# blairstar/NaturalDiffusion

Hardware: AMD Instinct MI355X
Metric: images/sec at 15-step Natural Inference (CIFAR10 32x32, NCSN++), 3-stream throughput (higher is better)
Workload: dtype bf16; 1 GPU; CIFAR10 NI 15-step step_15_weight_173.npz B=512/GPU NCSN++ 61.8M bf16, ni_step fp64 history; nfe=15, batch_per_gpu=512, streams=3

## Files before the change

include/natinf_ncsnpp.h:

```cpp
#ifndef NATINF_NCSNPP_H
#define NATINF_NCSNPP_H

#include <stdint.h>
#include "natinf.h"

#ifdef __cplusplus
extern "C" {
#endif

typedef struct natinf_ncsnpp* natinf_ncsnpp_t;

#define NATINF_NCSNPP_KEEP_ACTIVATIONS 1
#define NATINF_NCSNPP_DDPM 2

int64_t natinf_ncsnpp_param_count(void);
int64_t natinf_ncsnpp_packed_bytes(void);
int64_t natinf_ncsnpp_handle_param_count(natinf_ncsnpp_t h);
int64_t natinf_ncsnpp_handle_packed_bytes(natinf_ncsnpp_t h);
int64_t natinf_ncsnpp_workspace_bytes(natinf_ncsnpp_t h, int max_batch);

int natinf_ncsnpp_create(natinf_ncsnpp_t* out, int flags);
int natinf_ncsnpp_destroy(natinf_ncsnpp_t h);

int natinf_ncsnpp_describe(natinf_ncsnpp_t h, char* buf, int cap);

int natinf_ncsnpp_load(natinf_ncsnpp_t h, const float* params_f32, int64_t n_params,
                       void* packed, int64_t packed_bytes, natinf_stream_t stream);

int natinf_ncsnpp_share(natinf_ncsnpp_t h, natinf_ncsnpp_t loaded);

int natinf_ncsnpp_forward(natinf_ncsnpp_t h, const float* x, const float* labels, float* out, int B,
                          void* workspace, int64_t workspace_bytes, natinf_stream_t stream);

int natinf_ncsnpp_describe_gemms(natinf_ncsnpp_t h, int B, char* buf, int cap);

int natinf_debug_gemm(int variant, int M, int N, int K0, int K1, int taps, int logW, int batch,
                      const void* a0, const void* a1, const void* b, const float* bias_n, void* c, int c_f32, float scale,
                      int iters, natinf_stream_t stream);
int natinf_debug_quant_fp8_rows(const float* w, void* q, float* row_scale, int rows, int cols, natinf_stream_t stream);
int natinf_debug_gemm_fused(int variant, int M, int N, int K, const void* a, const void* b, const float* bias_n, const float* bias_m,
                            const float* rowvec, const float* gate, int log_rows_per_sample, const void* resid_bf16, const float* resid_f32,
                            float scale, int act, void* c, int c_f32, float* gn_part, int* bm_out, int fp32_slab, natinf_stream_t stream);
int natinf_debug_set_conv_operand(int logW, const void* a1, int c1);
int natinf_debug_gemm_fp8(int M, int N, int K, const void* a8, const float* a_scale, const void* a_mx, const void* b8, const float* b_scale,
                          const float* bias_n, void* c, void* c_mx, int c_mode, int iters, natinf_stream_t stream);
int natinf_debug_conv_gn_up(int flags);
int natinf_debug_conv_gn_fin(float* fin_scale, float* fin_shift, const float* gamma, const float* beta, int channels_per_group, float mul);
int natinf_debug_conv_gn(int res, int B, int N, int cin, int c1, const void* x, const float* scale, const float* shift, const void* w_packed, void* w_frag,
                         const void* a1, const float* bias_n, const void* resid, float out_scale, void* out, float* gn_part, int iters,
                         natinf_stream_t stream);
#define NATINF_ATTN_BLOCK_OFF_WQKV 0
#define NATINF_ATTN_BLOCK_OFF_W3 393216
#define NATINF_ATTN_BLOCK_OFF_FOLD_WQK 524288
#define NATINF_ATTN_BLOCK_OFF_FOLD_WVO 786432
#define NATINF_ATTN_BLOCK_OFF_FOLD_CQ 1048576
#define NATINF_ATTN_BLOCK_OFF_FOLD_BO 1049600
#define NATINF_ATTN_BLOCK_OFF_WQK_PACKED 1050624
#define NATINF_ATTN_BLOCK_OFF_WVO_PACKED 1181696
#define NATINF_ATTN_BLOCK_PACKED_BYTES 1312768
#define NATINF_ATTN_BLOCK_SCRATCH_BYTES_PER_SAMPLE 393216
int natinf_debug_attn_block(int plan, int B, const void* x, int x_ld, const float* scale, const float* shift, const float* w, const float* bias,
                            void* packed, void* scratch, void* out, int o_ld, float out_scale, float* gn_part, natinf_stream_t stream);
int natinf_set_gemm_variant(int variant);
int natinf_set_gemm_epilogue(int fp32_slab);
int natinf_set_gemm_pref512(int on);
int natinf_set_gemm_half_issue(int on);
int natinf_set_gemm_round_model(int on);
int natinf_set_gemm_w128(int on);
int natinf_set_gemm_raster(int rows);
int natinf_set_fuse_gn(int on);
int natinf_set_conv_gn_wide(int mask);
int natinf_set_conv_gn_w128(int mask);
int natinf_set_conv_gn_w128_min_k(int shape, int k);
int natinf_set_conv_gn_regw(int on);
int natinf_set_fuse_up(int on);
int natinf_set_fuse_up_fold(int on);
int natinf_debug_fold_up_weights(const float* w, int N, int cin, float w_mul, float* out_f32, void* out_packed, natinf_stream_t stream);
int natinf_debug_conv_up_fold(int B, int N, int cin, const void* x, const float* scale, const float* shift, const float* w, void* w_packed, void* h_scratch,
                              const float* bias_n, const float* rowvec, float out_scale, void* out, float* gn_part, int iters, natinf_stream_t stream);
int natinf_set_fuse_head(int on);
int natinf_set_fuse_gn8(int on);
int natinf_set_fuse_gn4(int on);
int natinf_set_fuse_fin(int on);
int natinf_set_conv_gn_warm(int mask);
int natinf_set_attn256(int on);
int natinf_set_attn_proj(int on);
int natinf_set_attn_waves8(int on);
int natinf_set_attn_block(int on);
int natinf_set_attn_qkv(int on);
int natinf_set_conv_gn8_tile(int one_image);
int natinf_set_gemm_splitk(int on);
int natinf_debug_set_splitk_workspace(float* ws, int max_slices);
int natinf_debug_timestamps(void* dev_buf16);

int natinf_ncsnpp_profile(natinf_ncsnpp_t h, int enable);
int natinf_ncsnpp_profile_read(natinf_ncsnpp_t h, double* ms_by_class , int64_t* launches_by_class );

int natinf_gemm_profile(int enable);
int natinf_gemm_profile_read(char* buf, int cap);

int natinf_ncsnpp_debug_tap(natinf_ncsnpp_t h, int module_idx, float* out, int64_t capacity_elems,
                            natinf_stream_t stream);

int natinf_debug_gn_stats(const void* x, int ld, int C, int HW, int B, const float* gamma, const float* beta, float* scale, float* shift, float eps, float out_mul,
                          natinf_stream_t stream);
int natinf_debug_gn_finalize(const float* P0, int tps0, int quads0, const float* P1, int tps1, int quads1, int C, int HW, int B, const float* gamma, const float* beta,
                             float* scale, float* shift, float eps, float out_mul, natinf_stream_t stream);
int natinf_debug_gn_fold(const float* P, int tps, int quads, int fold, int B, float* out, natinf_stream_t stream);
int natinf_debug_gn_apply(const void* x, int ld, int C, int logW, int logHW, int B, const float* scale, const float* shift, void* y, void* xr, int act, int mode, int pad,
                          natinf_stream_t stream);
int natinf_debug_head_conv(const void* x, int ld, int B, const float* scale, const float* shift, const void* w16, const float* bias, float* out, natinf_stream_t stream);
int natinf_debug_time_embed(const float* labels, void* emb, int B, natinf_stream_t stream);
int natinf_debug_stem_im2col(const float* x, void* A, int B, natinf_stream_t stream);
int natinf_debug_pack_conv(const float* src, void* dst, int N, int Cin, int taps, int dst_ld, int koff, int tap_stride_c, int chunked, float wmul, natinf_stream_t stream);
int natinf_debug_pack_transpose(const float* src, void* dst, int K, int N, int dst_ld, natinf_stream_t stream);
int natinf_debug_nhwc_to_nchw(const void* x, int ld, int C, int HW, int B, float* out, natinf_stream_t stream);

#ifdef __cplusplus
}
#endif
#endif
```

naturaldiffusion_amd/_lib.py:

```python
from __future__ import annotations

import ctypes as C
import os
from pathlib import Path

os.environ.setdefault("GPU_MAX_HW_QUEUES", "8")

_HERE = Path(__file__).resolve().parent
LIB_PATH = Path(os.environ.get("NATINF_LIB", _HERE / "libnatinf.so"))

if not LIB_PATH.exists():
    raise ImportError(
        f"{LIB_PATH} not found: build it with `make -C {_HERE / 'csrc'}` "
        "(or `python -c 'import __graft_entry__ as g; g.build()'`). "
        "naturaldiffusion_amd has no CPU or eager-PyTorch fallback.")

lib = C.CDLL(str(LIB_PATH))

_p, _i32, _i64, _f32, _f64 = C.c_void_p, C.c_int, C.c_int64, C.c_float, C.c_double

SIGNATURES = {
    "natinf_abi_version": (C.c_int, []),
    "natinf_strerror": (C.c_char_p, [_i32]),
    "natinf_probe": (C.c_int, []),
    "natinf_step_f64hist": (C.c_int, [_p, _p, _p, _p, _p, _p, _p, _i32, _f64, _i32, _f64, _f64, _f32, _f32, _i64, _p]),
    "natinf_step_f32hist": (C.c_int, [_p, _p, _p, _p, _p, _p, _p, _i32, _f32, _i32, _f32, _f32, _f32, _f32, _i64, _p]),
    "natinf_weighted_sum_f64": (C.c_int, [_p, _p, _p, _p, _i32, _i64, _p]),
    "natinf_randn_philox_f32": (C.c_int, [_p, _i64, _i64, _p, _i64, _i64, C.c_uint64, _p]),
    "natinf_randn_philox_col_f32": (C.c_int, [_p, _i64, _i64, _p, _i64, _i64, C.c_uint64, C.c_uint32, _p]),
    "natinf_step_f64hist_noise": (C.c_int, [_p, _p, _p, _p, _p, _p, _p, _i32, _f64, _p, _p, _i32, _i32, _f64, _f64, _f32,
                                            C.c_uint64, _p, _i64, _i64, _i64, _i64, _p]),
    "natinf_known_blend_f32": (C.c_int, [_p, _p, _p, _p, _i64, _i64, _f32, _f32, C.c_uint32, C.c_uint64, _p, _i64, _i64, _i64, _i64, _p]),
    "natinf_step_f64hist_inpaint": (C.c_int, [_p, _p, _p, _p, _p, _p, _p, _i32, _f64, _p, _p, _i32, _i32, _f64, _f64, _f32,
                                              C.c_uint64, _p, _i64, _i64, _i64, _i64, _p, _p, _i64, _i64, _f32, _f32, C.c_uint32, _p]),
    "natinf_x0_threshold_f64": (C.c_int, [_p, _p, _i64, _i64, _i32, _f64, _f64, _p]),
    "natinf_step_f64hist_x0fix": (C.c_int, [_p, _p, _p, _p, _p, _p, _p, _i32, _f64, _p, _p, _i32, _i32, _f64, _f64, _f32,
                                            C.c_uint64, _p, _i64, _i64, _i64, _i64, _p, _p, _i64, _i64, _f32, _f32, C.c_uint32,
                                            _i32, _f64, _f64, _p, _p]),
    "natinf_x0_project_f64": (C.c_int, [_p, _p, _p, _i64, _i32, _i32, _i32, _i32, _i64, _p]),
    "natinf_step_f64hist_project": (C.c_int, [_p, _p, _p, _p, _p, _p, _p, _i32, _f64, _p, _p, _i32, _i32, _f64, _f64, _f32,
                                              C.c_uint64, _p, _i64, _i64, _i64, _i64, _p, _i64, _i32, _i32, _i32, _i32, _p, _p]),
    "natinf_color_blend_f32": (C.c_int, [_p, _p, _p, _i64, _p, _p, _f32, _f32, C.c_uint32, C.c_uint64, _p, _i64, _i64, _i64, _i64, _p]),
    "natinf_step_f64hist_colorize": (C.c_int, [_p, _p, _p, _p, _p, _p, _p, _i32, _f64, _p, _p, _i32, _i32, _f64, _f64, _f32,
                                               C.c_uint64, _p, _i64, _i64, _i64, _i64, _p, _i64, _p, _p, _f32, _f32, C.c_uint32, _p]),
    "natinf_to_pixel_u8": (C.c_int, [_p, _p, _i32, _i32, _i32, _i32, _i32, _p]),
    "natinf_step_f32prod": (C.c_int, [_p, _p, _p, _f32, _i64, _i64, _p, _p, _p, _p, _p, _i32, _f32, _p, _p, _i32,
                                      _i32, _f32, _f32, _i64, _p]),
    "natinf_step_f32prod_noise": (C.c_int, [_p, _p, _p, _f32, _i64, _i64, _p, _p, _p, _p, _p, _i32, _f32, _p, _p, _i32,
                                            _i32, _f32, _f32, C.c_uint64, _p, _i64, _i64, _i64, _p]),
    "natinf_step_f32prod_noise_guided": (C.c_int, [_p, _p, _p, _p, _p, _i32, _i64, _i64, _p, _p, _p, _p, _p, _i32, _f32, _p, _p, _i32,
                                                   _i32, _f32, _f32, C.c_uint64, _p, _i64, _i64, _i64, _p]),
    "natinf_step_f32prod_inpaint": (C.c_int, [_p, _p, _p, _p, _p, _i32, _i64, _i64, _p, _p, _p, _p, _p, _i32, _f32, _p, _p, _i32,
                                              _i32, _f32, _f32, C.c_uint64, _p, _i64, _i64, _i64,
                                              _p, _p, _i64, _i64, _f32, _f32, C.c_uint32, _p]),
    "natinf_weighted_sum_f32prod": (C.c_int, [_p, _p, _p, _p, _i32, _i64, _p]),
    "natinf_step_f16chain": (C.c_int, [_p, _p, _p, _p, _p, _p, _p, _p, _p, _i32, _f32, _f32, _i32, _f32, _f32, _f32,
                                       _f32, _i32, _i64, _p]),
    "natinf_step_f16chain_guided": (C.c_int, [_p, _p, _p, _p, _p, _i32, _i64, _p, _p, _p, _p, _p, _p, _i32, _f32, _f32, _i32, _f32, _f32,
                                              _f32, _i32, _i64, _p]),
    "natinf_known_blend_f16": (C.c_int, [_p, _p, _p, _p, _p, _i64, _i64, _f32, _f32, C.c_uint32, C.c_uint64, _p, _i64, _i64, _i64, _i64, _p]),
    "natinf_step_f16chain_inpaint": (C.c_int, [_p, _p, _p, _p, _p, _i32, _i64, _p, _p, _p, _p, _p, _p, _i32, _f32, _f32, _i32, _f32, _f32,
                                               _f32, _i32, _i64, _p, _p, _i64, _i64, C.c_uint32, C.c_uint64, _p, _i64, _i64, _p]),
    "natinf_weighted_mean_f16": (C.c_int, [_p, _p, _p, _p, _i32, _f32, _i64, _p]),
    "natinf_flow_input_f16": (C.c_int, [_p, _p, _p, _f32, _f32, _i64, _p]),
    "natinf_ncsnpp_param_count": (C.c_int64, []),
    "natinf_ncsnpp_workspace_bytes": (C.c_int64, [_p, _i32]),
    "natinf_ncsnpp_packed_bytes": (C.c_int64, []),
    "natinf_ncsnpp_handle_param_count": (_i64, [_p]),
    "natinf_ncsnpp_handle_packed_bytes": (_i64, [_p]),
    "natinf_ncsnpp_create": (C.c_int, [C.POINTER(_p), _i32]),
    "natinf_ncsnpp_describe": (C.c_int, [_p, C.c_char_p, _i32]),
    "natinf_ncsnpp_destroy": (C.c_int, [_p]),
    "natinf_ncsnpp_load": (C.c_int, [_p, _p, _i64, _p, _i64, _p]),
    "natinf_ncsnpp_share": (C.c_int, [_p, _p]),
    "natinf_ncsnpp_forward": (C.c_int, [_p, _p, _p, _p, _i32, _p, _i64, _p]),
    "natinf_ncsnpp_debug_tap": (C.c_int, [_p, _i32, _p, _i64, _p]),
    "natinf_ncsnpp_describe_gemms": (C.c_int, [_p, _i32, C.c_char_p, _i32]),
    "natinf_debug_gemm": (C.c_int, [_i32, _i32, _i32, _i32, _i32, _i32, _i32, _i32, _p, _p, _p, _p, _p, _i32, _f32, _i32, _p]),
    "natinf_set_gemm_variant": (C.c_int, [_i32]),
    "natinf_debug_timestamps": (C.c_int, [_p]),
    "natinf_set_gemm_epilogue": (C.c_int, [_i32]),
    "natinf_debug_gemm_fused": (C.c_int, [_i32, _i32, _i32, _i32, _p, _p, _p, _p, _p, _p, _i32, _p, _p, _f32, _i32, _p, _i32, _p, _p, _i32, _p]),
    "natinf_set_gemm_pref512": (C.c_int, [_i32]),
    "natinf_set_gemm_half_issue": (C.c_int, [_i32]),
    "natinf_set_gemm_raster": (C.c_int, [_i32]),
    "natinf_set_gemm_round_model": (C.c_int, [_i32]),
    "natinf_set_gemm_w128": (C.c_int, [_i32]),
    "natinf_set_fuse_gn": (C.c_int, [_i32]),
    "natinf_set_conv_gn_wide": (C.c_int, [_i32]),
    "natinf_set_attn_block": (C.c_int, [_i32]),
    "natinf_set_conv_gn_w128": (C.c_int, [_i32]),
    "natinf_set_conv_gn_w128_min_k": (C.c_int, [_i32, _i32]),
    "natinf_set_conv_gn_regw": (C.c_int, [_i32]),
    "natinf_set_fuse_up": (C.c_int, [_i32]),
    "natinf_set_fuse_up_fold": (C.c_int, [_i32]),
    "natinf_debug_fold_up_weights": (C.c_int, [_p, _i32, _i32, _f32, _p, _p, _p]),
    "natinf_debug_conv_up_fold": (C.c_int, [_i32, _i32, _i32, _p, _p, _p, _p, _p, _p, _p, _p, _f32, _p, _p, _i32, _p]),
    "natinf_set_fuse_head": (C.c_int, [_i32]),
    "natinf_set_fuse_gn8": (C.c_int, [_i32]),
    "natinf_set_fuse_gn4": (C.c_int, [_i32]),
    "natinf_set_fuse_fin": (C.c_int, [_i32]),
    "natinf_set_attn_proj": (C.c_int, [_i32]),
    "natinf_set_attn_waves8": (C.c_int, [_i32]),
    "natinf_set_attn_qkv": (C.c_int, [_i32]),
    "natinf_set_conv_gn_warm": (C.c_int, [_i32]),
    "natinf_set_attn256": (C.c_int, [_i32]),
    "natinf_set_conv_gn8_tile": (C.c_int, [_i32]),
    "natinf_set_gemm_splitk": (C.c_int, [_i32]),
    "natinf_debug_set_splitk_workspace": (C.c_int, [_p, _i32]),
    "natinf_debug_set_conv_operand": (C.c_int, [_i32, _p, _i32]),
    "natinf_debug_conv_gn": (C.c_int, [_i32, _i32, _i32, _i32, _i32, _p, _p, _p, _p, _p, _p, _p, _p, _f32, _p, _p, _i32, _p]),
    "natinf_debug_conv_gn_up": (C.c_int, [_i32]),
    "natinf_debug_conv_gn_fin": (C.c_int, [_p, _p, _p, _p, _i32, _f32]),
    "natinf_debug_attn_block": (C.c_int, [_i32, _i32, _p, _i32, _p, _p, _p, _p, _p, _p, _p, _i32, _f32, _p, _p]),
    "natinf_debug_gn_stats": (C.c_int, [_p, _i32, _i32, _i32, _i32, _p, _p, _p, _p, _f32, _f32, _p]),
    "natinf_debug_gn_finalize": (C.c_int, [_p, _i32, _i32, _p, _i32, _i32, _i32, _i32, _i32, _p, _p, _p, _p, _f32, _f32, _p]),
    "natinf_debug_gn_fold": (C.c_int, [_p, _i32, _i32, _i32, _i32, _p, _p]),
    "natinf_debug_gn_apply": (C.c_int, [_p, _i32, _i32, _i32, _i32, _i32, _p, _p, _p, _p, _i32, _i32, _i32, _p]),
    "natinf_debug_head_conv": (C.c_int, [_p, _i32, _i32, _p, _p, _p, _p, _p, _p]),
    "natinf_debug_time_embed": (C.c_int, [_p, _p, _i32, _p]),
    "natinf_debug_stem_im2col": (C.c_int, [_p, _p, _i32, _p]),
    "natinf_debug_pack_conv": (C.c_int, [_p, _p, _i32, _i32, _i32, _i32, _i32, _i32, _i32, _f32, _p]),
    "natinf_debug_pack_transpose": (C.c_int, [_p, _p, _i32, _i32, _i32, _p]),
    "natinf_debug_nhwc_to_nchw": (C.c_int, [_p, _i32, _i32, _i32, _i32, _p, _p]),
    "natinf_ncsnpp_profile": (C.c_int, [_p, _i32]),
    "natinf_ncsnpp_profile_read": (C.c_int, [_p, C.POINTER(C.c_double), C.POINTER(C.c_int64)]),
    "natinf_debug_quant_fp8_rows": (C.c_int, [_p, _p, _p, _i32, _i32, _p]),
    "natinf_debug_gemm_fp8": (C.c_int, [_i32, _i32, _i32, _p, _p, _p, _p, _p, _p, _p, _p, _i32, _i32, _p]),
    "natinf_dit_create": (C.c_int, [C.POINTER(_p), _i32, _i32, _i32, _i32]),
    "natinf_dit_create_sized": (C.c_int, [C.POINTER(_p), _i32, _i32, _i32, _i32, _i32]),
    "natinf_dit_input_size": (C.c_int, [_p]),
    "natinf_dit_attention_bf16": (C.c_int, [_p, _p, _p, _i32, _p, _i32, _i32, _i32, _i32, _i32, _i32, _p]),
    "natinf_dit_destroy": (C.c_int, [_p]),
    "natinf_dit_param_count": (C.c_int64, [_p]),
    "natinf_dit_packed_bytes": (C.c_int64, [_p]),
    "natinf_dit_workspace_bytes": (C.c_int64, [_p, _i32]),
    "natinf_dit_load": (C.c_int, [_p, _p, _i64, _p, _i64, _p]),
    "natinf_dit_forward": (C.c_int, [_p, _p, _p, _p, _p, _i32, _p, _i64, _p]),
    "natinf_dit_stream_sites": (C.c_int, [_p]),
    "natinf_dit_stream_status_reset": (C.c_int, [_p, _p, _p]),
    "natinf_dit_stream_status": (C.c_int, [_p, _p, _p, _p]),
    "natinf_debug_ln_modulate": (C.c_int, [_p, _i32, _p, _p, _i32, _p, _p, _p, _i32, _i64, _i32, C.POINTER(_i32), _p]),
    "natinf_debug_softmax_rows": (C.c_int, [_i32, _p, _p, _i32, _i64, _p]),
    "natinf_mmdit_create": (C.c_int, [C.POINTER(_p), _i32, _i32, _i32, _i32, _i32, _i32, _i32, _i32]),
    "natinf_mmdit_destroy": (C.c_int, [_p]),
    "natinf_mmdit_param_count": (C.c_int64, [_p]),
    "natinf_mmdit_packed_bytes": (C.c_int64, [_p]),
    "natinf_mmdit_workspace_bytes": (C.c_int64, [_p, _i32]),
    "natinf_mmdit_load": (C.c_int, [_p, _p, _i64, _p, _i64, _p]),
    "natinf_mmdit_forward": (C.c_int, [_p, _p, _p, _p, _p, _p, _i32, _p, _i64, _p]),
    "natinf_mmdit_stream_sites": (C.c_int, [_p]),
    "natinf_mmdit_stream_status_reset": (C.c_int, [_p, _p, _p]),
    "natinf_mmdit_stream_status": (C.c_int, [_p, _p, _p, _p]),
    "natinf_attention_hd64_bf16": (C.c_int, [_p, _p, _i32, _i64, _p, _p, _i32, _i64, _i32, _i32, _i32, _i32, C.c_float, _p]),
    "natinf_debug_attention_hd64_fp8out": (C.c_int, [_p, _p, _i32, _i64, _p, _p, _p, _i32, _i32, _i32, _i32, C.c_float, _p]),
    "natinf_inception_create": (C.c_int, [_p, _i32, _i32]),
    "natinf_inception_destroy": (C.c_int, [_p]),
    "natinf_set_inception_conv": (C.c_int, [_i32]),
    "natinf_debug_conv_ring": (C.c_int, [_i32] * 14 + [_p, _p, _p, _p, _p, _p, _i32, _p]),
    "natinf_debug_inc_stem": (C.c_int, [_p, _i32, _i32, _i32, _i32, _i32, _i32, _p, _p]),
    "natinf_debug_inc_pool": (C.c_int, [_i32] * 8 + [_p, _i32, _p, _i32, _p]),
    "natinf_debug_inc_global_avg": (C.c_int, [_i32, _i32, _i32, _i32, _p, _p, _p]),
    "natinf_debug_inc_pack": (C.c_int, [_i32, _p, _p, _p, _p, _p] + [_i32] * 7 + [_p, _p, _p, _p]),
    "natinf_debug_inc_im2col": (C.c_int, [_i32] * 11 + [_p, _p, _p]),
    "natinf_inception_param_count": (_i64, [_p]),
    "natinf_inception_packed_bytes": (_i64, [_p]),
    "natinf_inception_workspace_bytes": (_i64, [_p, _i32]),
    "natinf_inception_load": (C.c_int, [_p, _p, _i64, _p, _i64, _p]),
    "natinf_inception_forward": (C.c_int, [_p, _p, _i32, _p, _i32, _p, _i64, _p]),
    "natinf_gemm_profile": (C.c_int, [_i32]),
    "natinf_gemm_profile_read": (C.c_int, [_p, _i32]),
    "natinf_set_mmdit_stream16": (C.c_int, [_i32]),
    "natinf_set_dit_stream16": (C.c_int, [_i32]),
    "natinf_set_mmdit_text_flat": (C.c_int, [_i32]),
    "natinf_attention_profile": (C.c_int, [_i32]),
    "natinf_set_mmdit_text_stream": (C.c_int, [_i32]),
    "natinf_set_flash_mode": (C.c_int, [_i32]),
    "natinf_attention_profile_read": (C.c_int, [_p, _p]),
    "natinf_vae_create": (C.c_int, [C.POINTER(_p), _i32, _i32]),
    "natinf_vae_destroy": (C.c_int, [_p]),
    "natinf_vae_param_count": (C.c_int64, [_p]),
    "natinf_vae_packed_bytes": (C.c_int64, [_p]),
    "natinf_vae_workspace_bytes": (C.c_int64, [_p, _i32]),
    "natinf_vae_load": (C.c_int, [_p, _p, _i64, _p, _i64, _p]),
    "natinf_vae_decode": (C.c_int, [_p, _p, _p, _i32, _p, _i64, _p]),
    "natinf_vae_enc_create": (C.c_int, [C.POINTER(_p), _i32, _i32]),
    "natinf_vae_enc_destroy": (C.c_int, [_p]),
    "natinf_vae_enc_param_count": (C.c_int64, [_p]),
    "natinf_vae_enc_packed_bytes": (C.c_int64, [_p]),
    "natinf_vae_enc_workspace_bytes": (C.c_int64, [_p, _i32]),
    "natinf_vae_enc_load": (C.c_int, [_p, _p, _i64, _p, _i64, _p]),
    "natinf_vae_posterior_f32": (C.c_int, [_p, _p, _i64, _i32, _i64, _i32, _f32, _f32, C.c_uint64, _p, _i64, _i64, _p]),
    "natinf_vae_encode": (C.c_int, [_p, _p, _p, _p, _i32, _i32, _f32, _f32, C.c_uint64, _p, _i64, _i64, _p, _i64, _p]),
    "natinf_posterior_workspace_bytes": (C.c_int64, [_i32, _i32]),
    "natinf_posterior_samples": (C.c_int, [_p, _p, _f32, _f32, C.c_uint64, _p, _i64, _i64, _i32, _i32, _p, _p]),
    "natinf_posterior_stats": (C.c_int, [_p, _f64, _i32, _i32, _p, _p, _p, _p]),
    "natinf_posterior_debug_planes": (C.c_int, [_p, _i32, _i32, _p]),
    "natinf_prdc_workspace_bytes": (C.c_int64, [_i64, _i64, _i32, _i32]),
    "natinf_prdc_planes": (C.c_int, [_p, _i64, _i32, _p, _p, _p]),
    "natinf_prdc_knn_radius": (C.c_int, [_p, _p, _i64, _p, _p, _i64, _i32, _i32, _i64, _p, _p, _i64, _p]),
    "natinf_prdc_ball_counts": (C.c_int, [_p, _p, _i64, _p, _p, _i64, _i32, _i64, _p, _p, _p, _p, _p]),
    "natinf_prdc_debug_dist2": (C.c_int, [_p, _p, _i64, _p, _p, _i64, _i32, _i64, _p, _p]),
    "natinf_nn_workspace_bytes": (C.c_int64, [_i64, _i64, _i32, _i32]),
    "natinf_nn_nearest": (C.c_int, [_p, _p, _i64, _p, _p, _i64, _i32, _i32, _i64, _p, _p, _p, _i64, _p]),
    "natinf_kid_workspace_bytes": (C.c_int64, [_i64, _i64, _i32]),
    "natinf_kid_row_sums": (C.c_int, [_p, _i64, _i64, _p, _i64, _i64, _i32, _i64, _f64, _f64, _p, _p, _i64, _p]),
    "natinf_is_workspace_bytes": (C.c_int64, [_i64, _i32, _i32]),
    "natinf_is_row_stats": (C.c_int, [_p, _i64, _i64, _p, _i64, _i32, _i32, _p, _p, _p, _p, _p, _p, _i64, _p]),
    "natinf_ideal_tplanes": (C.c_int, [_p, _i64, _i32, _p, _p]),
    "natinf_ideal_workspace_bytes": (C.c_int64, [_i64, _i64, _i32]),
    "natinf_ideal_posterior_mean": (C.c_int, [_p, _p, _i64, _p, _p, _p, _i64, _i32, _i64, _p, _p, _p, _p, _p, _p, _p, _p, _p, _i64, _p]),
    "natinf_ideal_debug_weights": (C.c_int, [_p, _p, _i64, _p, _p, _i64, _i32, _i64, _p, _p, _p, _i64, _p]),
    "natinf_fit_gram_f64": (C.c_int, [_p, _i64, C.POINTER(C.c_int32), _i32, _p, _p, _i64, _i64, _p, _p]),
}

for _name, (_res, _args) in SIGNATURES.items():
    try:
        _fn = getattr(lib, _name)
    except AttributeError as e:
        raise ImportError(f"{LIB_PATH} does not export {_name}; rebuild it") from e
    _fn.restype, _fn.argtypes = _res, _args

X0_CLIP, X0_DYNAMIC = 1, 2
SD3_CFG_ON_VELOCITY = 1
SD3_BLEND_MEAN = 2
DIT_UNFUSED_ATTENTION = 1
DIT_FP8 = 2
DIT_STREAM_GUARD = 16
MMDIT_FP8 = 1
MMDIT_STREAM_GUARD = 2


def check(rc: int, what: str) -> None:
    if rc != 0:
        raise RuntimeError(f"{what} failed: {lib.natinf_strerror(rc).decode()} ({rc})")


def stream_ptr(stream=None) -> int:
    import torch
    s = stream if stream is not None else torch.cuda.current_stream()
    return int(s.cuda_stream)


def ptr(t) -> int:
    return 0 if t is None else int(t.data_ptr())


class StreamGuardStatus:
    _guard_api = ""
    guard = False

    def _guard_entry(self, name):
        if not self.guard:
            raise RuntimeError("this engine was created without guard=True: it keeps no stream status")
        return getattr(lib, f"{self._guard_api}_{name}")

    @property
    def site_names(self):
        n = self._guard_entry("stream_sites")(self._h)
        check(min(n, 0), f"{self._guard_api}_stream_sites")
        return ["patch_embed"] + [f"blocks.{i // 2}.{'mlp' if i % 2 else 'attn'}" for i in range(n - 1)]

    def reset_stream_status(self) -> None:
        import torch
        with torch.cuda.device(self._ws.device):
            check(self._guard_entry("stream_status_reset")(self._h, ptr(self._ws), stream_ptr()), f"{self._guard_api}_stream_status_reset")

    def stream_status(self):
        import torch
        n = len(self.site_names)
        buf = torch.empty(2 * n, dtype=torch.int32, device=self._ws.device)
        with torch.cuda.device(self._ws.device):
            check(self._guard_entry("stream_status")(self._h, ptr(self._ws), ptr(buf), stream_ptr()), f"{self._guard_api}_stream_status")
        raw = buf.cpu().numpy().view("uint32").reshape(n, 2)
# ... 10 lines not shown
```

naturaldiffusion_amd/csrc/engine_core.h:

```cpp
#pragma once
#include <functional>
#include <map>
#include <vector>

#include "natinf_ncsnpp.h"
#include "gemm_launch.h"

namespace ncsn {

__global__ void k_transpose_f32(const float* __restrict__ src, float* __restrict__ dst, int N, int K)
{
    const int64_t i = (int64_t)blockIdx.x * blockDim.x + threadIdx.x;
    if (i >= (int64_t)N * K) return;
    const int n = (int)(i / K), k = (int)(i - (int64_t)n * K);
    dst[(int64_t)k * N + n] = src[i];
}
}

namespace {

inline int ilog2(int v) { int l = 0; while ((1 << l) < v) ++l; return l; }
inline int64_t align_up(int64_t v, int64_t a) { return (v + a - 1) / a * a; }

struct TRef { int64_t off = -1; int C = 0, ld = 0, res = 0, coff = 0, pad = 0; };

struct Ctx {
    int B; unsigned char* ws; const unsigned char* wp; hipStream_t stream;
    const float* x; const float* labels; float* out;
    int* part_bm;
    hipStream_t stream2 = nullptr; hipEvent_t* ev = nullptr;
    unsigned char* fin_done = nullptr;
    uint32_t* guard = nullptr;
    uint32_t* site(int i) const { return guard ? guard + 2 * i : nullptr; }
    bf16* act(const TRef& t) const { return reinterpret_cast<bf16*>(ws + t.off * B) + t.coff; }
    template <class T> T* at(int64_t off) const { return reinterpret_cast<T*>(ws + off * B); }
    template <class T> const T* w(int64_t off) const { return reinterpret_cast<const T*>(wp + off); }
};
using OpFn = std::function<void(const Ctx&)>;

struct PackCtx { const float* params; unsigned char* packed; hipStream_t stream; };
using PackFn = std::function<void(const PackCtx&)>;

struct Arena {
    bool keep = false; int64_t top = 0, peak = 0;
    std::map<int64_t, int64_t> free_;
    std::map<int64_t, int64_t> live_;
    int64_t alloc(int64_t bytes) {
        bytes = align_up(bytes, 256);
        if (!keep)
            for (auto it = free_.begin(); it != free_.end(); ++it)
                if (it->second >= bytes) {
                    const int64_t off = it->first, rest = it->second - bytes;
                    free_.erase(it);
                    if (rest) free_[off + bytes] = rest;
                    live_[off] = bytes;
                    return off;
                }
        const int64_t off = top; top += bytes; if (top > peak) peak = top;
        live_[off] = bytes;
        return off;
    }
    void release(int64_t off) {
        if (keep || off < 0) return;
        auto it = live_.find(off);
        if (it == live_.end()) return;
        int64_t o = off, s = it->second;
        live_.erase(it);
        auto nx = free_.lower_bound(o);
        if (nx != free_.end() && o + s == nx->first) { s += nx->second; nx = free_.erase(nx); }
        if (nx != free_.begin()) { auto pv = std::prev(nx); if (pv->first + pv->second == o) { o = pv->first; s += pv->second; free_.erase(pv); } }
        if (o + s == top) top = o; else free_[o] = s;
    }
};

}

struct EngineCore {
    int64_t n_params = 0, packed_bytes = 0, ws_per_image = 0;
    std::vector<OpFn> ops;
    std::vector<PackFn> packs;
    const unsigned char* packed = nullptr;
    bool configured = false;
    std::vector<int> part_bm{128};
    int guard_sites = 0;
    int64_t guard_bytes() const { return guard_sites ? align_up((int64_t)guard_sites * 8, 256) : 0; }
    int64_t workspace_bytes(int max_batch) const { return ws_per_image * (int64_t)max_batch + guard_bytes(); }
    int status_reset(void* ws, hipStream_t s) const {
        if (!guard_sites || !ws) return NATINF_EINVAL;
        return hipMemsetAsync(ws, 0, (size_t)guard_sites * 8, s) == hipSuccess ? NATINF_OK : NATINF_ELAUNCH;
    }
    int status_read(const void* ws, uint32_t* out_dev, hipStream_t s) const {
        if (!guard_sites || !ws || !out_dev) return NATINF_EINVAL;
        return hipMemcpyAsync(out_dev, ws, (size_t)guard_sites * 8, hipMemcpyDeviceToDevice, s) == hipSuccess ? NATINF_OK : NATINF_ELAUNCH;
    }
    int load(const float* params_f32, int64_t n, void* dst, int64_t dst_bytes, hipStream_t s) {
        if (!params_f32 || !dst || n != n_params || dst_bytes < packed_bytes) return NATINF_EINVAL;
        PackCtx p{params_f32, reinterpret_cast<unsigned char*>(dst), s};
        for (const auto& f : packs) f(p);
        packed = reinterpret_cast<const unsigned char*>(dst);
        return hipGetLastError() == hipSuccess ? NATINF_OK : NATINF_ELAUNCH;
    }
    int run(const float* x, const float* t, float* out, int B, void* ws, int64_t ws_bytes, hipStream_t s, hipStream_t s2 = nullptr, hipEvent_t* ev = nullptr) {
        if (!x || !t || !out || !ws || B <= 0) return NATINF_EINVAL;
        if (!packed) return NATINF_ESTATE;
        if (ws_bytes < workspace_bytes(B)) return NATINF_EINVAL;
        if (!configured) { if (!configure_gemm_kernels()) return NATINF_ENODEV; configured = true; }
        Ctx c{B, reinterpret_cast<unsigned char*>(ws) + guard_bytes(), packed, s, x, t, out, part_bm.data()};
        c.stream2 = s2; c.ev = ev;
        if (guard_sites) { c.guard = reinterpret_cast<uint32_t*>(ws); g_launch_error = 0; }
        for (const auto& f : ops) f(c);
        if (guard_sites && g_launch_error) { g_launch_error = 0; return NATINF_ESTATE; }
        return hipGetLastError() == hipSuccess ? NATINF_OK : NATINF_ELAUNCH;
    }
};

namespace {

struct PlanBuilder {
    EngineCore& E;
    Arena arena;
    int64_t wtop = 0, poff = 0;
    explicit PlanBuilder(EngineCore& e) : E(e) {}
    int64_t wres(int64_t bytes) { const int64_t o = wtop; wtop += align_up(bytes, 256); return o; }
    int64_t take(int64_t n) { const int64_t o = poff; poff += n; return o; }
    void op(OpFn f) { E.ops.push_back(std::move(f)); }
    int64_t pack_bf16(int64_t src, int rows, int cols) {
        const int64_t dst = wres((int64_t)rows * cols * 2);
        E.packs.push_back([=](const PackCtx& p) {
            const int64_t n = (int64_t)rows * cols;
            hipLaunchKernelGGL(k_pack_conv, dim3(grid1d(n, 256, 1 << 30)), dim3(256), 0, p.stream, p.params + src,
                               reinterpret_cast<bf16*>(p.packed + dst), rows, cols, 1, cols, 0, cols, 0, 1.0f);
        });
        return dst;
    }
    void pack_bf16_at(int64_t src, int rows, int cols, int64_t dst) {
        E.packs.push_back([=](const PackCtx& p) {
            const int64_t n = (int64_t)rows * cols;
            hipLaunchKernelGGL(k_pack_conv, dim3(grid1d(n, 256, 1 << 30)), dim3(256), 0, p.stream, p.params + src,
                               reinterpret_cast<bf16*>(p.packed + dst), rows, cols, 1, cols, 0, cols, 0, 1.0f);
        });
    }
    int64_t pack_f32(int64_t src, int64_t n, int64_t src2 = -1) {
        const int64_t dst = wres(n * 4);
        pack_f32_at(src, n, dst, src2);
        return dst;
    }
    int64_t pack_f32_transposed(int64_t src, int rows, int cols) {
        const int64_t dst = wres((int64_t)rows * cols * 4);
        E.packs.push_back([=](const PackCtx& p) {
            const int64_t n = (int64_t)rows * cols;
            hipLaunchKernelGGL(k_transpose_f32, dim3(grid1d(n, 256, 1 << 30)), dim3(256), 0, p.stream, p.params + src,
                               reinterpret_cast<float*>(p.packed + dst), rows, cols);
        });
        return dst;
    }
    void pack_f32_at(int64_t src, int64_t n, int64_t dst, int64_t src2 = -1) {
        E.packs.push_back([=](const PackCtx& p) {
            hipLaunchKernelGGL(k_copy_add_f32, dim3(grid1d(n, 256, 1 << 30)), dim3(256), 0, p.stream, p.params + src,
                               src2 >= 0 ? p.params + src2 : (const float*)nullptr, reinterpret_cast<float*>(p.packed + dst), (int)n);
        });
    }

    void pack_fp8_at(int64_t src, int rows, int cols, int64_t wdst, int64_t sdst) {
        E.packs.push_back([=](const PackCtx& p) {
            hipLaunchKernelGGL(k_pack_fp8_rows, dim3((unsigned)((rows + 3) / 4)), dim3(256), 0, p.stream, p.params + src,
                               reinterpret_cast<uint8_t*>(p.packed + wdst), reinterpret_cast<float*>(p.packed + sdst), rows, cols);
        });
    }

    void finish() { E.n_params = poff; E.packed_bytes = wtop; E.ws_per_image = arena.peak; }
};

}
```

naturaldiffusion_amd/csrc/gemm_launch.h:

```cpp
#pragma once
#include <hip/hip_runtime.h>
#include <stdint.h>
#include <stdio.h>
#include <string.h>
#include <string>
#include <type_traits>
#include <utility>
#include <vector>

#include "ncsnpp_kernels.h"
#include "gemm_dma.h"
#include "gemm_w128.h"
#include "conv_gn2.h"
#include "gemm_fp8.h"

using namespace ncsn;

bool configure_conv_ring();
namespace { bool configure_ncsnpp_kernels();
            bool configure_dit_attention();
            bool configure_flash_attention(); }
namespace ncsn_sg { bool configure(); bool has_tile(int variant); void launch_tile(const void* gemm_args, int variant, int raster, void* stream);
                    void launch_fp8(const void* gemm_args, int mxa, int w128, int raster, void* stream); void launch_splitk_reduce(const void* gemm_args, int slices, void* stream);
                    void launch_patch_embed(const float* z, const float* Wt, const float* bias, const float* pos, float* x, int C, int g, int D, int64_t rows, int x_f16, uint32_t* guard, void* stream); }
namespace ncsn_upf { bool configure(); void launch(const void* gemm_args, int epi, void* stream); void fold(const float* w, void* dst_bf16, float* dst_f32, int N, int Cin, float wmul, void* stream); }
namespace ncsn_cg3 { bool configure(); int tile_rows(int shape); int tile_cols(int shape); void launch(const void* gemm_args, int shape, int epi, void* stream); }

namespace {

int g_epi_fp32_slab = 0;
GemmArgs gemm_defaults() {
    GemmArgs g;
    memset(&g, 0, sizeof(g));
    g.epi_fp32_slab = g_epi_fp32_slab;
    g.taps = 1; g.batch = 1; g.scale = 1.0f; g.act = ACT_NONE; g.c_mode = OUT_BF16;
    return g;
}
constexpr int NUM_CU = 256;
enum GemmVariant {
    V_AUTO = 0, V_GENERIC = 1,
    V_DMA_256x256 = 2, V_DMA_256x128 = 3, V_DMA_128x128 = 4,
    V_RING_256x256 = 5, V_RING_256x128 = 6, V_RING_128x128 = 7,
    V_RING_64x128 = 8,
    V_RING_256x128_W4 = 9,
    V_DMA_256x128_W4 = 10,
    V_DMA_256x256_S = 11, V_DMA_128x128_S = 12,
    V_DMA_512x128 = 13,
    V_PATCH_256x256 = 14, V_PATCH_256x128 = 15,
    V_DMA_256x256_P = 16, V_DMA_256x128W4_P = 18,
    V_DMA_128x128_P = 17,
    V_8PH_256x256 = 19, V_8PH_NOPRIO = 20, V_8PH_READFIRST = 21, V_8PH_BOTH = 22,
    V_FP8_256x256 = 23,
    V_ABL_NODMA = 24, V_ABL_NOMFMA = 25,
    V_DMA_256x256_H = 26, V_DMA_512x128_H = 27,
    V_CONV_GN = 28,
    V_W128 = 29,
    V_W128_A = 30, V_W128_D = 31, V_W128_X = 32,
    V_COUNT
};
const char* variant_name(int v) {
    static const char* n[] = {"auto", "generic128", "dma256x256", "dma256x128", "dma128x128", "ring256x256", "ring256x128",
                              "ring128x128", "ring64x128", "ring256x128w4", "dma256x128w4", "dma256x256s", "dma128x128s", "dma512x128", "patch256x256", "patch256x128", "dma256x256p", "dma128x128p", "dma256x128w4p", "gemm8ph", "gemm8ph_np", "gemm8ph_rf", "gemm8ph_nprf", "fp8_256x256", "abl_nodma", "abl_nomfma", "dma256x256h", "dma512x128h", "conv_gn", "w128_256x256", "w128_a", "w128_d", "w128_x"};
    return v >= 0 && v < V_COUNT ? n[v] : "?";
}
unsigned long long* g_dbg_ts = nullptr;
int g_force_variant = V_AUTO;
int g_round_model = 1;
int g_round_model_w128 = 13;
int g_pref_512 = 1;
std::string* g_record = nullptr;

int g_raster_g = 8;
template <class Cfg, class K>
inline void launch_tiles(K kernel, const GemmArgs& g0, hipStream_t s) {
    const int nM = (g0.M + Cfg::BM_ - 1) / Cfg::BM_, nN = (g0.N + Cfg::BN_ - 1) / Cfg::BN_;
    GemmArgs g = g0;
    g.raster_g = (g_raster_g > 1 && nN >= 8 && nM >= g_raster_g) ? g_raster_g : 0;
    hipLaunchKernelGGL(kernel, dim3(nM * nN, 1, g.batch), dim3(Cfg::THREADS), Cfg::LDS_BYTES, s, g);
}
template <class Cfg, class K>
inline bool set_lds(K kernel) {
    return hipFuncSetAttribute(reinterpret_cast<const void*>(kernel), hipFuncAttributeMaxDynamicSharedMemorySize, Cfg::LDS_BYTES) == hipSuccess;
}
int g_cg_warm = 15;

constexpr unsigned EPI_ALL = 0x1FF;
template <unsigned MASK, int E, class F> inline void epi_case(F&& f) { if constexpr ((MASK >> E) & 1u) f(std::integral_constant<int, E>{}); }
template <unsigned MASK, class F> inline bool for_each_epi(F&& f) {
    bool ok = true;
    auto one = [&](auto tag) { ok = ok && f(tag); };
    epi_case<MASK, 0>(one); epi_case<MASK, 1>(one); epi_case<MASK, 2>(one); epi_case<MASK, 3>(one); epi_case<MASK, 4>(one);
    epi_case<MASK, 5>(one); epi_case<MASK, 6>(one); epi_case<MASK, 7>(one); epi_case<MASK, 8>(one);
    return ok;
}
#define NATINF_EPI_OF(tag) decltype(tag)::value

template <class... F> struct FamList {};
template <class Fam> bool configure_family() {
    return for_each_epi<Fam::EPI>([](auto t) { return set_lds<typename Fam::Cfg>(Fam::template kernel<NATINF_EPI_OF(t)>()); });
}
template <class... F> bool configure_families(FamList<F...>) { return (configure_family<F>() && ...); }
template <class Fam> void launch_family(int e, const GemmArgs& g, hipStream_t s) {
    for_each_epi<Fam::EPI>([&](auto t) {
        if (NATINF_EPI_OF(t) != e) return true;
        launch_tiles<typename Fam::Cfg>(Fam::template kernel<NATINF_EPI_OF(t)>(), g, s);
        return false;
    });
}

using CfgD256x256 = DmaCfg<2, 4, 8, 4>;
struct FamD128  { static constexpr int V = V_DMA_128x128_P;    using Cfg = DmaCfg<2, 2, 4, 4>;     static constexpr unsigned EPI = EPI_ALL;
                  template <int E> static constexpr auto kernel() { return &k_gemm_dma<2, 2, 4, 4, 2, E>; } };
struct FamRW4   { static constexpr int V = V_RING_256x128_W4;  using Cfg = RingCfg<2, 2, 8, 4, 3>; static constexpr unsigned EPI = EPI_ALL & ~(1u << 3);
                  template <int E> static constexpr auto kernel() { return &k_gemm_ring<2, 2, 8, 4, 3, E>; } };
struct FamR64   { static constexpr int V = V_RING_64x128;      using Cfg = RingCfg<2, 2, 2, 4, 4>; static constexpr unsigned EPI = EPI_ALL;
                  template <int E> static constexpr auto kernel() { return &k_gemm_ring<2, 2, 2, 4, 4, E>; } };
struct FamD256H { static constexpr int V = V_DMA_256x256_H;    using Cfg = CfgD256x256;            static constexpr unsigned EPI = EPI_ALL & ~(1u << 3);
                  template <int E> static constexpr auto kernel() { return &k_gemm_dma<2, 4, 8, 4, 6, E>; } };
struct FamD512H { static constexpr int V = V_DMA_512x128_H;    using Cfg = DmaCfg<4, 2, 8, 4>;     static constexpr unsigned EPI = EPI_ALL & ~((1u << 3) | (1u << 4) | (1u << 7) | (1u << 8));
                  template <int E> static constexpr auto kernel() { return &k_gemm_dma<4, 2, 8, 4, 6, E>; } };
struct FamW128  { static constexpr int V = V_W128;             using Cfg = W128Cfg;                static constexpr unsigned EPI = EPI_ALL & ~((1u << 2) | (1u << 3) | (1u << 6));
                  template <int E> static constexpr auto kernel() { return &k_gemm_w128<E>; } };
using GemmFamilies = FamList<FamD128, FamRW4, FamR64, FamD256H, FamD512H, FamW128>;
using CfgR128x128 = RingCfg<2, 2, 4, 4, 4>;

template <class F, class... Fam> constexpr bool with_family(int v, F&& f, FamList<Fam...>) { return ((v == Fam::V && (f(Fam{}), true)) || ...); }
template <class F> constexpr bool with_family(int v, F&& f) { return with_family(v, f, GemmFamilies{}); }
constexpr bool variant_shipped(int v) {
    return v == V_AUTO || v == V_GENERIC || v == V_FP8_256x256 || v == V_CONV_GN || with_family(v, [](auto) {});
}
constexpr unsigned epi_mask(int v) { unsigned m = 1u; with_family(v, [&](auto f) { m = decltype(f)::EPI; }); return m; }
constexpr int variant_bm(int v) {
    int bm = (v == V_CONV_GN || v == V_FP8_256x256) ? 256 : 128;
    with_family(v, [&](auto f) { bm = decltype(f)::Cfg::BM_; });
    return bm;
}
static_assert(variant_bm(V_RING_64x128) == 64 && variant_bm(V_DMA_128x128_P) == 128 && variant_bm(V_RING_256x128_W4) == 256 && variant_bm(V_DMA_256x256_H) == 256 &&
              variant_bm(V_DMA_512x128_H) == 512 && variant_bm(V_W128) == 256 && variant_bm(V_GENERIC) == 128, "the block-tile rows choose_variant and the GroupNorm partial tables count on");
static_assert(variant_shipped(V_W128) && !variant_shipped(V_DMA_256x256) && !variant_shipped(V_W128_X) && epi_mask(V_GENERIC) == 1u, "retired ids stay refused");

constexpr unsigned EPI_CONV_GN = (1u << 1) | (1u << 2) | (1u << 5) | (1u << 6);
template <int RES_, bool WIDE, int TM = 8, int NG = 1, int TN = 4> struct CgShape {
    static constexpr int RES = RES_; using Cfg = ConvGn2Cfg<RES_, WIDE, TM, NG, TN>; static constexpr unsigned EPI = EPI_CONV_GN;
    template <int E> static constexpr auto kernel() { return &k_conv_gn2<RES_, WIDE, E, TM, NG, TN>; }
    static bool takes(int res, int bm) { return res == RES_ && (RES_ <= 8 || WIDE == (bm == 128)); }
};
using CgH4T = CgShape<4, true, 4, 2, 2>;
using ConvGnShapes = FamList<CgShape<32, false>, CgShape<32, true>, CgShape<16, false>, CgShape<16, true>, CgShape<8, true, 4>, CgH4T>;
template <class... S> void launch_conv_gn2(FamList<S...>, int res, int bm, int e, const GemmArgs& g, hipStream_t s) {
    ((S::takes(res, bm) && (launch_family<S>(e, g, s), true)) || ...);
}

constexpr int UPFOLD_W = 16, UPFOLD_BM = UPFOLD_W * UPFOLD_W, UPFOLD_BN = 256;

constexpr unsigned EPI_FP8 = 0xF;
template <bool MXA> struct FamF8     { using Cfg = CfgD256x256; static constexpr unsigned EPI = EPI_FP8; template <int E> static constexpr auto kernel() { return &k_gemm_fp8<MXA, E>; } };
template <bool MXA> struct FamF8W128 { using Cfg = W128F8Cfg;   static constexpr unsigned EPI = EPI_FP8; template <int E> static constexpr auto kernel() { return &k_gemm_w128_fp8<MXA, E>; } };
using Fp8Families = FamList<FamF8<false>, FamF8<true>, FamF8W128<false>, FamF8W128<true>>;

bool configure_gemm_kernels() {
    bool ok = hipFuncSetAttribute(reinterpret_cast<const void*>(&k_gemm_bf16), hipFuncAttributeMaxDynamicSharedMemorySize,
                                  GEMM_LDS_BYTES) == hipSuccess;
    ok = ok && set_lds<CfgR128x128>(&k_gemm_ring<2, 2, 4, 4, 4, 9>) && set_lds<W128Cfg>(&k_gemm_w128<9>) &&
         configure_families(GemmFamilies{}) && configure_families(ConvGnShapes{}) && ncsn_upf::configure() && configure_families(Fp8Families{}) &&
         ncsn_cg3::configure() && ncsn_sg::configure() && ::configure_conv_ring() && configure_ncsnpp_kernels() && configure_dit_attention() && configure_flash_attention();
    if (!ok) (void)hipGetLastError();
    return ok;
}


int packed_epi(const GemmArgs& g, int bm);
int g_cg3 = 7;
int g_cg_wide = 3;
int g_cg3_min_k[3] = {2304, 0, 2304};
inline int conv_gn3_shape(const GemmArgs& g) {
    const int res = 1 << g.logW;
    if (!g_cg3 || !g.b_frag || g.N % 128) return -1;
    int sh = -1;
    if (res == 32) sh = g.N % 256 ? ((g_cg3 & 1) ? 0 : -1) : ((g_cg3 & 2) ? 1 : -1);
    else if (res == 16) sh = (g.N % 256 == 0 && (g_cg3 & 4)) ? 2 : -1;
    if (sh >= 0 && 9 * g.a0_C + (g.a1 ? g.a1_C : 0) < g_cg3_min_k[sh]) sh = -1;
    return sh;
}
inline int conv_gn_bm(const GemmArgs& g) {
    const int res = 1 << g.logW;
    if (const int sh3 = conv_gn3_shape(g); sh3 >= 0) return ncsn_cg3::tile_rows(sh3);
    if (res == 8 || res == 4) return 64;
    if (res == 32) return ((g_cg_wide & 2) && g.N % 256 == 0 && g.b_frag) ? 128 : 256;
    return ((g_cg_wide & 1) && res == 16 && g.N % 256 == 0) ? 128 : 256;
}
inline int conv_gn_part_rows(const GemmArgs& g) { const int res = 1 << g.logW; return res <= 8 ? res * res : conv_gn_bm(g); }
inline bool conv_gn_regw(const GemmArgs& g) { return g.b_frag && (conv_gn3_shape(g) >= 0 || g.N % ((conv_gn_bm(g) <= 128 && (1 << g.logW) != 4) ? 256 : 128) == 0); }
inline int conv_gn_epi(const GemmArgs& g) { GemmArgs t = g; t.epi_fp32_slab = 0; return packed_epi(t, conv_gn_part_rows(g)); }
inline bool conv_gn_ok(const GemmArgs& g) {
    if (!g.gn_scale || !g.gn_shift || !g.gn_folded || g.taps != 9 || g.batch != 1 || g.a0_C % BK || (g.a1 && g.a1_C % BK)) return false;
    const int res = 1 << g.logW;
    if (g.logHW != 2 * g.logW || (res != 32 && res != 16 && res != 8 && res != 4) || g.N % 8) return false;
    if (res == 4 && (g.a0_C % (64 * CgH4T::Cfg::NG) || (g.a1 && g.a1_C % (64 * CgH4T::Cfg::NG)))) return false;
    if (res <= 8 ? (g.M % (res * res) || g.N % (res == 4 ? 128 : 256) || g.a0_up || g.a1_up || (g.resid && g.rowvec)) : g.M % std::max(256, conv_gn_bm(g)) != 0) return false;
    if (!conv_gn_regw(g)) return false;
    const int e = conv_gn_epi(g);
    return e == 1 || e == 2 || e == 5 || e == 6;
}
int g_w128 = 1;
bool w128_ok(const GemmArgs& g) {
    if (g.taps != 1 || g.a1 || g.gn_scale || g.deq_m || g.deq_n || g.splitk > 1) return false;
    if (g.a0_C % BK || g.a0_C < 2 * BK || g.N % 8 || g.M % 8) return false;
    return (int64_t)g.M * g.a0_ld * 2 < (int64_t)1 << 32 && (int64_t)g.N * g.b_ld * 2 < (int64_t)1 << 32;
}
int choose_variant(const GemmArgs& g) {
    if (g.gn_scale) return V_CONV_GN;
    const int K0 = g.taps * g.a0_C, K1 = g.a1 ? g.a1_C : 0;
    const bool dma = K0 % BK == 0 && K1 % BK == 0 && (g.taps == 1 || (g.a0_padded && g.a0_C % BK == 0));
    if (!dma) return V_GENERIC;
    if (g_force_variant == V_W128) {
        if (w128_ok(g) && (!g.gn_part || (1 << g.logHW) % 256 == 0)) return V_W128;
    }
    else if (g_force_variant > V_GENERIC && g_force_variant != V_CONV_GN && g_force_variant != V_FP8_256x256) {
        if (!g.gn_part || ((g.taps == 9 || g.logHW > 0) && (1 << g.logHW) % variant_bm(g_force_variant) == 0)) return g_force_variant;
    }
    const int64_t mt256 = (g.M + 255) / 256, mt128 = (g.M + 127) / 128;
    const int64_t nt128 = (g.N + 127) / 128;
    const bool w128 = g_w128 && w128_ok(g) && (!g.gn_part || (1 << g.logHW) % 256 == 0);
    const int64_t nt256 = (g.N + 255) / 256;
    const bool n_ok256 = g.N % 256 == 0 || (w128 && g.N % 128 == 0);
    if (g_round_model && g.taps == 1 && !g.gn_part && g.batch == 1 && n_ok256 && K0 + K1 >= 1024 && mt256 * nt256 < 2 * NUM_CU) {
        const int64_t r256 = (mt256 * nt256 + NUM_CU - 1) / NUM_CU, r128 = (mt128 * nt128 + 2 * NUM_CU - 1) / (2 * NUM_CU);
        const int64_t c256 = w128 ? g_round_model_w128 : 15;
        if (mt128 * nt128 >= NUM_CU / 2) return c256 * r256 < 10 * r128 ? (w128 ? V_W128 : V_DMA_256x256_H) : V_DMA_128x128_P;
    }
    if (n_ok256 && K0 + K1 >= 1024 && mt256 * nt256 * g.batch >= NUM_CU) return w128 ? V_W128 : V_DMA_256x256_H;
    if (g_pref_512 && g.N <= 128 && K0 + K1 >= 1024 && ((g.M + 511) / 512) * g.batch >= 2 * NUM_CU &&
        (!g.gn_part || (g.taps == 9 && (1 << g.logHW) % 512 == 0)))
        return V_DMA_512x128_H;
    if (mt256 * nt128 * g.batch >= 2 * NUM_CU) return V_RING_256x128_W4;
    if (mt128 * nt128 * g.batch >= NUM_CU) return V_DMA_128x128_P;
    return V_RING_64x128;
}

int fp8_epi(const GemmArgs& g) {
    if (g.epi_fp32_slab || g.resid || g.gn_part) return 0;
    if ((g.rowvec || g.gate) && g.log_rows_per_sample < 30 && ((1 << g.log_rows_per_sample) % 256 != 0)) return 0;
    if (g.c_mode == OUT_F32 && g.resid_f32 && !g.bias_m && g.act == ACT_NONE && g.resid_f32_ld % 4 == 0 && g.c_ld % 4 == 0) return 3;
    if (g.resid_f32 || g.gate) return 0;
    if (g.c_mode == OUT_BF16 && g.act == ACT_NONE) return 1;
    if (g.c_mode == OUT_FP8_MX && g.act == ACT_GELU_TANH && g.c_mx && g.N % 32 == 0 && !g.bias_m && g.scale == 1.0f) return 2;
    return 0;
}
bool w128_fp8_ok(const GemmArgs& g) {
    return g.taps == 1 && !g.a1 && g.a0_C % 256 == 0 && g.N % 8 == 0 && g.M % 8 == 0 && (!g.a_mx || g.M % 256 == 0) &&
           (int64_t)g.M * g.a0_ld < (int64_t)1 << 32 && (int64_t)g.N * g.b_ld < (int64_t)1 << 32;
}
bool fp8_on_w128(const GemmArgs& g) { return g_w128 && w128_fp8_ok(g) && (fp8_epi(g) != 2 || g_w128 != 2); }
template <bool MXA>
void launch_gemm_fp8_t(const GemmArgs& g, hipStream_t s) {
    if (fp8_on_w128(g)) launch_family<FamF8W128<MXA>>(fp8_epi(g), g, s);
    else launch_family<FamF8<MXA>>(fp8_epi(g), g, s);
}
std::string gemm_row(int M, int N, int K0, int K1, int taps, int batch, const std::string& name, int epi) {
    char line[160];
    snprintf(line, sizeof(line), "%d %d %d %d %d %d %s/e%d", M, N, K0, K1, taps, batch, name.c_str(), epi);
    return line;
}
void record_gemm(const GemmArgs& g, const std::string& name, int epi) { *g_record += gemm_row(g.M, g.N, g.taps * g.a0_C, g.a1 ? g.a1_C : 0, g.taps, g.batch, name, epi) + "\n"; }
struct GemmProf {
    struct Rec { hipEvent_t a, b; std::string tag; };
    bool on = false; std::vector<Rec> ev; std::vector<std::pair<hipEvent_t, hipEvent_t>> pool;
    bool begin(Rec& r, hipStream_t s) {
        r.a = r.b = nullptr;
        if (!pool.empty()) { r.a = pool.back().first; r.b = pool.back().second; pool.pop_back(); }
        else if (hipEventCreate(&r.a) != hipSuccess || hipEventCreate(&r.b) != hipSuccess) { r.a = r.b = nullptr; (void)hipGetLastError(); return false; }
        (void)hipEventRecord(r.a, s);
        return true;
    }
    void end(Rec& r, hipStream_t s) { (void)hipEventRecord(r.b, s); ev.push_back(std::move(r)); }
} g_gemm_prof;
thread_local int g_launch_error = 0;
void launch_gemm_fp8(const GemmArgs& g, hipStream_t s) {
    if (g.stream_guard && fp8_epi(g) != 3) { g_launch_error = 1; return; }
    GemmProf::Rec r;
    const bool prof = g_gemm_prof.on && !g_record && g_gemm_prof.begin(r, s);
    if (prof) r.tag = gemm_row(g.M, g.N, g.taps * g.a0_C, 0, g.taps, g.batch, std::string(fp8_on_w128(g) ? "w128_fp8" : "fp8_256x256") + (g.a_mx ? "_mxa" : ""), g.stream_guard ? 4 : fp8_epi(g));
    if (g.stream_guard) ncsn_sg::launch_fp8(&g, g.a_mx != nullptr, fp8_on_w128(g), g_raster_g, (void*)s);
    else if (g.a_mx) launch_gemm_fp8_t<true>(g, s); else launch_gemm_fp8_t<false>(g, s);
    if (prof) g_gemm_prof.end(r, s);
}

int packed_epi(const GemmArgs& g, int bm) {
    if (g.epi_fp32_slab || g.deq_m || g.deq_n || g.act == ACT_RELU) return 0;
    if (g.bias_m) return (g.c_mode == OUT_BF16 && !g.resid && !g.resid_f32 && !g.gate && !g.rowvec && !g.gn_part && g.act == ACT_NONE) ? 8 : 0;
    if ((g.rowvec || g.gate) && g.log_rows_per_sample < 30 && ((1 << g.log_rows_per_sample) % bm != 0)) return 0;
    if (g.c_mode == OUT_F32 && g.resid_f32 && !g.resid && !g.gn_part && g.act == ACT_NONE && g.resid_f32_ld % 4 == 0 && g.c_ld % 4 == 0) return 7;
    if (g.c_mode != OUT_BF16 || g.resid_f32 || g.gate) return 0;
    if (g.resid && (g.act != ACT_NONE || g.resid_ld % 4 != 0)) return 0;
    if (g.gn_part) return (g.act == ACT_NONE && g.M % bm == 0) ? (g.resid ? 6 : 2) : 0;
    if (g.resid) return 5;
    return g.act == ACT_NONE ? 1 : (g.act == ACT_SILU ? 3 : 4);
}
inline int effective_epi(int v, const GemmArgs& g) { const int e = packed_epi(g, variant_bm(v)); return ((epi_mask(v) >> e) & 1u) ? e : 0; }

thread_local bool g_fin_written = false;
int g_splitk = 1;
float* g_dbg_splitk_ws = nullptr; int g_dbg_splitk_max = 0;
int splitk_slices(const GemmArgs& g) {
    if (!g_splitk || !g.splitk_ws || g.splitk_max < 2 || g.batch != 1 || g.gn_scale || g.c_mode != OUT_BF16 || g.N % 8 || 256 % (g.N / 8)) return 1;
    if (g.gn_part && (g.M % SPLITK_ROWS || g.act != ACT_NONE || (g.taps == 9 && (1 << g.logHW) % SPLITK_ROWS))) return 1;
    if (g.bias_m || g.gate || g.resid_f32 || g.deq_m || g.deq_n) return 1;
    const int K0 = g.taps * g.a0_C, K1 = g.a1 ? g.a1_C : 0;
    if (K0 % 64 || K1 % 64 || (g.taps == 9 && !g.a0_padded) || K0 + K1 < 2048) return 1;
    const int64_t tiles = ((g.M + 127) / 128) * ((g.N + 127) / 128);
    if (tiles >= 2 * NUM_CU) return 1;
    int S = (int)((2 * NUM_CU + tiles - 1) / tiles);
    if (S > g.splitk_max) S = g.splitk_max;
    while (S > 1 && (K0 + K1) / 32 / S < 16) --S;
    return S;
}
int w128_splitk_slices(const GemmArgs& g) {
// ... 101 lines not shown
```

naturaldiffusion_amd/csrc/ncsnpp.hip:

```cpp
#include <hip/hip_runtime.h>
#include <stdint.h>
#include <stdio.h>
#include <string.h>
#include <stdlib.h>
#include <functional>
#include <map>
#include <memory>
#include <string>
#include <vector>

#include "natinf_ncsnpp.h"
#include "gemm_launch.h"
#include "engine_core.h"
#include "head_conv.h"
#include "attn256.h"
#include "attn_qkv.h"
#include "attn_blk256.h"

namespace {

constexpr int NF = 128, IMG = 32, TEMB = 512, NLEVEL = 4;
constexpr int CH_MULT[NLEVEL] = {1, 2, 2, 2};
constexpr float GN_EPS = 1e-6f;
constexpr float INV_SQRT2 = 0.70710678118654752440f;
inline bool attn_at(int res) { return res == 16; }

enum Kind { K_LIN, K_CONV, K_RES, K_ATTN, K_GN, K_DOWN, K_UP };
const char* kind_name(int k) { static const char* n[] = {"lin", "conv", "res", "attn", "gn", "down", "up"}; return n[k]; }

struct Mod { int idx, kind, cin, cout, up, down, res; int64_t poff; };

enum { CLS_GEMM = 0, CLS_OTHER = 1, CLS_CONV_GN = 2, CLS_CONV_GN8 = 3, N_CLS = 4 };

int g_fuse_head = 1;
constexpr int ATTN_BLK_DEFAULT = 2;
int g_attn_blk = ATTN_BLK_DEFAULT;
int g_attn_qkv = 1;
int g_attn_w8 = 1;
int g_attn_proj = 1;
int g_fuse_gn8 = 1;
int g_fuse_fin = 3;
int g_fuse_gn4 = 1;
int g_fuse_gn = 1;
constexpr int UP_FOLD_DEFAULT = 1;
int g_fuse_up_fold = UP_FOLD_DEFAULT;
int g_fuse_up = 1;

}

struct natinf_ncsnpp : EngineCore {
    int flags = 0;
    std::vector<Mod> mods;
    std::vector<int> op_cls;
    bool prof = false;
    struct Rec { hipEvent_t a, b; int cls; };
    std::vector<Rec> recs;
    std::vector<hipEvent_t> pool;
    std::map<int, TRef> taps;
    uint64_t plan_sig = 0;
    int last_B = 0; unsigned char* last_ws = nullptr;
    std::vector<unsigned char> fin_done;
};

namespace {

bool configure_ncsnpp_kernels() {
    return hipFuncSetAttribute(reinterpret_cast<const void*>(&k_head_conv), hipFuncAttributeMaxDynamicSharedMemorySize, HeadConvCfg::LDS_BYTES) == hipSuccess &&
           hipFuncSetAttribute(reinterpret_cast<const void*>(&k_qkv256), hipFuncAttributeMaxDynamicSharedMemorySize, QKV_LDS_BYTES) == hipSuccess &&
           hipFuncSetAttribute(reinterpret_cast<const void*>(&k_attn256<false>), hipFuncAttributeMaxDynamicSharedMemorySize, A256_LDS_BYTES) == hipSuccess &&
           hipFuncSetAttribute(reinterpret_cast<const void*>(&k_attn256<true>), hipFuncAttributeMaxDynamicSharedMemorySize, A256_LDS_BYTES) == hipSuccess &&
           hipFuncSetAttribute(reinterpret_cast<const void*>(&k_attn256<true, 8>), hipFuncAttributeMaxDynamicSharedMemorySize, A256_LDS_BYTES) == hipSuccess &&
           hipFuncSetAttribute(reinterpret_cast<const void*>(&k_attn_blk256), hipFuncAttributeMaxDynamicSharedMemorySize, ABLK_LDS_BYTES) == hipSuccess &&
           hipFuncSetAttribute(reinterpret_cast<const void*>(&k_attn_blk256_v2), hipFuncAttributeMaxDynamicSharedMemorySize, ABLK2_LDS_BYTES) == hipSuccess;
}

struct AttnBlk256 {
    int plan = 0;
    int B = 0;
    const bf16* x = nullptr; int x_ld = 0;
    const float* sc = nullptr; const float* sh = nullptr;
    const bf16* wqkvf = nullptr; const float* bqk = nullptr; const float* bv = nullptr; bf16* qk = nullptr; bf16* vT = nullptr;
    const bf16* w3f = nullptr; const float* b3 = nullptr;
    const bf16* wqf2 = nullptr; const float* cq2 = nullptr; const bf16* wvof2 = nullptr; const float* bo2 = nullptr;
    bf16* out = nullptr; int o_ld = 0; float out_scale = 1.0f;
    float2* gn_part = nullptr; int gn_quads = 0;
};
void pack_attn_qkv_w(const float* w0, const float* w1, const float* w2, bf16* wqkvf, hipStream_t s) {
    hipLaunchKernelGGL(k_pack_qkv_w, dim3(3 * 256), dim3(256), 0, s, w0, w1, w2, wqkvf);
}
void pack_attn_w3(const float* w3, bf16* w3f, hipStream_t s) { hipLaunchKernelGGL(k_pack_attn_w3, dim3(256), dim3(256), 0, s, w3, w3f); }
void pack_attn_fold(const float* w0, const float* w1, const float* w2, const float* w3, const float* b0, const float* b2, const float* b3,
                    float* fq, float* cq, float* fv, float* bo, bf16* wqf2, bf16* wvof2, hipStream_t s) {
    hipLaunchKernelGGL(k_attn_fold_w, dim3(257), dim3(256), 0, s, w0, w1, w2, w3, b0, b2, b3, fq, cq, fv, bo);
    hipLaunchKernelGGL(k_pack_qkv_w, dim3(256), dim3(256), 0, s, (const float*)fq, (const float*)fq, (const float*)fq, wqf2, 1);
    hipLaunchKernelGGL(k_pack_attn_w3, dim3(256), dim3(256), 0, s, (const float*)fv, wvof2);
}
void launch_attn_qkv256(const AttnBlk256& a, hipStream_t s) {
    hipLaunchKernelGGL(k_qkv256, dim3((unsigned)a.B), dim3(512), QKV_LDS_BYTES, s, a.x, a.x_ld, a.sc, a.sh, a.wqkvf, a.bqk, a.bv, a.qk, a.vT);
}
int launch_attn_blk256(const AttnBlk256& a, hipStream_t s) {
    constexpr int C = 256;
    if (a.plan == 2) {
        hipLaunchKernelGGL(k_attn_blk256_v2, dim3((unsigned)a.B), dim3(512), ABLK2_LDS_BYTES, s, a.x, a.x_ld, a.sc, a.sh,
                           a.wqf2, a.cq2, 1.0f / sqrtf((float)C), a.wvof2, a.bo2, a.out, a.o_ld, a.out_scale, a.gn_part, a.gn_quads);
        return 256;
    }
    if (a.plan == 1) {
        hipLaunchKernelGGL(k_attn_blk256, dim3((unsigned)a.B), dim3(512), ABLK_LDS_BYTES, s, a.x, a.x_ld, a.sc, a.sh,
                           a.wqkvf, a.bqk, a.bv, a.qk, a.vT, 1.0f / sqrtf((float)C), a.w3f, a.b3, a.out, a.o_ld, a.out_scale, a.gn_part, a.gn_quads);
        return 256;
    }
    if (g_attn_w8) {
        hipLaunchKernelGGL((k_attn256<true, 8>), dim3((unsigned)a.B), dim3(512), A256_LDS_BYTES, s, (const bf16*)a.qk, 2 * C, C, (const bf16*)a.vT, a.out, a.o_ld,
                           1.0f / sqrtf((float)C), a.w3f, a.b3, a.x, a.x_ld, a.out_scale, a.gn_part, a.gn_quads);
        return 256;
    }
    hipLaunchKernelGGL(k_attn256<true>, dim3((unsigned)(2 * a.B)), dim3(256), A256_LDS_BYTES, s, (const bf16*)a.qk, 2 * C, C, (const bf16*)a.vT, a.out, a.o_ld,
                       1.0f / sqrtf((float)C), a.w3f, a.b3, a.x, a.x_ld, a.out_scale, a.gn_part, a.gn_quads);
    return 128;
}

struct Builder : PlanBuilder {
    natinf_ncsnpp& E;
    int dense_total = 0; int64_t dense_w = 0, dense_b = 0, dense_out = 0;

    const bool ddpm;
    const int NUM_RES;
    const float res_scale;
    explicit Builder(natinf_ncsnpp& e) : PlanBuilder(e), E(e), ddpm((e.flags & NATINF_NCSNPP_DDPM) != 0), NUM_RES(ddpm ? 2 : 4), res_scale(ddpm ? 1.0f : INV_SQRT2) {
        arena.keep = (e.flags & NATINF_NCSNPP_KEEP_ACTIVATIONS) != 0;
    }

    void op(int cls, OpFn f) { E.ops.push_back(std::move(f)); E.op_cls.push_back(cls); }

    void pack_conv(int64_t src, int64_t dst, int N, int Cin, int taps, int dst_ld, int koff, int tapstride, float wmul = 1.0f) {
        const int chunked = taps == 9 && Cin % BK == 0;
        E.packs.push_back([=](const PackCtx& p) {
            const int64_t n = (int64_t)N * Cin * taps;
            hipLaunchKernelGGL(k_pack_conv, dim3(grid1d(n, 256, 1 << 30)), dim3(256), 0, p.stream, p.params + src,
                               reinterpret_cast<bf16*>(p.packed + dst), N, Cin, taps, dst_ld, koff, tapstride, chunked, wmul);
        });
    }
    void pack_frag(int64_t src_packed, int64_t dst, int N, int ld, int cin, int c1) {
        E.packs.push_back([=](const PackCtx& p) {
            const int64_t n = (int64_t)(N / 16) * (9 * (cin / 32) + c1 / 32) * 64;
            hipLaunchKernelGGL(k_pack_frag, dim3(grid1d(n, 256, 1 << 30)), dim3(256), 0, p.stream, reinterpret_cast<const bf16*>(p.packed + src_packed),
                               reinterpret_cast<bf16*>(p.packed + dst), N, ld, cin, c1);
        });
    }
    void pack_fold_up(int64_t src, int64_t dst, int N, int Cin, float wmul) {
        E.packs.push_back([=](const PackCtx& p) {
            ncsn_upf::fold(p.params + src, p.packed + dst, nullptr, N, Cin, wmul, (void*)p.stream);
        });
    }
    void pack_transpose(int64_t src, int64_t dst, int K, int N, int dst_ld) {
        E.packs.push_back([=](const PackCtx& p) {
            hipLaunchKernelGGL(k_pack_transpose, dim3(grid1d((int64_t)K * N, 256, 1 << 30)), dim3(256), 0, p.stream,
                               p.params + src, reinterpret_cast<bf16*>(p.packed + dst), K, N, dst_ld);
        });
    }
    void pack_zero(int64_t dst, int64_t n) {
        E.packs.push_back([=](const PackCtx& p) {
            hipLaunchKernelGGL(k_fill_bf16_zero, dim3(grid1d(n, 256, 1 << 30)), dim3(256), 0, p.stream,
                               reinterpret_cast<bf16*>(p.packed + dst), n);
        });
    }

    struct GN { int64_t gamma, beta; };
    GN take_gn(int C) { GN g; g.gamma = pack_f32(take(C), C); g.beta = pack_f32(take(C), C); return g; }

    void emit_gn_stats(const TRef& x, GN gn, int64_t& sc, int64_t& sh, float out_mul = 1.0f) {
        if (emit_gn_from_parts(x, gn, sc, sh, out_mul)) return;
        const int HW = x.res * x.res;
        op(CLS_OTHER, [=](const Ctx& c) {
            hipLaunchKernelGGL(k_gn_stats, dim3(c.B), dim3(256), 0, c.stream, c.act(x), x.ld, x.C, HW,
                               c.w<float>(gn.gamma), c.w<float>(gn.beta), c.at<float>(sc), c.at<float>(sh), GN_EPS, out_mul);
        });
    }
    void emit_gn_apply(const TRef& x, int64_t sc, int64_t sh, const TRef& y, const TRef* xr, int act, int mode) {
        const int logW = ilog2(x.res), logHW = 2 * logW;
        const int rd = mode == RS_UP ? 2 * x.res : (mode == RS_DOWN ? x.res / 2 : x.res);
        const int rows_per_img = rd + 2 * y.pad;
        const TRef xrr = xr ? *xr : TRef();
        op(CLS_OTHER, [=](const Ctx& c) {
            hipLaunchKernelGGL(k_gn_apply, dim3((unsigned)((rows_per_img + GN_ROWS - 1) / GN_ROWS), (unsigned)c.B), dim3(256), 0, c.stream, c.act(x), x.ld, x.C,
                               logW, logHW, c.at<float>(sc), c.at<float>(sh), c.act(y),
                               xrr.off >= 0 ? c.act(xrr) : (bf16*)nullptr, act, mode, y.pad);
        });
    }
    TRef new_act(int res, int C, int pad = 0) {
        TRef t; t.off = arena.alloc((int64_t)(res + 2 * pad) * (res + 2 * pad) * C * 2); t.C = C; t.ld = C; t.res = res; t.pad = pad;
        return t;
    }

    void emit_res(const Mod& m, const TRef& x, const TRef& out) {
        const int cin = m.cin, cout = m.cout;
        const int ro = m.up ? m.res * 2 : (m.down ? m.res / 2 : m.res);
        const bool shortcut = cin != cout || m.up || m.down;
        const GN gn0 = take_gn(cin);
        const int64_t p_c0w = take((int64_t)cout * cin * 9), p_c0b = take(cout);
        const int64_t p_dw = take((int64_t)cout * TEMB), p_db = take(cout);
        const GN gn1 = take_gn(cout);
        const int64_t p_c1w = take((int64_t)cout * cout * 9), p_c1b = take(cout);
        const int64_t p_c2w = shortcut ? take((int64_t)cout * cin) : -1, p_c2b = shortcut ? take(cout) : -1;

        const int K0a = 9 * cin, K1tot = 9 * cout + (shortcut ? cin : 0);
        const bool fusable_res = g_fuse_gn && (ro == 32 || ro == 16 || (ro == 8 && g_fuse_gn8 && cout % 256 == 0) || (ro == 4 && g_fuse_gn4 && cout % 256 == 0));
        const bool fuse1 = fusable_res && cout % BK == 0;
        const bool fuse_up = fuse1 && ro > 8 && g_fuse_up && m.up && cin % BK == 0 && cout % 128 == 0;
        const bool fold_up = fuse_up && g_fuse_up_fold && !ddpm && ro == 2 * UPFOLD_W && cout == UPFOLD_BN;
        const bool fuse = (fusable_res && !m.up && !m.down && cin % BK == 0) || (fuse_up && !fold_up);
        const float LOG2E = 1.4426950408889634f, LN2 = 0.6931471805599453f;
        const float gn_mul = fuse ? -LOG2E : 1.0f, w_mul = fuse ? -LN2 : 1.0f, gn_mul1 = fuse1 ? -LOG2E : 1.0f, w_mul1 = fuse1 ? -LN2 : 1.0f;
        const int64_t w0 = wres((int64_t)cout * (fold_up ? 16 * cin : K0a) * 2), w1 = wres((int64_t)cout * K1tot * 2);
        if (fold_up) pack_fold_up(p_c0w, w0, cout, cin, w_mul);
        else pack_conv(p_c0w, w0, cout, cin, 9, K0a, 0, cin, w_mul);
        pack_conv(p_c1w, w1, cout, cout, 9, K1tot, 0, cout, w_mul1);
        if (shortcut && !ddpm) pack_conv(p_c2w, w1, cout, cin, 1, K1tot, 9 * cout, cin);
        if (shortcut && ddpm) pack_transpose(p_c2w, w1 + (int64_t)9 * cout * 2, cin, cout, K1tot);
        const int64_t w0f = (fuse && cout % 16 == 0) ? wres((int64_t)cout * K0a * 2) : -1, w1f = (fuse1 && cout % 16 == 0) ? wres((int64_t)cout * K1tot * 2) : -1;
        if (w0f >= 0) pack_frag(w0, w0f, cout, K0a, cin, 0);
        if (w1f >= 0) pack_frag(w1, w1f, cout, K1tot, cout, shortcut ? cin : 0);
        const int64_t b0 = pack_f32(p_c0b, cout), b1 = pack_f32(p_c1b, cout, shortcut ? p_c2b : -1);
        const int drow = dense_rows_next;
        pack_conv(p_dw, dense_w + (int64_t)drow * TEMB * 2, cout, TEMB, 1, TEMB, 0, TEMB);
        pack_f32_at(p_db, cout, dense_b + (int64_t)drow * 4);
        dense_rows_next += cout;

        const int64_t own_sc = arena.alloc((int64_t)std::max(cin, cout) * 4), own_sh = arena.alloc((int64_t)std::max(cin, cout) * 4);
        int64_t sc = own_sc, sh = own_sh;
        emit_gn_stats(x, gn0, sc, sh, gn_mul);
        TRef h, xr;
        if (fold_up) {
            h = new_act(m.res, cin, 1);
            emit_gn_apply(x, sc, sh, h, nullptr, ACT_SILU, RS_NONE);
        } else if (!fuse) {
            h = new_act(ro, cin, 1);
            if (m.up || m.down) xr = new_act(ro, cin);
            emit_gn_apply(x, sc, sh, h, (m.up || m.down) ? &xr : nullptr, ACT_SILU, m.up ? RS_UP : (m.down ? RS_DOWN : RS_NONE));
        }

        const int SK_MAX = 4;
        const int64_t skws = (ro <= 8) ? arena.alloc((int64_t)SK_MAX * ro * ro * cout * 4) : -1;
        TRef t = new_act(ro, cout);
        const Part pt = register_output(t, fuse);
        const int logW = ilog2(ro), logHW = 2 * logW, HWo = ro * ro;
        const int dtotal = dense_total; const int64_t dout = dense_out;
        op((fuse || fold_up) ? (ro <= 8 ? CLS_CONV_GN8 : CLS_CONV_GN) : CLS_GEMM, [=](const Ctx& c) {
            GemmArgs g = gemm_defaults();
            if (fold_up) {
                g.a0 = c.act(h); g.a0_ld = h.ld; g.a0_padded = 1; g.a0_C = cin; g.taps = 4; g.logW = logW - 1; g.logHW = logHW - 2;
                g.M = c.B * (HWo / 4); g.N = 4 * cout; g.b = c.w<bf16>(w0); g.b_ld = 4 * cin; g.bias_n = c.w<float>(b0);
                g.rowvec = c.at<float>(dout) + drow; g.rowvec_ld = dtotal; g.log_rows_per_sample = logHW - 2;
                g.c = c.act(t); g.c_ld = t.ld;
                if (pt.valid) { g.gn_part = c.at<float>(pt.off); g.gn_quads = pt.quads; }
                const int bm = launch_gemm(g, c.stream);
                if (pt.valid) c.part_bm[pt.id] = bm;
                return;
            }
            if (fuse) { g.a0 = c.act(x); g.a0_ld = x.ld; g.gn_scale = c.at<float>(sc); g.gn_shift = c.at<float>(sh); g.gn_ld = cin; g.gn_folded = 1; g.a0_up = fuse_up; }
            else { g.a0 = c.act(h); g.a0_ld = h.ld; g.a0_padded = 1; }
            g.a0_C = cin; g.taps = 9; g.logW = logW; g.logHW = logHW;
            g.M = c.B * HWo; g.N = cout; g.b = c.w<bf16>(w0); g.b_ld = K0a;
            if (w0f >= 0) g.b_frag = c.w<bf16>(w0f);
            g.bias_n = c.w<float>(b0);
            g.rowvec = c.at<float>(dout) + drow; g.rowvec_ld = dtotal; g.log_rows_per_sample = logHW;
            if (skws >= 0) { g.splitk_ws = c.at<float>(skws); g.splitk_max = SK_MAX; }
            g.c = c.act(t); g.c_ld = t.ld;
            if (pt.valid) { g.gn_part = c.at<float>(pt.off); g.gn_quads = pt.quads; set_fin(g, pt, c); }
            g_fin_written = false;
            const int bm = launch_gemm(g, c.stream);
            if (pt.valid) c.part_bm[pt.id] = bm;
            if (pt.fin && pt.fin->check) c.fin_done[pt.id] = g_fin_written;
        });
        if (!fuse) arena.release(h.off);
        int64_t sc1 = own_sc, sh1 = own_sh;
        emit_gn_stats(t, gn1, sc1, sh1, gn_mul1);
        TRef u;
        if (!fuse1) {
            u = new_act(ro, cout, 1);
            emit_gn_apply(t, sc1, sh1, u, nullptr, ACT_SILU, RS_NONE);
            arena.release(t.off);
        }
        if (pt.valid) arena.release(pt.off);
        const TRef xs = ((m.up || m.down) && !fuse_up) ? xr : x;
        const float rs = res_scale;
        const Part po = register_output(out, fuse1);
        op(fuse1 ? (ro <= 8 ? CLS_CONV_GN8 : CLS_CONV_GN) : CLS_GEMM, [=](const Ctx& c) {
            GemmArgs g = gemm_defaults();
            if (fuse1) { g.a0 = c.act(t); g.a0_ld = t.ld; g.gn_scale = c.at<float>(sc1); g.gn_shift = c.at<float>(sh1); g.gn_ld = cout; g.gn_folded = 1; }
            else { g.a0 = c.act(u); g.a0_ld = u.ld; g.a0_padded = 1; }
            g.a0_C = cout; g.taps = 9; g.logW = logW; g.logHW = logHW;
            if (shortcut) { g.a1 = c.act(xs); g.a1_ld = xs.ld; g.a1_C = cin; g.a1_up = fuse_up; }
            else { g.resid = c.act(xs); g.resid_ld = xs.ld; }
            g.M = c.B * HWo; g.N = cout; g.b = c.w<bf16>(w1); g.b_ld = K1tot;
            if (w1f >= 0) g.b_frag = c.w<bf16>(w1f);
            g.bias_n = c.w<float>(b1); g.scale = rs;
            if (skws >= 0) { g.splitk_ws = c.at<float>(skws); g.splitk_max = SK_MAX; }
            g.c = c.act(out); g.c_ld = out.ld;
            if (po.valid) { g.gn_part = c.at<float>(po.off); g.gn_quads = po.quads; set_fin(g, po, c); }
            g_fin_written = false;
            const int bm = launch_gemm(g, c.stream);
            if (po.valid) c.part_bm[po.id] = bm;
            if (po.fin && po.fin->check) c.fin_done[po.id] = g_fin_written;
        });
        if (skws >= 0) arena.release(skws);
        if (fuse1) arena.release(t.off); else arena.release(u.off);
        if ((m.up || m.down) && !fuse_up) arena.release(xr.off);
        arena.release(own_sc); arena.release(own_sh);
        if (sc != own_sc) { arena.release(sc); arena.release(sh); }
        if (sc1 != own_sc) { arena.release(sc1); arena.release(sh1); }
        E.taps[m.idx] = out;
    }

    void emit_attn(const Mod& m, const TRef& x, const TRef& out) {
        const int C = m.cin, T = m.res * m.res;
        const GN gn = take_gn(C);
        int64_t pw[4], pb[4];
        for (int i = 0; i < 4; ++i) { pw[i] = take((int64_t)C * C); pb[i] = take(C); }
        const int64_t wqk = wres((int64_t)2 * C * C * 2), wv = wres((int64_t)C * C * 2), w3 = wres((int64_t)C * C * 2);
        pack_transpose(pw[0], wqk, C, C, C);
        pack_transpose(pw[1], wqk + (int64_t)C * C * 2, C, C, C);
        pack_transpose(pw[2], wv, C, C, C);
        pack_transpose(pw[3], w3, C, C, C);
        const int64_t bqk = wres((int64_t)2 * C * 4);
        pack_f32_at(pb[0], C, bqk); pack_f32_at(pb[1], C, bqk + (int64_t)C * 4);
        const int64_t bv = pack_f32(pb[2], C), b3 = pack_f32(pb[3], C);

        const int64_t own_sc = arena.alloc((int64_t)C * 4), own_sh = arena.alloc((int64_t)C * 4);
        int64_t sc = own_sc, sh = own_sh;
        emit_gn_stats(x, gn, sc, sh);
        const bool fuse_qkv = T == 256 && C == 256 && g_attn_qkv;
        TRef h = new_act(m.res, C);
        if (!fuse_qkv) emit_gn_apply(x, sc, sh, h, nullptr, ACT_NONE, RS_NONE);
        const int64_t qk = arena.alloc((int64_t)T * 2 * C * 2), vT = arena.alloc((int64_t)C * T * 2);
        const bool blk = fuse_qkv && g_attn_proj && g_attn_w8 && g_attn_blk;
        int64_t wqkvf = -1;
        const int64_t sc_q = sc, sh_q = sh;
        if (fuse_qkv) {
            wqkvf = wres((int64_t)3 * C * C * 2);
            const int64_t s0 = pw[0], s1 = pw[1], s2 = pw[2];
            E.packs.push_back([=](const PackCtx& p) { pack_attn_qkv_w(p.params + s0, p.params + s1, p.params + s2, reinterpret_cast<bf16*>(p.packed + wqkvf), p.stream); });
            const int64_t sc_ = sc, sh_ = sh;
            if (!blk)
            op(CLS_GEMM, [=](const Ctx& c) {
                if (g_record) return;
                AttnBlk256 a;
                a.B = c.B; a.x = c.act(x); a.x_ld = x.ld; a.sc = c.at<float>(sc_); a.sh = c.at<float>(sh_);
                a.wqkvf = c.w<bf16>(wqkvf); a.bqk = c.w<float>(bqk); a.bv = c.w<float>(bv); a.qk = c.at<bf16>(qk); a.vT = c.at<bf16>(vT);
                launch_attn_qkv256(a, c.stream);
            });
        }
        if (!fuse_qkv)
        op(CLS_GEMM, [=](const Ctx& c) {
            GemmArgs g = gemm_defaults();
            g.a0 = c.act(h); g.a0_ld = C; g.a0_C = C; g.M = c.B * T; g.N = 2 * C;
            g.b = c.w<bf16>(wqk); g.b_ld = C; g.bias_n = c.w<float>(bqk);
            g.c = c.at<bf16>(qk); g.c_ld = 2 * C;
            launch_gemm(g, c.stream);
        });
        if (!fuse_qkv)
        op(CLS_GEMM, [=](const Ctx& c) {
            GemmArgs g = gemm_defaults();
            g.a0 = c.w<bf16>(wv); g.a0_ld = C; g.a0_C = C; g.a_bs = 0; g.M = C; g.N = T;
            g.b = c.act(h); g.b_ld = C; g.b_bs = (int64_t)T * C; g.bias_m = c.w<float>(bv);
            g.c = c.at<bf16>(vT); g.c_ld = T; g.c_bs = (int64_t)C * T; g.batch = c.B;
            launch_gemm(g, c.stream);
        });
        arena.release(h.off);
        const bool proj = T == 256 && C == 256 && g_attn_proj;
        int64_t w3f = -1;
        if (proj) {
            w3f = wres((int64_t)C * C * 2);
            const int64_t src = pw[3];
            E.packs.push_back([=](const PackCtx& p) { pack_attn_w3(p.params + src, reinterpret_cast<bf16*>(p.packed + w3f), p.stream); });
        }
        const bool blk2 = blk && g_attn_blk == 2;
        int64_t wqf2 = -1, wvof2 = -1, cq2 = -1, bo2 = -1;
        if (blk2) {
            const int64_t fq = wres((int64_t)C * C * 4), fv = wres((int64_t)C * C * 4);
            cq2 = wres((int64_t)C * 4); bo2 = wres((int64_t)C * 4);
            wqf2 = wres((int64_t)C * C * 2); wvof2 = wres((int64_t)C * C * 2);
            const int64_t w0_ = pw[0], w1_ = pw[1], w2_ = pw[2], w3_ = pw[3], b0_ = pb[0], b2_ = pb[2], b3_ = pb[3], cq_ = cq2, bo_ = bo2, wq_ = wqf2, wv_ = wvof2;
            E.packs.push_back([=](const PackCtx& p) {
                pack_attn_fold(p.params + w0_, p.params + w1_, p.params + w2_, p.params + w3_, p.params + b0_, p.params + b2_, p.params + b3_,
                               reinterpret_cast<float*>(p.packed + fq), reinterpret_cast<float*>(p.packed + cq_), reinterpret_cast<float*>(p.packed + fv),
                               reinterpret_cast<float*>(p.packed + bo_), reinterpret_cast<bf16*>(p.packed + wq_), reinterpret_cast<bf16*>(p.packed + wv_), p.stream);
            });
        }
        const Part po_attn = proj ? register_output(out) : Part();
        const float rs_attn = res_scale;
        TRef O = new_act(m.res, C);
        if (T == 256 && C == 256) {
            op(CLS_GEMM, [=](const Ctx& c) {
                if (g_record) return;
                if (proj) {
                    AttnBlk256 a;
                    a.plan = blk2 ? 2 : (blk ? 1 : 0); a.B = c.B; a.x = c.act(x); a.x_ld = x.ld; a.sc = c.at<float>(sc_q); a.sh = c.at<float>(sh_q);
                    if (wqkvf >= 0) a.wqkvf = c.w<bf16>(wqkvf);
                    a.bqk = c.w<float>(bqk); a.bv = c.w<float>(bv); a.qk = c.at<bf16>(qk); a.vT = c.at<bf16>(vT); a.w3f = c.w<bf16>(w3f); a.b3 = c.w<float>(b3);
                    if (blk2) { a.wqf2 = c.w<bf16>(wqf2); a.cq2 = c.w<float>(cq2); a.wvof2 = c.w<bf16>(wvof2); a.bo2 = c.w<float>(bo2); }
                    a.out = c.act(out); a.o_ld = out.ld; a.out_scale = rs_attn;
                    if (po_attn.valid) { a.gn_part = c.at<float2>(po_attn.off); a.gn_quads = po_attn.quads; }
                    const int rows = launch_attn_blk256(a, c.stream);
                    if (po_attn.valid) c.part_bm[po_attn.id] = rows;
                }
                else
                    hipLaunchKernelGGL(k_attn256<false>, dim3((unsigned)(2 * c.B)), dim3(256), A256_LDS_BYTES, c.stream, c.at<bf16>(qk), 2 * C, C, c.at<bf16>(vT), c.act(O), C,
                                       1.0f / sqrtf((float)C), (const bf16*)nullptr, (const float*)nullptr, (const bf16*)nullptr, 0, 1.0f, (float2*)nullptr, 0);
            });
            arena.release(vT); arena.release(qk);
        } else {
        const int64_t S = arena.alloc((int64_t)T * T * 4);
            op(CLS_GEMM, [=](const Ctx& c) {
                GemmArgs g = gemm_defaults();
                g.a0 = c.at<bf16>(qk); g.a0_ld = 2 * C; g.a0_C = C; g.a_bs = (int64_t)T * 2 * C; g.M = T; g.N = T;
                g.b = c.at<bf16>(qk) + C; g.b_ld = 2 * C; g.b_bs = (int64_t)T * 2 * C;
                g.scale = 1.0f / sqrtf((float)C);
                g.c = c.at<float>(S); g.c_ld = T; g.c_bs = (int64_t)T * T; g.c_mode = OUT_F32; g.batch = c.B;
// ... 77 lines not shown
        const int64_t b = pack_f32(pb, C);
        if (ident_sc < 0) {
            ident_sc = arena.alloc((int64_t)2 * NF * 4); ident_sh = arena.alloc((int64_t)2 * NF * 4);
            const int64_t isc = ident_sc, ish = ident_sh;
            op(CLS_OTHER, [=](const Ctx& c) {
                const int64_t n = (int64_t)c.B * 2 * NF;
                hipLaunchKernelGGL(k_fill_f32, dim3(grid1d(n, 256, 1 << 30)), dim3(256), 0, c.stream, c.at<float>(isc), 1.0f, n);
                hipLaunchKernelGGL(k_fill_f32, dim3(grid1d(n, 256, 1 << 30)), dim3(256), 0, c.stream, c.at<float>(ish), 0.0f, n);
            });
        }
        TRef u = new_act(ro, C, 1);
        emit_gn_apply(x, ident_sc, ident_sh, u, nullptr, ACT_NONE, RS_UP);
        const Part po = register_output(out);
        const int logW = ilog2(ro);
        op(CLS_GEMM, [=](const Ctx& c) {
            GemmArgs g = gemm_defaults();
            g.a0 = c.act(u); g.a0_ld = u.ld; g.a0_C = C; g.taps = 9; g.logW = logW; g.logHW = 2 * logW; g.a0_padded = 1;
            g.M = c.B * ro * ro; g.N = C; g.b = c.w<bf16>(w); g.b_ld = Ku; g.bias_n = c.w<float>(b); g.log_rows_per_sample = 2 * logW;
            g.c = c.act(out); g.c_ld = out.ld;
            if (po.valid) { g.gn_part = c.at<float>(po.off); g.gn_quads = po.quads; }
            const int bm = launch_gemm(g, c.stream);
            if (po.valid) c.part_bm[po.id] = bm;
        });
        arena.release(u.off);
        E.taps[m.idx] = out;
    }

    int dense_rows_next = 0;

    struct Fin { int64_t sc = -1, sh = -1, gamma = -1, beta = -1; int C = 0; float out_mul = 1.0f; bool claimed = false, check = false; };
    struct Part { int64_t off = -1; int quads = 0, id = -1, res = 0; bool valid = false; std::shared_ptr<Fin> fin; };
    static void set_fin(GemmArgs& g, const Part& p, const Ctx& c) {
        if (!p.fin || !p.fin->claimed) return;
        const Fin& f = *p.fin;
        g.fin_scale = c.at<float>(f.sc); g.fin_shift = c.at<float>(f.sh); g.fin_gamma = c.w<float>(f.gamma); g.fin_beta = c.w<float>(f.beta);
        g.fin_ld = f.C; g.fin_cg = f.C / 32; g.fin_mul = f.out_mul; g.fin_eps = GN_EPS;
    }
    std::map<std::pair<int64_t, int>, Part> parts;
    int n_parts = 0;
    static bool fusable(int res) { return res >= 16; }
    Part new_part(int res, int C) {
        Part p; p.quads = C / 4; p.res = res; p.id = n_parts++; p.valid = true;
        p.off = arena.alloc((int64_t)std::max(res * res / 64, 1) * p.quads * 8);
        return p;
    }
    Part register_output(const TRef& out, bool fused8 = false) {
        Part p;
        if (fusable(out.res) || (out.res <= 8 && fused8)) p = new_part(out.res, out.C);
        if (p.valid && out.res <= 8 && fused8 && (g_fuse_fin & 1) && out.C == 256) {
            p.fin = std::make_shared<Fin>();
            p.fin->sc = arena.alloc((int64_t)out.C * 4); p.fin->sh = arena.alloc((int64_t)out.C * 4); p.fin->C = out.C;
        }
        if (p.valid && out.res == 16 && fused8 && (g_fuse_fin & 2) && out.C == 256 && !ddpm) {
            p.fin = std::make_shared<Fin>();
            p.fin->sc = arena.alloc((int64_t)out.C * 4); p.fin->sh = arena.alloc((int64_t)out.C * 4); p.fin->C = out.C; p.fin->check = true;
        }
        parts[{out.off, out.coff}] = p;
        return p;
    }
    bool emit_gn_from_parts(const TRef& x, GN gn, int64_t& sc, int64_t& sh, float out_mul) {
        std::vector<Part> src;
        int ch = 0;
        while (ch < x.C) {
            auto it = parts.find({x.off, x.coff + ch});
            if (it == parts.end() || !it->second.valid || it->second.res != x.res) return false;
            src.push_back(it->second);
            ch += it->second.quads * 4;
        }
        if (ch != x.C || src.empty() || src.size() > 2) return false;
        const Part p0 = src[0], p1 = src.size() > 1 ? src[1] : Part();
        const int HW = x.res * x.res, C = x.C;
        if (src.size() == 1 && p0.fin && !p0.fin->claimed && p0.fin->C == C) {
            Fin& f = *p0.fin;
            f.gamma = gn.gamma; f.beta = gn.beta; f.out_mul = out_mul; f.claimed = true;
            sc = f.sc; sh = f.sh;
            if (f.check) {
                const std::shared_ptr<Fin> fp = p0.fin;
                const int64_t fsc = f.sc, fsh = f.sh;
                op(CLS_OTHER, [=](const Ctx& c) {
                    if (c.fin_done[p0.id]) return;
                    hipLaunchKernelGGL(k_gn_finalize, dim3(c.B), dim3(256), 0, c.stream, c.at<float2>(p0.off), HW / c.part_bm[p0.id], p0.quads, (const float2*)nullptr, 0, 0, C, HW,
                                       c.w<float>(gn.gamma), c.w<float>(gn.beta), c.at<float>(fsc), c.at<float>(fsh), GN_EPS, out_mul);
                });
            }
            return true;
        }
        const int64_t sc_ = sc, sh_ = sh;
        op(CLS_OTHER, [=](const Ctx& c) {
            const int tps0 = HW / c.part_bm[p0.id], tps1 = p1.valid ? HW / c.part_bm[p1.id] : 0;
            hipLaunchKernelGGL(k_gn_finalize, dim3(c.B), dim3(256), 0, c.stream, c.at<float2>(p0.off), tps0, p0.quads,
                               p1.valid ? c.at<float2>(p1.off) : (const float2*)nullptr, tps1, p1.valid ? p1.quads : 0, C, HW,
                               c.w<float>(gn.gamma), c.w<float>(gn.beta), c.at<float>(sc_), c.at<float>(sh_), GN_EPS, out_mul);
        });
        return true;
    }

    void list_modules() {
        auto add = [&](int kind, int cin, int cout, int up, int down, int res) {
            Mod m; m.idx = (int)E.mods.size(); m.kind = kind; m.cin = cin; m.cout = cout; m.up = up; m.down = down; m.res = res; m.poff = 0;
            E.mods.push_back(m);
        };
        add(K_LIN, NF, TEMB, 0, 0, 0); add(K_LIN, TEMB, TEMB, 0, 0, 0); add(K_CONV, 3, NF, 0, 0, IMG);
        std::vector<int> skip = {NF};
        int ch = NF, res = IMG;
        for (int l = 0; l < NLEVEL; ++l) {
            for (int b = 0; b < NUM_RES; ++b) {
                add(K_RES, ch, NF * CH_MULT[l], 0, 0, res); ch = NF * CH_MULT[l];
                if (attn_at(res)) add(K_ATTN, ch, ch, 0, 0, res);
                skip.push_back(ch);
            }
            if (l != NLEVEL - 1) { if (ddpm) add(K_DOWN, ch, ch, 0, 0, res); else add(K_RES, ch, ch, 0, 1, res); res /= 2; skip.push_back(ch); }
        }
        add(K_RES, ch, ch, 0, 0, res); add(K_ATTN, ch, ch, 0, 0, res); add(K_RES, ch, ch, 0, 0, res);
        for (int l = NLEVEL - 1; l >= 0; --l) {
            for (int b = 0; b < NUM_RES + 1; ++b) { add(K_RES, ch + skip.back(), NF * CH_MULT[l], 0, 0, res); skip.pop_back(); ch = NF * CH_MULT[l]; }
            if (attn_at(res)) add(K_ATTN, ch, ch, 0, 0, res);
            if (l != 0) { if (ddpm) add(K_UP, ch, ch, 0, 0, res); else add(K_RES, ch, ch, 1, 0, res); res *= 2; }
        }
        add(K_GN, ch, ch, 0, 0, res); add(K_CONV, ch, 3, 0, 0, res);
    }

    void build() {
        list_modules();
        auto& M = E.mods;
        struct Cat { TRef buf; int ch_h, ch_s; };
        std::vector<Cat> cats;
        std::vector<int> skip_ch, skip_res;
        {
            int ch = NF, res = IMG; skip_ch.push_back(NF); skip_res.push_back(IMG);
            for (int l = 0; l < NLEVEL; ++l) {
                for (int b = 0; b < NUM_RES; ++b) { ch = NF * CH_MULT[l]; skip_ch.push_back(ch); skip_res.push_back(res); }
                if (l != NLEVEL - 1) { res /= 2; skip_ch.push_back(ch); skip_res.push_back(res); }
            }
            int sp = (int)skip_ch.size();
            for (int l = NLEVEL - 1; l >= 0; --l) {
                for (int b = 0; b < NUM_RES + 1; ++b) {
                    --sp;
                    Cat c; c.ch_h = ch; c.ch_s = skip_ch[sp];
                    c.buf = new_act(res, c.ch_h + c.ch_s);
                    cats.push_back(c);
                    ch = NF * CH_MULT[l];
                }
                if (l != 0) res *= 2;
            }
        }
        const int P = (int)skip_ch.size();
        auto skip_slot = [&](int i) { const Cat& c = cats[P - 1 - i]; TRef t = c.buf; t.C = c.ch_s; t.coff = c.ch_h; return t; };
        auto h_slot = [&](int j) { const Cat& c = cats[j]; TRef t = c.buf; t.C = c.ch_h; t.coff = 0; return t; };

        for (auto& m : M) if (m.kind == K_RES) dense_total += m.cout;
        dense_w = wres((int64_t)dense_total * TEMB * 2); dense_b = wres((int64_t)dense_total * 4);
        dense_out = arena.alloc((int64_t)dense_total * 4);
        const int64_t emb = arena.alloc(128 * 2), t1 = arena.alloc(TEMB * 2), t2 = arena.alloc(TEMB * 2);

        size_t mi = 0;
        {
            const Mod& m0 = M[mi++]; const Mod& m1 = M[mi++]; (void)m0; (void)m1;
            const int64_t pw0 = take((int64_t)TEMB * NF), pb0 = take(TEMB), pw1 = take((int64_t)TEMB * TEMB), pb1 = take(TEMB);
            const int64_t w0 = wres((int64_t)TEMB * NF * 2), w1 = wres((int64_t)TEMB * TEMB * 2);
            pack_conv(pw0, w0, TEMB, NF, 1, NF, 0, NF); pack_conv(pw1, w1, TEMB, TEMB, 1, TEMB, 0, TEMB);
            const int64_t b0 = pack_f32(pb0, TEMB), b1 = pack_f32(pb1, TEMB);
            const int64_t dw = dense_w, db = dense_b, dout = dense_out; const int dtot = dense_total;
            op(CLS_OTHER, [=](const Ctx& c) {
                hipLaunchKernelGGL(k_time_embed, dim3(grid1d((int64_t)c.B * 128, 256, 1 << 30)), dim3(256), 0, c.stream, c.labels, c.at<bf16>(emb), c.B);
            });
            op(CLS_GEMM, [=](const Ctx& c) {
                GemmArgs g = gemm_defaults();
                g.a0 = c.at<bf16>(emb); g.a0_ld = NF; g.a0_C = NF; g.M = c.B; g.N = TEMB;
                g.b = c.w<bf16>(w0); g.b_ld = NF; g.bias_n = c.w<float>(b0); g.act = ACT_SILU;
                g.c = c.at<bf16>(t1); g.c_ld = TEMB;
                launch_gemm(g, c.stream);
                g = gemm_defaults();
                g.a0 = c.at<bf16>(t1); g.a0_ld = TEMB; g.a0_C = TEMB; g.M = c.B; g.N = TEMB;
                g.b = c.w<bf16>(w1); g.b_ld = TEMB; g.bias_n = c.w<float>(b1); g.act = ACT_SILU;
                g.c = c.at<bf16>(t2); g.c_ld = TEMB;
                launch_gemm(g, c.stream);
                g = gemm_defaults();
                g.a0 = c.at<bf16>(t2); g.a0_ld = TEMB; g.a0_C = TEMB; g.M = c.B; g.N = dtot;
                g.b = c.w<bf16>(dw); g.b_ld = TEMB; g.bias_n = c.w<float>(db);
                g.c = c.at<float>(dout); g.c_ld = dtot; g.c_mode = OUT_F32;
                launch_gemm(g, c.stream);
            });
        }
        int si = 0;
        TRef cur = skip_slot(si++);
        {
            const Mod& m = M[mi++];
            const int64_t pw = take((int64_t)NF * 27), pb = take(NF);
            const int64_t w = wres((int64_t)NF * 64 * 2);
            pack_zero(w, (int64_t)NF * 64);
            pack_conv(pw, w, NF, 3, 9, 64, 0, 3);
            const int64_t b = pack_f32(pb, NF);
            const int64_t a0 = arena.alloc((int64_t)IMG * IMG * 64 * 2);
            const TRef dst = cur;
            const Part po = register_output(dst);
            op(CLS_OTHER, [=](const Ctx& c) {
                const int64_t rows = (int64_t)c.B * IMG * IMG;
                hipLaunchKernelGGL(k_stem_im2col, dim3((unsigned)((rows * 8 + 255) / 256)), dim3(256), 0, c.stream, c.x, c.at<bf16>(a0), rows);
            });
            op(CLS_GEMM, [=](const Ctx& c) {
                const int64_t rows = (int64_t)c.B * IMG * IMG;
                GemmArgs g = gemm_defaults();
                g.a0 = c.at<bf16>(a0); g.a0_ld = 64; g.a0_C = 64; g.M = (int)rows; g.N = NF;
                g.b = c.w<bf16>(w); g.b_ld = 64; g.bias_n = c.w<float>(b);
                g.c = c.act(dst); g.c_ld = dst.ld;
                if (po.valid) { g.gn_part = c.at<float>(po.off); g.gn_quads = po.quads; }
                const int bm = launch_gemm(g, c.stream);
                if (po.valid) c.part_bm[po.id] = bm;
            });
            arena.release(a0);
            E.taps[m.idx] = dst;
        }
        int res = IMG;
        for (int l = 0; l < NLEVEL; ++l) {
            for (int b = 0; b < NUM_RES; ++b) {
                const Mod& m = M[mi++];
                const TRef dst = skip_slot(si++);
                if (attn_at(res)) {
                    TRef tmp = new_act(res, m.cout);
                    emit_res(m, cur, tmp);
                    emit_attn(M[mi++], tmp, dst);
                    arena.release(tmp.off);
                } else {
                    emit_res(m, cur, dst);
                }
                cur = dst;
            }
            if (l != NLEVEL - 1) {
                const Mod& m = M[mi++];
                const TRef dst = skip_slot(si++);
                if (ddpm) emit_downconv(m, cur, dst); else emit_res(m, cur, dst);
                cur = dst; res /= 2;
            }
        }
        {
            TRef a = new_act(res, cur.C), b = new_act(res, cur.C);
            emit_res(M[mi++], cur, a);
            emit_attn(M[mi++], a, b);
            arena.release(a.off);
            emit_res(M[mi++], b, h_slot(0));
            arena.release(b.off);
        }
        int j = 0;
        TRef last;
        for (int l = NLEVEL - 1; l >= 0; --l) {
            for (int b = 0; b < NUM_RES + 1; ++b) {
                const Mod& m = M[mi++];
                const bool level_end = b == NUM_RES;
                TRef in = cats[j].buf;
                TRef dst = level_end ? new_act(res, m.cout) : h_slot(j + 1);
                emit_res(m, in, dst);
                arena.release(cats[j].buf.off);
                last = dst; ++j;
            }
            if (attn_at(res)) {
                TRef dst = new_act(res, last.C);
                emit_attn(M[mi++], last, dst);
                arena.release(last.off);
                last = dst;
            }
            if (l != 0) {
                const Mod& m = M[mi++];
                if (ddpm) emit_upconv(m, last, h_slot(j)); else emit_res(m, last, h_slot(j));
                arena.release(last.off);
                res *= 2;
            }
        }
        {
            const Mod& mg = M[mi++]; const Mod& mc = M[mi++];
            const GN gn = take_gn(mg.cin);
            const int64_t pw = take((int64_t)3 * mc.cin * 9), pb = take(3);
            const int Kf = 9 * mc.cin;
            const int64_t w = wres((int64_t)3 * Kf * 2);
            pack_conv(pw, w, 3, mc.cin, 9, Kf, 0, mc.cin);
            const int64_t b = pack_f32(pb, 3);
            int64_t sc = arena.alloc((int64_t)mg.cin * 4), sh = arena.alloc((int64_t)mg.cin * 4);
            const int logW = ilog2(res), cinf = mc.cin;
            if (g_fuse_head && res == HeadConvCfg::RES && mc.cin == HeadConvCfg::C) {
                const int64_t w16 = wres((int64_t)16 * Kf * 2);
                pack_zero(w16, (int64_t)16 * Kf);
                pack_conv(pw, w16, 3, mc.cin, 9, Kf, 0, mc.cin, -0.6931471805599453f);
                emit_gn_stats(last, gn, sc, sh, -1.4426950408889634f);
                const TRef src = last;
                op(CLS_GEMM, [=](const Ctx& c) {
                    if (g_record) { *g_record += gemm_row(c.B * res * res, 3, Kf, 0, 9, 1, "head_conv", 0) + "\n"; return; }
                    hipLaunchKernelGGL(k_head_conv, dim3((unsigned)(c.B * (HeadConvCfg::RES / HeadConvCfg::ROWS))), dim3(256), HeadConvCfg::LDS_BYTES, c.stream,
                                       c.act(src), src.ld, c.at<float>(sc), c.at<float>(sh), c.w<bf16>(w16), c.w<float>(b), c.out);
                });
            } else {
            emit_gn_stats(last, gn, sc, sh);
            TRef u = new_act(res, mg.cin, 1);
            emit_gn_apply(last, sc, sh, u, nullptr, ACT_SILU, RS_NONE);
            op(CLS_GEMM, [=](const Ctx& c) {
                GemmArgs g = gemm_defaults();
                g.a0 = c.act(u); g.a0_ld = u.ld; g.a0_C = cinf; g.taps = 9; g.logW = logW; g.logHW = 2 * logW; g.a0_padded = 1;
                g.M = c.B * res * res; g.N = 3; g.b = c.w<bf16>(w); g.b_ld = Kf; g.bias_n = c.w<float>(b);
                g.c = c.out; g.c_mode = OUT_F32_NCHW;
                launch_gemm(g, c.stream);
            });
            }
            E.taps[mg.idx] = last;
        }
        finish();
        E.part_bm.assign(n_parts > 0 ? n_parts : 1, 128);
        E.fin_done.assign(n_parts > 0 ? n_parts : 1, 0);
    }
};

int64_t module_param_count(const Mod& m) {
    switch (m.kind) {
        case K_LIN: return (int64_t)m.cout * m.cin + m.cout;
        case K_CONV: return (int64_t)m.cout * m.cin * 9 + m.cout;
        case K_GN: return 2 * (int64_t)m.cin;
        case K_DOWN: case K_UP: return (int64_t)m.cout * m.cin * 9 + m.cout;
        case K_ATTN: return 2 * (int64_t)m.cin + 4 * ((int64_t)m.cin * m.cin + m.cin);
        case K_RES: {
            int64_t n = 2 * (int64_t)m.cin + (int64_t)m.cout * m.cin * 9 + m.cout + (int64_t)m.cout * TEMB + m.cout +
                        2 * (int64_t)m.cout + (int64_t)m.cout * m.cout * 9 + m.cout;
            if (m.cin != m.cout || m.up || m.down) n += (int64_t)m.cout * m.cin + m.cout;
            return n;
        }
    }
    return 0;
}

natinf_ncsnpp* make_engine(int flags) {
    natinf_ncsnpp* e = new natinf_ncsnpp();
    e->flags = flags;
    Builder b(*e);
    b.build();
    int64_t off = 0;
    for (auto& m : e->mods) { m.poff = off; off += module_param_count(m); }
    if (off != e->n_params) { delete e; return nullptr; }
    return e;
}

const natinf_ncsnpp& reference_engine() {
    static natinf_ncsnpp* e = [] {
        int* knobs[] = {&g_fuse_gn, &g_fuse_up, &g_fuse_head, &g_fuse_gn8, &g_fuse_gn4, &g_fuse_fin, &g_attn_qkv, &g_attn_proj};
        int saved[sizeof(knobs) / sizeof(knobs[0])];
        for (size_t i = 0; i < sizeof(knobs) / sizeof(knobs[0]); ++i) { saved[i] = *knobs[i]; *knobs[i] = 1; }
        g_fuse_fin = 3;
        const int saved_fold = g_fuse_up_fold;
        g_fuse_up_fold = 0;
        natinf_ncsnpp* r = make_engine(0);
        g_fuse_up_fold = saved_fold;
        for (size_t i = 0; i < sizeof(knobs) / sizeof(knobs[0]); ++i) *knobs[i] = saved[i];
        return r;
    }();
    return *e;
}

}

extern "C" {

int64_t natinf_ncsnpp_param_count(void) { return reference_engine().n_params; }
int64_t natinf_ncsnpp_packed_bytes(void) { return reference_engine().packed_bytes; }

int64_t natinf_ncsnpp_handle_param_count(natinf_ncsnpp_t h) { return h ? h->n_params : NATINF_EINVAL; }
int64_t natinf_ncsnpp_handle_packed_bytes(natinf_ncsnpp_t h) { return h ? h->packed_bytes : NATINF_EINVAL; }

int64_t natinf_ncsnpp_workspace_bytes(natinf_ncsnpp_t h, int max_batch) {
    if (!h || max_batch <= 0) return NATINF_EINVAL;
    return h->ws_per_image * (int64_t)max_batch;
}

static uint64_t plan_signature() {
    const int k[] = {g_fuse_head, g_attn_qkv, g_attn_w8, g_attn_proj, g_fuse_gn8, g_fuse_fin, g_fuse_gn4, g_fuse_gn, g_cg_wide, g_fuse_up,
                     g_attn_blk , g_fuse_up_fold, g_cg3 };
    uint64_t h = 1469598103934665603ull;
    for (int v : k) h = (h ^ (uint64_t)(v & 0xff)) * 1099511628211ull;
    return h;
}

int natinf_ncsnpp_create(natinf_ncsnpp_t* out, int flags) {
    if (!out || (flags & ~(NATINF_NCSNPP_KEEP_ACTIVATIONS | NATINF_NCSNPP_DDPM))) return NATINF_EINVAL;
    natinf_ncsnpp* e = make_engine(flags);
    if (!e) return NATINF_ESTATE;
    e->plan_sig = plan_signature();
    *out = e;
    return NATINF_OK;
}

int natinf_ncsnpp_destroy(natinf_ncsnpp_t h) {
    if (!h) return NATINF_EINVAL;
    for (auto& r : h->recs) { (void)hipEventDestroy(r.a); (void)hipEventDestroy(r.b); }
    for (auto e : h->pool) (void)hipEventDestroy(e);
    delete h;
    return NATINF_OK;
}

int natinf_ncsnpp_describe(natinf_ncsnpp_t h, char* buf, int cap) {
    if (!h || !buf || cap <= 0) return NATINF_EINVAL;
    std::string s;
    char line[160];
    for (const auto& m : h->mods) {
        snprintf(line, sizeof(line), "%d %s %d %d %d %d %d %lld\n", m.idx, kind_name(m.kind), m.cin, m.cout, m.up, m.down, m.res,
                 (long long)m.poff);
        s += line;
    }
    if ((int)s.size() + 1 > cap) return NATINF_EINVAL;
    memcpy(buf, s.c_str(), s.size() + 1);
    return (int)s.size();
}

int natinf_ncsnpp_load(natinf_ncsnpp_t h, const float* params_f32, int64_t n_params, void* packed, int64_t packed_bytes,
                       natinf_stream_t stream) {
    return h ? h->load(params_f32, n_params, packed, packed_bytes, (hipStream_t)stream) : NATINF_EINVAL;
}

int natinf_ncsnpp_share(natinf_ncsnpp_t h, natinf_ncsnpp_t loaded) {
    if (!h || !loaded || h == loaded) return NATINF_EINVAL;
    if (!loaded->packed) return NATINF_ESTATE;
    if ((h->flags & NATINF_NCSNPP_DDPM) != (loaded->flags & NATINF_NCSNPP_DDPM) || h->n_params != loaded->n_params || h->packed_bytes != loaded->packed_bytes ||
        h->packs.size() != loaded->packs.size() || h->plan_sig != loaded->plan_sig)
        return NATINF_EINVAL;
    h->packed = loaded->packed;
    return NATINF_OK;
}

int natinf_ncsnpp_forward(natinf_ncsnpp_t h, const float* x, const float* labels, float* out, int B, void* workspace,
                          int64_t workspace_bytes, natinf_stream_t stream) {
    if (!h || !x || !labels || !out || !workspace || B <= 0) return NATINF_EINVAL;
    if (!h->packed) return NATINF_ESTATE;
    if (workspace_bytes < h->ws_per_image * (int64_t)B || (int64_t)B * IMG * IMG >= (1LL << 31)) return NATINF_EINVAL;
    if (!h->configured) {
        if (!configure_gemm_kernels()) return NATINF_ENODEV;
        h->configured = true;
    }
    Ctx c{B, reinterpret_cast<unsigned char*>(workspace), h->packed, (hipStream_t)stream, x, labels, out, h->part_bm.data()};
    c.fin_done = h->fin_done.data();
    g_launch_error = 0;
    if (!h->prof) {
        for (const auto& f : h->ops) f(c);
    } else {
        for (size_t i = 0; i < h->ops.size(); ++i) {
            natinf_ncsnpp::Rec r; r.cls = h->op_cls[i];
            for (hipEvent_t* e : {&r.a, &r.b}) {
                if (!h->pool.empty()) { *e = h->pool.back(); h->pool.pop_back(); }
                else if (hipEventCreate(e) != hipSuccess) return NATINF_ELAUNCH;
            }
            (void)hipEventRecord(r.a, c.stream);
            h->ops[i](c);
            (void)hipEventRecord(r.b, c.stream);
            h->recs.push_back(r);
        }
    }
    h->last_B = B; h->last_ws = c.ws;
    if (g_launch_error) { g_launch_error = 0; return NATINF_ESTATE; }
    return hipGetLastError() == hipSuccess ? NATINF_OK : NATINF_ELAUNCH;
}

int natinf_ncsnpp_describe_gemms(natinf_ncsnpp_t h, int B, char* buf, int cap) {
    if (!h || !buf || cap <= 0 || B <= 0) return NATINF_EINVAL;
    std::string out;
    g_record = &out;
    std::vector<int> scratch_bm(h->part_bm.size(), 128);
    std::vector<unsigned char> scratch_done(h->part_bm.size(), 0);
    Ctx c{B, reinterpret_cast<unsigned char*>(4096), reinterpret_cast<const unsigned char*>(4096), nullptr, nullptr, nullptr, nullptr, scratch_bm.data()};
    c.fin_done = scratch_done.data();
    for (size_t i = 0; i < h->ops.size(); ++i)
        if (h->op_cls[i] == CLS_GEMM || h->op_cls[i] == CLS_CONV_GN || h->op_cls[i] == CLS_CONV_GN8) h->ops[i](c);
    g_record = nullptr;
    if ((int)out.size() + 1 > cap) return NATINF_EINVAL;
    memcpy(buf, out.c_str(), out.size() + 1);
    return (int)out.size();
}

int natinf_debug_gemm(int variant, int M, int N, int K0, int K1, int taps, int logW, int batch,
                      const void* a0, const void* a1, const void* b, const float* bias_n, void* c, int c_f32, float scale,
                      int iters, natinf_stream_t stream) {
    if (variant < 0 || variant >= V_COUNT || !a0 || !b || !c || M <= 0 || N <= 0 || K0 <= 0 || K1 < 0 || iters <= 0 || (taps != 1 && taps != 9)) return NATINF_EINVAL;
    if (K0 % taps || N % 8 || (a1 != nullptr) != (K1 > 0)) return NATINF_EINVAL;
    if (taps == 9 && ((K0 / 9) % BK || logW < 1 || logW > 12 || M % (1 << (2 * logW)) || batch != 1)) return NATINF_EINVAL;
    if (!variant_shipped(variant) || variant == V_CONV_GN || variant == V_FP8_256x256) return NATINF_ESTATE;
#ifndef NATINF_DEV
    if (c_f32 >= 2) return NATINF_ESTATE;
#endif
    static bool configured = false;
    if (!configured) { if (!configure_gemm_kernels()) return NATINF_ENODEV; configured = true; }
    GemmArgs g = gemm_defaults();
    g.a0 = (const bf16*)a0; g.a0_C = K0 / taps; g.a0_ld = g.a0_C; g.taps = taps; g.logW = logW; g.logHW = 2 * logW; g.a0_padded = taps == 9;
    if (a1) { g.a1 = (const bf16*)a1; g.a1_C = K1; g.a1_ld = K1; }
    g.M = M; g.N = N; g.b = (const bf16*)b; g.b_ld = K0 + (a1 ? K1 : 0); g.batch = batch;
    if (batch > 1) { g.a_bs = (int64_t)M * g.a0_ld; g.b_bs = (int64_t)N * g.b_ld; g.c_bs = (int64_t)M * N; }
    g.bias_n = bias_n; g.scale = scale; g.c = c; g.c_ld = N; g.c_mode = c_f32 == 1 ? OUT_F32 : (c_f32 >= 2 ? 100 + c_f32 : OUT_BF16);
    g.dbg_ts = g_dbg_ts;
    g.splitk_ws = g_dbg_splitk_ws; g.splitk_max = g_dbg_splitk_max;
    const int saved = g_force_variant;
    g_force_variant = variant;
    g_launch_error = 0;
    for (int i = 0; i < iters; ++i) launch_gemm(g, (hipStream_t)stream);
    g_force_variant = saved;
    if (g_launch_error) { g_launch_error = 0; return NATINF_EINVAL; }
    return hipGetLastError() == hipSuccess ? NATINF_OK : NATINF_ELAUNCH;
}

int g_dbg_conv_logW = 0; const void* g_dbg_conv_a1 = nullptr; int g_dbg_conv_c1 = 0;
int natinf_debug_set_conv_operand(int logW, const void* a1, int c1) {
    if (logW < 0 || logW > 12 || c1 < 0 || c1 % BK || (c1 > 0) != (a1 != nullptr) || (logW == 0 && a1)) return NATINF_EINVAL;
    g_dbg_conv_logW = logW; g_dbg_conv_a1 = a1; g_dbg_conv_c1 = c1;
    return NATINF_OK;
}

int natinf_debug_gemm_fused(int variant, int M, int N, int K, const void* a, const void* b, const float* bias_n, const float* bias_m,
                            const float* rowvec, const float* gate, int log_rows_per_sample, const void* resid_bf16, const float* resid_f32,
                            float scale, int act, void* c, int c_f32, float* gn_part, int* bm_out, int fp32_slab, natinf_stream_t stream) {
    const int logW = g_dbg_conv_logW, c1 = g_dbg_conv_c1;
    const void* a1 = g_dbg_conv_a1;
    g_dbg_conv_logW = 0; g_dbg_conv_a1 = nullptr; g_dbg_conv_c1 = 0;
    if (variant < 0 || variant >= V_COUNT || !a || !b || !c || M <= 0 || N <= 0 || K <= 0 || c_f32 < 0 || c_f32 > 2) return NATINF_EINVAL;
    if (c_f32 == 2) {
        if (!logW || bias_m || rowvec || gate || resid_bf16 || resid_f32 || gn_part || act != ACT_NONE) return NATINF_EINVAL;
    } else if (N % 8) return NATINF_EINVAL;
    if (logW && (K % 9 || (K / 9) % BK || M % (1 << (2 * logW)))) return NATINF_EINVAL;
    if (!variant_shipped(variant) || variant == V_CONV_GN || variant == V_FP8_256x256) return NATINF_ESTATE;
    if (!configure_gemm_kernels()) return NATINF_ENODEV;
    GemmArgs g = gemm_defaults();
    g.a0 = (const bf16*)a; g.a0_C = K; g.a0_ld = K; g.M = M; g.N = N; g.b = (const bf16*)b; g.b_ld = K;
    if (logW) {
        g.taps = 9; g.a0_C = g.a0_ld = K / 9; g.logW = logW; g.logHW = 2 * logW; g.a0_padded = 1; g.b_ld = K + c1;
        if (a1) { g.a1 = (const bf16*)a1; g.a1_C = g.a1_ld = c1; }
    }
    g.bias_n = bias_n; g.bias_m = bias_m; g.rowvec = rowvec; g.rowvec_ld = N; g.gate = gate; g.gate_ld = N; g.log_rows_per_sample = log_rows_per_sample;
    g.resid = (const bf16*)resid_bf16; g.resid_ld = N; g.resid_f32 = resid_f32; g.resid_f32_ld = N;
    g.scale = scale; g.act = act; g.c = c; g.c_ld = N; g.c_mode = c_f32 == 2 ? OUT_F32_NCHW : (c_f32 ? OUT_F32 : OUT_BF16);
    g.gn_part = gn_part; g.gn_quads = N / 4; g.epi_fp32_slab = fp32_slab != 0;
    g.splitk_ws = g_dbg_splitk_ws; g.splitk_max = g_dbg_splitk_max;
    g.dbg_ts = g_dbg_ts;
    const int saved = g_force_variant;
    g_force_variant = variant;
    g_launch_error = 0;
    const int bm = launch_gemm(g, (hipStream_t)stream);
    g_force_variant = saved;
    if (bm_out) *bm_out = bm;
    if (g_launch_error) { g_launch_error = 0; return NATINF_EINVAL; }
    return hipGetLastError() == hipSuccess ? NATINF_OK : NATINF_ELAUNCH;
}

int g_dbg_cg_up = 0;
int natinf_debug_conv_gn_up(int flags) { if (flags & ~3) return NATINF_EINVAL; g_dbg_cg_up = flags; return NATINF_OK; }
float* g_dbg_fin_scale = nullptr; float* g_dbg_fin_shift = nullptr; const float* g_dbg_fin_gamma = nullptr; const float* g_dbg_fin_beta = nullptr;
int g_dbg_fin_cg = 0; float g_dbg_fin_mul = 1.0f;
int natinf_debug_conv_gn_fin(float* fin_scale, float* fin_shift, const float* gamma, const float* beta, int channels_per_group, float mul) {
    if (fin_scale && (!fin_shift || !gamma || !beta || channels_per_group < 4 || channels_per_group % 4)) return NATINF_EINVAL;
    g_dbg_fin_scale = fin_scale; g_dbg_fin_shift = fin_shift; g_dbg_fin_gamma = gamma; g_dbg_fin_beta = beta; g_dbg_fin_cg = channels_per_group; g_dbg_fin_mul = mul;
    return NATINF_OK;
}
int natinf_debug_conv_gn(int res, int B, int N, int cin, int c1, const void* x, const float* scale, const float* shift, const void* w_packed,
                         void* w_frag, const void* a1, const float* bias_n, const void* resid, float out_scale, void* out, float* gn_part, int iters,
                         natinf_stream_t stream) {
    if ((res != 32 && res != 16 && res != 8 && res != 4) || B <= 0 || N <= 0 || N % 8 || cin <= 0 || cin % 64 || c1 < 0 || c1 % 64 || (c1 > 0) != (a1 != nullptr) ||
        !x || !scale || !shift || !w_packed || !out || iters <= 0) return NATINF_EINVAL;
    static bool configured = false;
    if (!configured) { if (!configure_gemm_kernels()) return NATINF_ENODEV; configured = true; }
    GemmArgs g = gemm_defaults();
    g.a0 = (const bf16*)x; g.a0_ld = cin; g.a0_C = cin; g.taps = 9; g.logW = ilog2(res); g.logHW = 2 * g.logW;
    g.gn_scale = scale; g.gn_shift = shift; g.gn_ld = cin; g.gn_folded = 1;
    if (a1) { g.a1 = (const bf16*)a1; g.a1_ld = c1; g.a1_C = c1; }
    g.M = B * res * res; g.N = N; g.b = (const bf16*)w_packed; g.b_ld = 9 * cin + c1; g.bias_n = bias_n;
    g.resid = (const bf16*)resid; g.resid_ld = N; g.scale = out_scale; g.c = out; g.c_ld = N;
    g.gn_part = gn_part; g.gn_quads = N / 4;
    if (g_dbg_fin_scale) {
        if (!gn_part || N != 256 || res > 16 || N % g_dbg_fin_cg) return NATINF_EINVAL;
        g.fin_scale = g_dbg_fin_scale; g.fin_shift = g_dbg_fin_shift; g.fin_gamma = g_dbg_fin_gamma; g.fin_beta = g_dbg_fin_beta;
        g.fin_ld = N; g.fin_cg = g_dbg_fin_cg; g.fin_mul = g_dbg_fin_mul; g.fin_eps = GN_EPS;
    }
    g.dbg_ts = g_dbg_ts;
    g.a0_up = g_dbg_cg_up & 1; g.a1_up = (a1 && (g_dbg_cg_up & 2)) ? 1 : 0;
    if (w_frag && N % 16 == 0) g.b_frag = (const bf16*)w_frag;
    if (!conv_gn_ok(g)) return NATINF_EINVAL;
    if (g.b_frag) {
        const int64_t n = (int64_t)(N / 16) * (9 * (cin / 32) + c1 / 32) * 64;
        hipLaunchKernelGGL(k_pack_frag, dim3(grid1d(n, 256, 1 << 30)), dim3(256), 0, (hipStream_t)stream, (const bf16*)w_packed, (bf16*)w_frag, N, g.b_ld, cin, c1);
    }
    for (int i = 0; i < iters; ++i) launch_gemm(g, (hipStream_t)stream);
    return hipGetLastError() == hipSuccess ? NATINF_OK : NATINF_ELAUNCH;
}

int natinf_debug_fold_up_weights(const float* w, int N, int cin, float w_mul, float* out_f32, void* out_packed, natinf_stream_t stream) {
    if (!w || N <= 0 || cin <= 0 || (!out_f32 && !out_packed) || (out_packed && cin % 64)) return NATINF_EINVAL;
    ncsn_upf::fold(w, out_packed, out_f32, N, cin, w_mul, stream);
    return hipGetLastError() == hipSuccess ? NATINF_OK : NATINF_ELAUNCH;
}
int natinf_debug_conv_up_fold(int B, int N, int cin, const void* x, const float* scale, const float* shift, const float* w, void* w_packed, void* h_scratch,
                              const float* bias_n, const float* rowvec, float out_scale, void* out, float* gn_part, int iters, natinf_stream_t stream) {
    if (B <= 0 || N != UPFOLD_BN || cin <= 0 || cin % 64 || !x || !scale || !shift || !w || !w_packed || !h_scratch || !out || iters <= 0) return NATINF_EINVAL;
    static bool configured = false;
    if (!configured) { if (!configure_gemm_kernels()) return NATINF_ENODEV; configured = true; }
    hipStream_t s = (hipStream_t)stream;
    constexpr int W = UPFOLD_W, logW = 4;
    ncsn_upf::fold(w, w_packed, nullptr, N, cin, 1.0f, stream);
    hipLaunchKernelGGL(k_gn_apply, dim3((unsigned)((W + 2 + GN_ROWS - 1) / GN_ROWS), (unsigned)B), dim3(256), 0, s, (const bf16*)x, cin, cin, logW, 2 * logW, scale, shift,
                       (bf16*)h_scratch, (bf16*)nullptr, ACT_SILU, RS_NONE, 1);
    GemmArgs g = gemm_defaults();
    g.a0 = (const bf16*)h_scratch; g.a0_ld = cin; g.a0_padded = 1; g.a0_C = cin; g.taps = 4; g.logW = logW; g.logHW = 2 * logW;
    g.M = B * W * W; g.N = 4 * N; g.b = (const bf16*)w_packed; g.b_ld = 4 * cin; g.bias_n = bias_n;
    g.rowvec = rowvec; g.rowvec_ld = N; g.log_rows_per_sample = 2 * logW; g.scale = out_scale;
    g.c = out; g.c_ld = N; g.gn_part = gn_part; g.gn_quads = N / 4;
    if (!up_fold_epi(g)) return NATINF_EINVAL;
    g_launch_error = 0;
    for (int i = 0; i < iters; ++i) launch_gemm(g, s);
    if (g_launch_error) { g_launch_error = 0; return NATINF_EINVAL; }
    return hipGetLastError() == hipSuccess ? NATINF_OK : NATINF_ELAUNCH;
}

int natinf_debug_attn_block(int plan, int B, const void* x, int x_ld, const float* scale, const float* shift, const float* w, const float* bias,
                            void* packed, void* scratch, void* out, int o_ld, float out_scale, float* gn_part, natinf_stream_t stream) {
    if (plan < 0 || plan > 2 || B < 1 || !x || !scale || !shift || !w || !bias || !packed || !out || x_ld < 256 || x_ld % 8 || o_ld < 256 || o_ld % 8 ||
        (plan != 2 && !scratch)) return NATINF_EINVAL;
    static bool configured = false;
    if (!configured) { if (!configure_gemm_kernels()) return NATINF_ENODEV; configured = true; }
    constexpr int64_t WW = 256 * 256;
    unsigned char* pk = reinterpret_cast<unsigned char*>(packed);
    hipStream_t s = (hipStream_t)stream;
    AttnBlk256 a;
    a.plan = plan; a.B = B; a.x = (const bf16*)x; a.x_ld = x_ld; a.sc = scale; a.sh = shift;
    a.out = (bf16*)out; a.o_ld = o_ld; a.out_scale = out_scale; a.gn_part = reinterpret_cast<float2*>(gn_part); a.gn_quads = 64;
    if (plan == 2) {
        float* fq = reinterpret_cast<float*>(pk + NATINF_ATTN_BLOCK_OFF_FOLD_WQK); float* fv = reinterpret_cast<float*>(pk + NATINF_ATTN_BLOCK_OFF_FOLD_WVO);
        float* cq = reinterpret_cast<float*>(pk + NATINF_ATTN_BLOCK_OFF_FOLD_CQ); float* bo = reinterpret_cast<float*>(pk + NATINF_ATTN_BLOCK_OFF_FOLD_BO);
        bf16* wqf2 = reinterpret_cast<bf16*>(pk + NATINF_ATTN_BLOCK_OFF_WQK_PACKED); bf16* wvof2 = reinterpret_cast<bf16*>(pk + NATINF_ATTN_BLOCK_OFF_WVO_PACKED);
        pack_attn_fold(w, w + WW, w + 2 * WW, w + 3 * WW, bias, bias + 512, bias + 768, fq, cq, fv, bo, wqf2, wvof2, s);
        a.wqf2 = wqf2; a.cq2 = cq; a.wvof2 = wvof2; a.bo2 = bo;
    } else {
        bf16* wqkvf = reinterpret_cast<bf16*>(pk + NATINF_ATTN_BLOCK_OFF_WQKV); bf16* w3f = reinterpret_cast<bf16*>(pk + NATINF_ATTN_BLOCK_OFF_W3);
        pack_attn_qkv_w(w, w + WW, w + 2 * WW, wqkvf, s);
        pack_attn_w3(w + 3 * WW, w3f, s);
        a.wqkvf = wqkvf; a.bqk = bias; a.bv = bias + 512; a.w3f = w3f; a.b3 = bias + 768;
        a.qk = reinterpret_cast<bf16*>(scratch); a.vT = a.qk + (int64_t)B * 256 * 512;
        if (plan == 0) launch_attn_qkv256(a, s);
    }
    launch_attn_blk256(a, s);
    return hipGetLastError() == hipSuccess ? NATINF_OK : NATINF_ELAUNCH;
}

int natinf_debug_quant_fp8_rows(const float* w, void* q, float* row_scale, int rows, int cols, natinf_stream_t stream) {
    if (!w || !q || !row_scale || rows <= 0 || cols <= 0 || cols % 2) return NATINF_EINVAL;
    hipLaunchKernelGGL(k_pack_fp8_rows, dim3((unsigned)((rows + 3) / 4)), dim3(256), 0, (hipStream_t)stream, w, (uint8_t*)q, row_scale, rows, cols);
    return hipGetLastError() == hipSuccess ? NATINF_OK : NATINF_ELAUNCH;
}

int natinf_debug_gemm_fp8(int M, int N, int K, const void* a8, const float* a_scale, const void* a_mx, const void* b8, const float* b_scale,
                          const float* bias_n, void* c, void* c_mx, int c_mode, int iters, natinf_stream_t stream) {
    if (!a8 || !b8 || !c || M <= 0 || N <= 0 || K <= 0 || K % 128 || N % 8 || iters <= 0) return NATINF_EINVAL;
    static bool configured = false;
    if (!configured) { if (!configure_gemm_kernels()) return NATINF_ENODEV; configured = true; }
    GemmArgs g = gemm_defaults();
    g.a0 = (const bf16*)a8; g.a0_C = K; g.a0_ld = K; g.M = M; g.N = N; g.b = (const bf16*)b8; g.b_ld = K;
    const int act = c_mode >> 8; c_mode &= 0xff;
    if (act != ACT_NONE && act != ACT_GELU_TANH) return NATINF_EINVAL;
    g.deq_m = a_scale; g.deq_n = b_scale; g.bias_n = bias_n; g.c = c; g.c_ld = N; g.c_mode = c_mode; g.act = act;
    g.a_mx = (const uint8_t*)a_mx; g.a_mx_ld = M; g.c_mx = (uint8_t*)c_mx; g.c_mx_ld = M;
    if ((c_mode == OUT_FP8_MX && (!c_mx || N % 32)) || c_mode < 0 || c_mode > OUT_FP8_MX || c_mode == OUT_F32_NCHW) return NATINF_EINVAL;
    for (int i = 0; i < iters; ++i) launch_gemm_fp8(g, (hipStream_t)stream);
    return hipGetLastError() == hipSuccess ? NATINF_OK : NATINF_ELAUNCH;
}

int natinf_debug_timestamps(void* dev_buf16) {
#ifdef NATINF_DEV
    g_dbg_ts = reinterpret_cast<unsigned long long*>(dev_buf16); return NATINF_OK;
#else
    (void)dev_buf16; return NATINF_ESTATE;
#endif
}

int natinf_set_gemm_raster(int rows) { g_raster_g = rows; return NATINF_OK; }
int natinf_set_fuse_gn(int on) { g_fuse_gn = on != 0; return NATINF_OK; }
int natinf_set_fuse_gn8(int on) { g_fuse_gn8 = on != 0; return NATINF_OK; }
int natinf_set_attn256(int on) { return on ? NATINF_OK : NATINF_ESTATE; }
int natinf_set_conv_gn_warm(int mask) { if (mask < 0 || mask > 15) return NATINF_EINVAL; g_cg_warm = mask; return NATINF_OK; }
int natinf_set_attn_block(int on) { g_attn_blk = on < 0 ? ATTN_BLK_DEFAULT : (on > 2 ? 2 : on); return NATINF_OK; }
int natinf_set_attn_qkv(int on) { g_attn_qkv = on != 0; return NATINF_OK; }
int natinf_set_attn_waves8(int on) { g_attn_w8 = on != 0; return NATINF_OK; }
int natinf_set_attn_proj(int on) { g_attn_proj = on != 0; return NATINF_OK; }
int natinf_set_fuse_fin(int on) {
    if (on < 0 || on > 3) return NATINF_EINVAL;
    static const int mask[4] = {0, 3, 1, 2};
    g_fuse_fin = mask[on];
    return NATINF_OK;
}
int natinf_set_gemm_round_model(int on) { g_round_model = on != 0; g_round_model_w128 = on >= 10 ? on : 13; return NATINF_OK; }
int natinf_set_gemm_w128(int on) { g_w128 = on < 0 ? 0 : (on > 2 ? 2 : on); return NATINF_OK; }
int natinf_set_fuse_gn4(int on) { g_fuse_gn4 = on != 0; return NATINF_OK; }
int natinf_set_conv_gn8_tile(int one_image) { return one_image ? NATINF_OK : NATINF_ESTATE; }
int natinf_set_fuse_head(int on) { g_fuse_head = on != 0; return NATINF_OK; }
int natinf_set_conv_gn_w128(int mask) { if (mask < 0 || mask > 7) return NATINF_EINVAL; g_cg3 = mask; return NATINF_OK; }
int natinf_set_conv_gn_w128_min_k(int shape, int k) { if (shape < 0 || shape > 2 || k < 0) return NATINF_EINVAL; g_cg3_min_k[shape] = k; return NATINF_OK; }
int natinf_set_conv_gn_wide(int mask) { if (mask < 0 || mask > 3) return NATINF_EINVAL; g_cg_wide = mask; return NATINF_OK; }
int natinf_set_conv_gn_regw(int on) { return on ? NATINF_OK : NATINF_ESTATE; }
int natinf_set_fuse_up(int on) { g_fuse_up = on != 0; return NATINF_OK; }
int natinf_set_fuse_up_fold(int on) { g_fuse_up_fold = on < 0 ? UP_FOLD_DEFAULT : on != 0; return NATINF_OK; }
int natinf_set_gemm_splitk(int on) { g_splitk = on != 0; return NATINF_OK; }
int natinf_debug_set_splitk_workspace(float* ws, int max_slices) { g_dbg_splitk_ws = ws; g_dbg_splitk_max = ws ? max_slices : 0; return NATINF_OK; }
int natinf_set_gemm_half_issue(int on) { return on ? NATINF_OK : NATINF_ESTATE; }
int natinf_set_gemm_pref512(int on) { g_pref_512 = on != 0; return NATINF_OK; }
int natinf_set_gemm_epilogue(int fp32_slab) { g_epi_fp32_slab = fp32_slab != 0; return NATINF_OK; }

int natinf_set_gemm_variant(int variant) {
    if (variant < 0 || variant >= V_COUNT) return NATINF_EINVAL;
    if (!variant_shipped(variant) || variant == V_CONV_GN || variant == V_FP8_256x256) return NATINF_ESTATE;
    g_force_variant = variant;
    return NATINF_OK;
}

int natinf_gemm_profile(int enable) { g_gemm_prof.on = enable != 0; return NATINF_OK; }
int natinf_gemm_profile_read(char* buf, int cap) {
    if (!buf || cap <= 0) return NATINF_EINVAL;
    std::map<std::string, std::pair<double, int64_t>> by;
    std::vector<std::string> order;
    int rc = NATINF_OK;
    for (auto& e : g_gemm_prof.ev) {
        float ms = 0.f;
        if (hipEventSynchronize(e.b) != hipSuccess || hipEventElapsedTime(&ms, e.a, e.b) != hipSuccess) { (void)hipGetLastError(); rc = NATINF_ELAUNCH; }
        else {
            auto it = by.find(e.tag);
            if (it == by.end()) { order.push_back(e.tag); it = by.emplace(e.tag, std::make_pair(0.0, (int64_t)0)).first; }
            it->second.first += ms; it->second.second += 1;
        }
        g_gemm_prof.pool.emplace_back(e.a, e.b);
    }
    g_gemm_prof.ev.clear();
    if (rc != NATINF_OK) return rc;
    std::string out;
    for (auto& t : order) {
        char tail[64];
        snprintf(tail, sizeof(tail), " %lld %.6f\n", (long long)by[t].second, by[t].first);
        out += t + tail;
    }
    if ((int)out.size() + 1 > cap) return NATINF_EINVAL;
    memcpy(buf, out.c_str(), out.size() + 1);
    return (int)out.size();
}
int natinf_ncsnpp_profile(natinf_ncsnpp_t h, int enable) {
    if (!h) return NATINF_EINVAL;
    h->prof = enable != 0;
    return NATINF_OK;
}

int natinf_ncsnpp_profile_read(natinf_ncsnpp_t h, double* ms_by_class, int64_t* launches_by_class) {
    if (!h || !ms_by_class || !launches_by_class) return NATINF_EINVAL;
    for (int i = 0; i < N_CLS; ++i) { ms_by_class[i] = 0.0; launches_by_class[i] = 0; }
    for (const auto& r : h->recs) {
        float ms = 0.f;
        if (hipEventSynchronize(r.b) != hipSuccess || hipEventElapsedTime(&ms, r.a, r.b) != hipSuccess) {
            (void)hipGetLastError();
            return NATINF_ELAUNCH;
        }
        ms_by_class[r.cls] += ms; launches_by_class[r.cls] += 1;
        h->pool.push_back(r.a); h->pool.push_back(r.b);
    }
    h->recs.clear();
    return NATINF_OK;
}

int natinf_ncsnpp_debug_tap(natinf_ncsnpp_t h, int module_idx, float* out, int64_t capacity_elems, natinf_stream_t stream) {
    if (!h || !out) return NATINF_EINVAL;
    if (!(h->flags & NATINF_NCSNPP_KEEP_ACTIVATIONS) || !h->last_ws) return NATINF_ESTATE;
    auto it = h->taps.find(module_idx);
    if (it == h->taps.end()) return NATINF_EINVAL;
    const TRef& t = it->second;
    const int HW = t.res * t.res;
    const int64_t total = (int64_t)h->last_B * t.C * HW;
    if (capacity_elems < total) return NATINF_EINVAL;
    const bf16* src = reinterpret_cast<const bf16*>(h->last_ws + t.off * h->last_B) + t.coff;
    hipLaunchKernelGGL(k_nhwc_to_nchw_f32, dim3(grid1d(total, 256, 1 << 30)), dim3(256), 0, (hipStream_t)stream, src, t.ld, t.C, HW, out, total);
    return hipGetLastError() == hipSuccess ? NATINF_OK : NATINF_ELAUNCH;
}

static bool dbg_misaligned(const void* p, uintptr_t a) { return reinterpret_cast<uintptr_t>(p) % a != 0; }

int natinf_debug_gn_stats(const void* x, int ld, int C, int HW, int B, const float* gamma, const float* beta, float* scale, float* shift, float eps, float out_mul,
                          natinf_stream_t stream) {
    if (!x || !gamma || !beta || !scale || !shift || B < 1 || HW < 1 || C < 32 || C > 512 || C % 32 || ld < C || ld % 8 || dbg_misaligned(x, 16)) return NATINF_EINVAL;
    if ((256 / (C >> 3)) * C > 16 * 128 + 64) return NATINF_EINVAL;
    hipLaunchKernelGGL(k_gn_stats, dim3((unsigned)B), dim3(256), 0, (hipStream_t)stream, (const bf16*)x, ld, C, HW, gamma, beta, scale, shift, eps, out_mul);
    return hipGetLastError() == hipSuccess ? NATINF_OK : NATINF_ELAUNCH;
}

int natinf_debug_gn_finalize(const float* P0, int tps0, int quads0, const float* P1, int tps1, int quads1, int C, int HW, int B, const float* gamma, const float* beta,
                             float* scale, float* shift, float eps, float out_mul, natinf_stream_t stream) {
    if (!P0 || !gamma || !beta || !scale || !shift || B < 1 || HW < 1 || tps0 < 1 || quads0 < 1) return NATINF_EINVAL;
    if (P1 ? (tps1 < 1 || quads1 < 1) : (tps1 != 0 || quads1 != 0)) return NATINF_EINVAL;
    if (C < 128 || C > 512 || C % 128 || quads0 + quads1 > 128 || (quads0 + quads1) * 4 != C || dbg_misaligned(P0, 8) || dbg_misaligned(P1, 8)) return NATINF_EINVAL;
    hipLaunchKernelGGL(k_gn_finalize, dim3((unsigned)B), dim3(256), 0, (hipStream_t)stream, reinterpret_cast<const float2*>(P0), tps0, quads0,
                       reinterpret_cast<const float2*>(P1), tps1, quads1, C, HW, gamma, beta, scale, shift, eps, out_mul);
    return hipGetLastError() == hipSuccess ? NATINF_OK : NATINF_ELAUNCH;
}

int natinf_debug_gn_apply(const void* x, int ld, int C, int logW, int logHW, int B, const float* scale, const float* shift, void* y, void* xr, int act, int mode, int pad,
                          natinf_stream_t stream) {
    if (!x || !scale || !shift || !y || B < 1 || B > 65535 || C < 8 || C % 8 || (C >> 3) > 256 || ld < C || ld % 8) return NATINF_EINVAL;
    if (logW < 0 || logHW < logW || logHW > 24 || mode < RS_NONE || mode > RS_DOWN || (pad != 0 && pad != 1) || (act != ACT_NONE && act != ACT_SILU)) return NATINF_EINVAL;
    if (mode == RS_DOWN && (logW < 1 || logHW - logW < 1)) return NATINF_EINVAL;
    if (dbg_misaligned(x, 16) || dbg_misaligned(y, 16) || dbg_misaligned(xr, 16) || dbg_misaligned(scale, 16) || dbg_misaligned(shift, 16)) return NATINF_EINVAL;
    const int Hs = 1 << (logHW - logW), Hd = mode == RS_UP ? 2 * Hs : (mode == RS_DOWN ? Hs / 2 : Hs);
    const int rows_per_img = Hd + 2 * pad;
    hipLaunchKernelGGL(k_gn_apply, dim3((unsigned)((rows_per_img + GN_ROWS - 1) / GN_ROWS), (unsigned)B), dim3(256), 0, (hipStream_t)stream, (const bf16*)x, ld, C,
                       logW, logHW, scale, shift, (bf16*)y, (bf16*)xr, act, mode, pad);
    return hipGetLastError() == hipSuccess ? NATINF_OK : NATINF_ELAUNCH;
}

int natinf_debug_head_conv(const void* x, int ld, int B, const float* scale, const float* shift, const void* w16, const float* bias, float* out, natinf_stream_t stream) {
    if (!x || !scale || !shift || !w16 || !bias || !out || B < 1 || ld < HeadConvCfg::C || ld % 8) return NATINF_EINVAL;
    if (dbg_misaligned(x, 16) || dbg_misaligned(w16, 16) || dbg_misaligned(out, 16)) return NATINF_EINVAL;
    if (hipFuncSetAttribute(reinterpret_cast<const void*>(&k_head_conv), hipFuncAttributeMaxDynamicSharedMemorySize, HeadConvCfg::LDS_BYTES) != hipSuccess) {
        (void)hipGetLastError();
        return NATINF_ENODEV;
    }
    hipLaunchKernelGGL(k_head_conv, dim3((unsigned)(B * (HeadConvCfg::RES / HeadConvCfg::ROWS))), dim3(256), HeadConvCfg::LDS_BYTES, (hipStream_t)stream,
                       (const bf16*)x, ld, scale, shift, (const bf16*)w16, bias, out);
    return hipGetLastError() == hipSuccess ? NATINF_OK : NATINF_ELAUNCH;
}

int natinf_debug_time_embed(const float* labels, void* emb, int B, natinf_stream_t stream) {
    if (!labels || !emb || B < 1 || B >= (1 << 21)) return NATINF_EINVAL;
    hipLaunchKernelGGL(k_time_embed, dim3(grid1d((int64_t)B * 128, 256, 1 << 30)), dim3(256), 0, (hipStream_t)stream, labels, (bf16*)emb, B);
    return hipGetLastError() == hipSuccess ? NATINF_OK : NATINF_ELAUNCH;
}

int natinf_debug_stem_im2col(const float* x, void* A, int B, natinf_stream_t stream) {
    if (!x || !A || B < 1 || B > (1 << 17) || dbg_misaligned(A, 16)) return NATINF_EINVAL;
    const int64_t rows = (int64_t)B * 1024;
    hipLaunchKernelGGL(k_stem_im2col, dim3((unsigned)((rows * 8 + 255) / 256)), dim3(256), 0, (hipStream_t)stream, x, (bf16*)A, rows);
    return hipGetLastError() == hipSuccess ? NATINF_OK : NATINF_ELAUNCH;
}

int natinf_debug_pack_conv(const float* src, void* dst, int N, int Cin, int taps, int dst_ld, int koff, int tap_stride_c, int chunked, float wmul, natinf_stream_t stream) {
    if (!src || !dst || N < 1 || Cin < 1 || taps < 1 || koff < 0 || (chunked != 0 && chunked != 1)) return NATINF_EINVAL;
    const int64_t n = (int64_t)N * Cin * taps;
    const int64_t span = chunked ? (int64_t)((Cin + 63) / 64) * taps * 64 : (int64_t)(taps - 1) * tap_stride_c + Cin;
    if ((!chunked && tap_stride_c < Cin) || koff + span > dst_ld || n > ((int64_t)1 << 30) * 256) return NATINF_EINVAL;
    hipLaunchKernelGGL(k_pack_conv, dim3(grid1d(n, 256, 1 << 30)), dim3(256), 0, (hipStream_t)stream, src, (bf16*)dst, N, Cin, taps, dst_ld, koff, tap_stride_c, chunked, wmul);
    return hipGetLastError() == hipSuccess ? NATINF_OK : NATINF_ELAUNCH;
}

int natinf_debug_pack_transpose(const float* src, void* dst, int K, int N, int dst_ld, natinf_stream_t stream) {
    if (!src || !dst || K < 1 || N < 1 || dst_ld < K) return NATINF_EINVAL;
    hipLaunchKernelGGL(k_pack_transpose, dim3(grid1d((int64_t)K * N, 256, 1 << 30)), dim3(256), 0, (hipStream_t)stream, src, (bf16*)dst, K, N, dst_ld);
    return hipGetLastError() == hipSuccess ? NATINF_OK : NATINF_ELAUNCH;
}

int natinf_debug_nhwc_to_nchw(const void* x, int ld, int C, int HW, int B, float* out, natinf_stream_t stream) {
    if (!x || !out || B < 1 || C < 1 || HW < 1 || ld < C) return NATINF_EINVAL;
    const int64_t total = (int64_t)B * C * HW;
    if (total > ((int64_t)1 << 30) * 256) return NATINF_EINVAL;
    hipLaunchKernelGGL(k_nhwc_to_nchw_f32, dim3(grid1d(total, 256, 1 << 30)), dim3(256), 0, (hipStream_t)stream, (const bf16*)x, ld, C, HW, out, total);
    return hipGetLastError() == hipSuccess ? NATINF_OK : NATINF_ELAUNCH;
}

}
#include "dit_engine.inc"
#include "mmdit_engine.inc"
#include "vae_engine.inc"
#include "inception_engine.inc"
```

naturaldiffusion_amd/ncsnpp.py:

```python
from __future__ import annotations

import ctypes as C
from typing import Dict, List, Tuple

import torch

from . import _lib
from ._lib import lib, check, ptr, stream_ptr

KEEP_ACTIVATIONS = 1
DDPM = 2
ARCH_FLAGS = {"ncsnpp": 0, "ddpm": DDPM}


def module_table(handle=None, arch: str = "ncsnpp") -> List[Tuple[int, str, int, int, int, int, int, int]]:
    own = handle is None
    if own:
        h = C.c_void_p()
        check(lib.natinf_ncsnpp_create(C.byref(h), ARCH_FLAGS[arch]), "natinf_ncsnpp_create")
        handle = h
    buf = C.create_string_buffer(1 << 14)
    n = lib.natinf_ncsnpp_describe(handle, buf, len(buf))
    if n < 0:
        check(n, "natinf_ncsnpp_describe")
    if own:
        lib.natinf_ncsnpp_destroy(handle)
    rows = []
    for line in buf.value.decode().strip().split("\n"):
        f = line.split()
        rows.append((int(f[0]), f[1], *map(int, f[2:])))
    return rows


def param_layout(nf: int = 128, arch: str = "ncsnpp") -> List[Tuple[str, Tuple[int, ...]]]:
    out: List[Tuple[str, Tuple[int, ...]]] = []
    sc = lambda c: c if c == 3 else c * nf // 128
    TEMB = 4 * nf
    for idx, kind, cin, cout, up, down, res, _ in module_table(arch=arch):
        cin, cout = sc(cin), sc(cout)
        p = f"all_modules.{idx}."
        if kind == "lin":
            out += [(p + "weight", (cout, cin)), (p + "bias", (cout,))]
        elif kind == "conv":
            out += [(p + "weight", (cout, cin, 3, 3)), (p + "bias", (cout,))]
        elif kind == "gn":
            out += [(p + "weight", (cin,)), (p + "bias", (cin,))]
        elif kind == "attn":
            out += [(p + "GroupNorm_0.weight", (cin,)), (p + "GroupNorm_0.bias", (cin,))]
            for i in range(4):
                out += [(p + f"NIN_{i}.W", (cin, cin)), (p + f"NIN_{i}.b", (cin,))]
        elif kind == "res":
            out += [(p + "GroupNorm_0.weight", (cin,)), (p + "GroupNorm_0.bias", (cin,)),
                    (p + "Conv_0.weight", (cout, cin, 3, 3)), (p + "Conv_0.bias", (cout,)),
                    (p + "Dense_0.weight", (cout, TEMB)), (p + "Dense_0.bias", (cout,)),
                    (p + "GroupNorm_1.weight", (cout,)), (p + "GroupNorm_1.bias", (cout,)),
                    (p + "Conv_1.weight", (cout, cout, 3, 3)), (p + "Conv_1.bias", (cout,))]
            if arch == "ddpm":
                if cin != cout:
                    out += [(p + "NIN_0.W", (cin, cout)), (p + "NIN_0.b", (cout,))]
            elif cin != cout or up or down:
                out += [(p + "Conv_2.weight", (cout, cin, 1, 1)), (p + "Conv_2.bias", (cout,))]
        elif kind in ("down", "up"):
            out += [(p + "Conv_0.weight", (cout, cin, 3, 3)), (p + "Conv_0.bias", (cout,))]
        else:
            raise RuntimeError(f"unknown module kind {kind}")
    return out


def flatten_state_dict(sd: Dict[str, torch.Tensor], arch: str = "ncsnpp") -> torch.Tensor:
    sd = {(k[7:] if k.startswith("module.") else k): v for k, v in sd.items()}
    parts = []
    for name, shape in param_layout(arch=arch):
        if name not in sd:
            raise KeyError(f"checkpoint lacks {name}")
        t = sd[name]
        if tuple(t.shape) != tuple(shape):
            raise ValueError(f"{name}: shape {tuple(t.shape)} != expected {shape}")
        parts.append(t.detach().to("cpu", torch.float32).reshape(-1))
    return torch.cat(parts)


def flatten_ema(shadow_params: List[torch.Tensor], nf: int = 128, arch: str = "ncsnpp") -> torch.Tensor:
    layout = param_layout(nf, arch)
    if len(shadow_params) != len(layout):
        raise ValueError(f"EMA list has {len(shadow_params)} tensors, the model has {len(layout)} parameters")
    parts = []
    for (name, shape), t in zip(layout, shadow_params):
        if tuple(t.shape) != tuple(shape):
            raise ValueError(f"EMA entry for {name}: shape {tuple(t.shape)} != expected {shape}")
        parts.append(t.detach().to("cpu", torch.float32).reshape(-1))
    return torch.cat(parts)


def load_score_sde_checkpoint(path: str, nf: int = 128, arch: str = "ncsnpp") -> torch.Tensor:
    state = torch.load(path, map_location="cpu", weights_only=False)
    for key in ("model", "ema", "step"):
        if key not in state:
            raise KeyError(f"{path}: not a score_sde checkpoint (no '{key}' entry; utils.py:22-29)")
    shadow = list(state["ema"]["shadow_params"])
    model_sd = {(k[7:] if k.startswith("module.") else k): v for k, v in state["model"].items()}
    for (name, shape), t in zip(param_layout(nf, arch), shadow):
        if name in model_sd and tuple(model_sd[name].shape) != tuple(t.shape):
            raise ValueError(f"{path}: EMA entry for {name} has shape {tuple(t.shape)}, the model's is {tuple(model_sd[name].shape)}")
    return flatten_ema(shadow, nf, arch)


class NCSNppEngine:
    def __init__(self, flat_params: torch.Tensor, max_batch: int, device="cuda:0", keep_activations: bool = False, arch: str = "ncsnpp"):
        _lib.require_gpu()
        self.device = torch.device(device)
        self.max_batch = int(max_batch)
        self.arch = arch
        self._h = C.c_void_p()
        self._flags = (KEEP_ACTIVATIONS if keep_activations else 0) | ARCH_FLAGS[arch]
        check(lib.natinf_ncsnpp_create(C.byref(self._h), self._flags), "natinf_ncsnpp_create")
        n = lib.natinf_ncsnpp_handle_param_count(self._h)
        if flat_params.numel() != n:
            raise ValueError(f"expected {n} parameters, got {flat_params.numel()}")
        with torch.cuda.device(self.device):
            params = flat_params.to(self.device, torch.float32).contiguous()
            self._packed = torch.empty(lib.natinf_ncsnpp_handle_packed_bytes(self._h), dtype=torch.uint8, device=self.device)
            check(lib.natinf_ncsnpp_load(self._h, ptr(params), n, ptr(self._packed), self._packed.numel(), stream_ptr()),
                  "natinf_ncsnpp_load")
            torch.cuda.current_stream().synchronize()
            ws = lib.natinf_ncsnpp_workspace_bytes(self._h, self.max_batch)
            self._ws = torch.empty(ws, dtype=torch.uint8, device=self.device)
        self.workspace_bytes = ws

    def clone(self, max_batch: int = None) -> "NCSNppEngine":
        other = object.__new__(NCSNppEngine)
        other.device, other.arch = self.device, self.arch
        other.max_batch = int(max_batch or self.max_batch)
        other._h = C.c_void_p()
        check(lib.natinf_ncsnpp_create(C.byref(other._h), self._flags), "natinf_ncsnpp_create")
        check(lib.natinf_ncsnpp_share(other._h, self._h), "natinf_ncsnpp_share")
        other._flags = self._flags
        other._packed = self._packed
        with torch.cuda.device(self.device):
            ws = lib.natinf_ncsnpp_workspace_bytes(other._h, other.max_batch)
            other._ws = torch.empty(ws, dtype=torch.uint8, device=self.device)
        other.workspace_bytes = ws
        return other

    def __call__(self, x: torch.Tensor, labels: torch.Tensor, out: torch.Tensor = None) -> torch.Tensor:
        if x.dtype != torch.float32 or x.dim() != 4 or tuple(x.shape[1:]) != (3, 32, 32) or not x.is_cuda:
            raise ValueError("x must be a CUDA fp32 tensor of shape [B,3,32,32]")
        B = x.shape[0]
        if B > self.max_batch:
            raise ValueError(f"batch {B} exceeds max_batch {self.max_batch}")
        x = x.contiguous()
        labels = labels.to(x.device, torch.float32).contiguous()
        if labels.numel() != B:
            raise ValueError("labels must have one entry per sample")
        if out is None:
            out = torch.empty_like(x)
        check(lib.natinf_ncsnpp_forward(self._h, ptr(x), ptr(labels), ptr(out), B, ptr(self._ws), self._ws.numel(),
                                        stream_ptr()), "natinf_ncsnpp_forward")
        return out

    def profile(self, enable: bool) -> None:
        check(lib.natinf_ncsnpp_profile(self._h, 1 if enable else 0), "natinf_ncsnpp_profile")

    def profile_read(self):
        ms = (C.c_double * 4)()
        n = (C.c_int64 * 4)()
        check(lib.natinf_ncsnpp_profile_read(self._h, ms, n), "natinf_ncsnpp_profile_read")
        return {"gemm": (ms[0], n[0]), "other": (ms[1], n[1]), "conv_gn": (ms[2], n[2]), "conv_gn8": (ms[3], n[3])}

    def describe_gemms(self, B: int):
        buf = C.create_string_buffer(1 << 16)
        n = lib.natinf_ncsnpp_describe_gemms(self._h, B, buf, len(buf))
        if n < 0:
            check(n, "natinf_ncsnpp_describe_gemms")
        rows = []
        for line in buf.value.decode().strip().split("\n"):
            f = line.split()
            rows.append((*map(int, f[:6]), f[6]))
        return rows

    def tap(self, module_idx: int, shape) -> torch.Tensor:
        out = torch.empty(shape, dtype=torch.float32, device=self.device)
        check(lib.natinf_ncsnpp_debug_tap(self._h, module_idx, ptr(out), out.numel(), stream_ptr()), "natinf_ncsnpp_debug_tap")
        return out

    def __del__(self):
        h = getattr(self, "_h", None)
        if h:
            lib.natinf_ncsnpp_destroy(h)
            self._h = None
```

naturaldiffusion_amd/sampler.py:

```python
from __future__ import annotations

import math
from typing import Callable, Optional

import numpy as np
import torch

from . import _lib
from ._lib import lib, check, ptr, stream_ptr
from .coeff import SparseRows, is_stochastic


def vp_std_f32(t: float, beta_0: float = 0.1, beta_1: float = 20.0) -> float:
    vt = torch.ones(1, dtype=torch.float32) * t
    lmc = -0.25 * vt ** 2 * (beta_1 - beta_0) - 0.5 * vt * beta_0
    return float(torch.sqrt(1.0 - torch.exp(2.0 * lmc))[0])


def image_index_args(index, n_images: int, device):
    if index is None:
        return None, 0, 1
    if isinstance(index, torch.Tensor):
        if (index.dtype != torch.int64 or index.device != device or not index.is_contiguous()
                or index.numel() != n_images):
# ... 364 lines not shown
            if seed is None:
                raise ValueError("stochastic NI matrix (B[k, j >= 1] != 0): the injected noise needs a seed")
            if self.fast:
                raise ValueError("stochastic NI matrix: fast_f32 mode only covers column 0 of B")
            _check_elems_per_image(elems_per_image, self.E)
            self.rows_b = SparseRows(self.B, lambda k: min(k + 2, self.B.shape[1]), torch.float32, self.device,
                                     diag=False, dense=dense)
        self.seed = None if seed is None else int(seed) & (2 ** 64 - 1)
        self.epi = None if elems_per_image is None else int(elems_per_image)
        hdt = torch.float32 if self.fast else torch.float64
        self.rows = SparseRows(self.C, lambda k: k + 1, hdt, self.device, dense=dense)
        self.hist = torch.empty((self.n_step, self.E), dtype=hdt, device=self.device)
        self._x = [torch.empty(self.E, dtype=torch.float32, device=self.device) for _ in range(2)]
        self.std = [vp_std_f32(self.node[k, 0]) for k in range(self.n_step)] if stds is None else [float(v) for v in stds]
        self.labels = [float(np.float32(self.node[k, 0]) * np.float32(999)) for k in range(self.n_step)]
        self._rows_b0 = None
        self._known_level = _level_memo(lambda known_final: known_schedule(self.node, known_final))
        self._color_level = _level_memo(lambda known_final: color_schedule(self.node, known_final))

    def _noise_rows(self) -> SparseRows:
        if self.stochastic:
            return self.rows_b
        if self._rows_b0 is None:
            self._rows_b0 = SparseRows(self.B[:, :1], lambda k: 1, torch.float32, self.device, diag=False, dense=True)
        return self._rows_b0

    def first_input(self, noise: torch.Tensor, known: Optional[torch.Tensor] = None, mask: Optional[torch.Tensor] = None, index=None,
                    elems_per_image: Optional[int] = None, known_final: str = "mean", *, gray_u: Optional[torch.Tensor] = None) -> torch.Tensor:
        epi = self.epi if elems_per_image is None else int(elems_per_image)
        noise = _flat_noise_f32(noise, self.E)
        if gray_u is not None:
            if known is not None or mask is not None:
                raise ValueError("gray_u (colorization) does not go with known / mask (inpainting)")
            gs = check_gray(gray_u, self.E, epi, seed=self.seed, fast_f32=self.fast, device=noise.device)
            ga, gstd, gcol = self._color_level(0, known_final)
            index, first, stride = image_index_args(index, self.E // epi, noise.device)
            out = torch.empty_like(noise)
            check(lib.natinf_color_blend_f32(ptr(noise), ptr(out), ptr(gray_u), gs, _f9(COLOR_M), _f9(COLOR_W), ga, gstd, gcol, self.seed,
                                             ptr(index), first, stride, epi, self.E, stream_ptr()), "natinf_color_blend_f32")
            return out
        return _known_blend_f32(noise, known, mask, self.E, epi, self.seed, self._known_level, known_final, index, fast_f32=self.fast)

    def step(self, k: int, x_k: torch.Tensor, model_out: torch.Tensor, noise: torch.Tensor,
             x_next: Optional[torch.Tensor] = None, index=None, elems_per_image: Optional[int] = None, *,
             known: Optional[torch.Tensor] = None, mask: Optional[torch.Tensor] = None, known_final: str = "mean",
             gray_u: Optional[torch.Tensor] = None, low: Optional[torch.Tensor] = None) -> torch.Tensor:
        epi = self.epi if elems_per_image is None else int(elems_per_image)
        inpaint = known is not None or mask is not None
        if self.sr_scale:
            check_project(self.sr_scale, self.image_shape, seed=self.seed, elems_per_image=epi, conditioned=inpaint or gray_u is not None)
            _check_elems_per_image(epi, self.E)
            if low is None:
                raise ValueError("a sampler made with sr_scale needs low= at every step")
            ls = check_low(low, self.E, epi, self.sr_scale, device=x_k.device)
        elif low is not None:
            raise ValueError("low= belongs to a sampler made with sr_scale")
        if self.x0_mode:
            check_x0_fix(self.x0_fix, self.x0_ratio, self.x0_max, seed=self.seed, elems_per_image=epi, gray=gray_u is not None)
            _check_elems_per_image(epi, self.E)
        if gray_u is not None:
            if inpaint:
                raise ValueError("gray_u (colorization) does not go with known / mask (inpainting)")
            gs = check_gray(gray_u, self.E, epi, seed=self.seed, fast_f32=self.fast, device=x_k.device)
            ga, gstd, gcol = self._color_level(k + 1, known_final)
        if inpaint:
            ks, ms = check_known(known, mask, self.E, epi, seed=self.seed, fast_f32=self.fast, device=x_k.device)
            ka, kstd, kcol = self._known_level(k + 1, known_final)
        if x_next is None:
            x_next = _pingpong(self._x, k, x_k)
        for t in (x_k, model_out, noise):
            if t.dtype != torch.float32 or t.numel() != self.E or not t.is_contiguous():
                raise ValueError("x_k / model_out / noise must be contiguous fp32 tensors of n_elem elements")
        idx, val, n = self.rows.ptrs(k)
        r = self.rows.rows[k]
        a, s = float(self.node[k, 1]), float(self.node[k, 2])
        if inpaint or gray_u is not None or self.stochastic or self.x0_mode or self.sr_scale:
            if epi is None:
                raise ValueError("stochastic NI matrix: elems_per_image is needed to key the injected noise")
            ib, vb, nb = self._noise_rows().ptrs(k)
            index, first, stride = image_index_args(index, self.E // epi, x_k.device)
        if self.sr_scale:
            n_images = self.E // epi
            if self.sr_r is None or self.sr_r.shape[1] != n_images:
                self.sr_r = torch.zeros((self.n_step, n_images), dtype=torch.float64, device=self.device)
            c, h, w = self.image_shape
            check(lib.natinf_step_f64hist_project(ptr(x_k), ptr(model_out), ptr(noise), ptr(self.hist), ptr(x_next), idx, val, n,
                                                  r.diag, ib, vb, nb, k, a, s, self.std[k], self.seed, ptr(index), first, stride,
                                                  epi, self.E, ptr(low), ls, c, h, w, self.sr_scale, ptr(self.sr_r[k]), stream_ptr()),
                  "natinf_step_f64hist_project")
            return x_next
        if self.x0_mode:
            n_images = self.E // epi
            if self.x0_s is None or self.x0_s.shape[1] != n_images:
                self.x0_s = torch.zeros((self.n_step, n_images), dtype=torch.float64, device=self.device)
            kargs = (ptr(known), ptr(mask), ks, ms, ka, kstd, kcol) if inpaint else (0, 0, 0, 0, 0.0, 0.0, 0)
            check(lib.natinf_step_f64hist_x0fix(ptr(x_k), ptr(model_out), ptr(noise), ptr(self.hist), ptr(x_next), idx, val, n,
                                                r.diag, ib, vb, nb, k, a, s, self.std[k], self.seed, ptr(index), first, stride,
                                                epi, self.E, *kargs, self.x0_mode, self.x0_ratio, self.x0_max, ptr(self.x0_s[k]),
                                                stream_ptr()), "natinf_step_f64hist_x0fix")
            return x_next
        if inpaint:
            check(lib.natinf_step_f64hist_inpaint(ptr(x_k), ptr(model_out), ptr(noise), ptr(self.hist), ptr(x_next), idx, val, n,
                                                  r.diag, ib, vb, nb, k, a, s, self.std[k], self.seed, ptr(index), first, stride,
                                                  epi, self.E, ptr(known), ptr(mask), ks, ms, ka, kstd, kcol, stream_ptr()),
                  "natinf_step_f64hist_inpaint")
            return x_next
        if gray_u is not None:
            check(lib.natinf_step_f64hist_colorize(ptr(x_k), ptr(model_out), ptr(noise), ptr(self.hist), ptr(x_next), idx, val, n,
                                                   r.diag, ib, vb, nb, k, a, s, self.std[k], self.seed, ptr(index), first, stride,
                                                   epi, self.E, ptr(gray_u), gs, _f9(COLOR_M), _f9(COLOR_W), ga, gstd, gcol, stream_ptr()),
                  "natinf_step_f64hist_colorize")
            return x_next
        if self.stochastic:
            check(lib.natinf_step_f64hist_noise(ptr(x_k), ptr(model_out), ptr(noise), ptr(self.hist), ptr(x_next), idx, val, n,
                                                r.diag, ib, vb, nb, k, a, s, self.std[k], self.seed, ptr(index), first, stride,
                                                epi, self.E, stream_ptr()), "natinf_step_f64hist_noise")
            return x_next
        b0 = float(np.float32(self.B[k, 0]))
        fn = lib.natinf_step_f32hist if self.fast else lib.natinf_step_f64hist
        check(fn(ptr(x_k), ptr(model_out), ptr(noise), ptr(self.hist), ptr(x_next), idx, val, n, r.diag, k,
                 a, s, self.std[k], b0, self.E, stream_ptr()), "natinf_step_f64hist")
        return x_next

    def run(self, model_fn: Callable, noise: torch.Tensor, return_all: bool = False, index=None, *,
            known: Optional[torch.Tensor] = None, mask: Optional[torch.Tensor] = None, known_final: str = "mean",
            gray_u: Optional[torch.Tensor] = None, low: Optional[torch.Tensor] = None, sr_final: str = "step"):
        shape, B = noise.shape, noise.shape[0]
        noise = noise.contiguous()
        epi = self.epi if self.epi is not None else noise.numel() // B
        inpaint = known is not None or mask is not None
        if sr_final not in ("step", "x0"):
            raise ValueError('sr_final must be "step" or "x0"')
        if self.sr_scale:
            check_project(self.sr_scale, self.image_shape, seed=self.seed, elems_per_image=epi, conditioned=inpaint or gray_u is not None)
            if low is None:
                raise ValueError("a sampler made with sr_scale needs low=")
        elif low is not None or sr_final != "step":
            raise ValueError('low= and sr_final="x0" belong to a sampler made with sr_scale')
        if gray_u is not None and inpaint:
            raise ValueError("gray_u (colorization) does not go with known / mask (inpainting)")
        if self.x0_mode:
            check_x0_fix(self.x0_fix, self.x0_ratio, self.x0_max, seed=self.seed, elems_per_image=epi, gray=gray_u is not None)
        kw = dict(index=index, elems_per_image=epi) if self.stochastic or inpaint or gray_u is not None or self.x0_mode or self.sr_scale else {}
        if self.sr_scale:
            kw.update(low=low.reshape(-1))
        if gray_u is not None:
            kw.update(gray_u=gray_u.reshape(-1), known_final=known_final)
        elif inpaint:
            flat = lambda t: t if t is None else (t.view(torch.uint8) if t.dtype == torch.bool else t).reshape(-1)
            kw.update(known=flat(known), mask=flat(mask), known_final=known_final)
        x = self.first_input(noise, **kw) if inpaint or gray_u is not None else noise
        xs = [x.view(shape)]
        for k in range(self.n_step):
            labels = torch.full((B,), self.labels[k], dtype=torch.float32, device=self.device)
            out = model_fn(x.view(shape), labels)
            x = self.step(k, x.reshape(-1), out.contiguous().reshape(-1), noise.reshape(-1), **kw)
            if return_all:
                x = x.clone()
                xs.append(x.view(shape))
        if sr_final == "x0":
            x = self.hist[self.n_step - 1].to(torch.float32)
            xs.append(x.view(shape))
        return xs if return_all else x.view(shape)


class ValidateNI:

    def __init__(self, C: np.ndarray, B: np.ndarray, node: np.ndarray, c1: np.ndarray, c2: np.ndarray, n_elem: int,
                 device="cuda:0", dense: bool = False, *, seed: Optional[int] = None, elems_per_image: Optional[int] = None):
        _lib.require_gpu()
        if n_elem % 4:
            raise ValueError("element count must be a multiple of 4")
        self.n_step = int(np.asarray(B).shape[0])
        self.node = np.asarray(node, np.float64)
        self.E = int(n_elem)
        self.device = torch.device(device)
        self.seed = None if seed is None else int(seed) & (2 ** 64 - 1)
        if elems_per_image is not None:
            if seed is None:
                raise ValueError("elems_per_image belongs to the seeded (in-kernel noise) form: give a seed")
            _check_elems_per_image(elems_per_image, self.E)
        self.epi = None if elems_per_image is None else int(elems_per_image)
        self.rows_c = SparseRows(C, lambda k: k + 1, torch.float32, self.device, dense=dense)
        self.rows_b = SparseRows(B, lambda k: min(k + 2, np.asarray(B).shape[1]), torch.float32, self.device, dense=dense, diag=False)
        self.c1 = [float(np.float32(v)) for v in c1]
        self.c2 = [float(np.float32(v)) for v in c2]
        self.hist_x0 = torch.empty((self.n_step, self.E), dtype=torch.float32, device=self.device)
        self.hist_eps = None if self.seed is not None else torch.empty((self.n_step + 1, self.E), dtype=torch.float32, device=self.device)
        self._z = [torch.empty(self.E, dtype=torch.float32, device=self.device) for _ in range(2)]
        self._known_level = _level_memo(lambda known_final: known_schedule(self.node, known_final))
        self._launch_wide = {}

    def _launch_wide_guidance(self, n: int, cfg: float, have_uncond: bool):
        key = (n, float(cfg), bool(have_uncond))
        if key not in self._launch_wide:
            slots = torch.arange(n, dtype=torch.int32) if have_uncond else torch.full((n,), -1, dtype=torch.int32)
            self._launch_wide[key] = (torch.full((n,), float(cfg), dtype=torch.float32).to(self.device), slots.to(self.device))
        return self._launch_wide[key]

    def first_input(self, noise: torch.Tensor, known: torch.Tensor, mask: torch.Tensor, index=None, known_final: str = "mean",
                    elems_per_image: Optional[int] = None) -> torch.Tensor:
        epi = self.epi if elems_per_image is None else int(elems_per_image)
        return _known_blend_f32(_flat_noise_f32(noise, self.E), known, mask, self.E, epi, self.seed, self._known_level, known_final, index)

    def step(self, k: int, z: torch.Tensor, cond: torch.Tensor, uncond: Optional[torch.Tensor], cfg,
             sample_elems: Optional[int] = None, eps_sample_stride: Optional[int] = None, *,
             noise: Optional[torch.Tensor] = None, index=None, uncond_slot: Optional[torch.Tensor] = None,
             n_uncond: Optional[int] = None, known: Optional[torch.Tensor] = None, mask: Optional[torch.Tensor] = None,
             known_final: str = "mean") -> torch.Tensor:
        se = self.E if sample_elems is None else int(sample_elems)
        st = se if eps_sample_stride is None else int(eps_sample_stride)
        guided = isinstance(cfg, torch.Tensor)
        inpaint = known is not None or mask is not None
        if inpaint:
            if self.seed is None:
                raise ValueError("known / mask belong to the seeded form: the slab form has no blend")
            ks, ms = check_known(known, mask, self.E, se, seed=self.seed, device=z.device)
            ka, kstd, kcol = self._known_level(k + 1, known_final)
        if guided and (self.seed is None or noise is None):
            raise ValueError("a tensor cfg (per-image scales) belongs to the seeded form with noise= / index=: the slab form takes one float")
        if not guided and (uncond_slot is not None or n_uncond is not None):
            raise ValueError("uncond_slot / n_uncond go with a tensor cfg (per-image scales)")
        z_next = _pingpong(self._z, k, z)
        ic, vc, nc = self.rows_c.ptrs(k)
        ib, vb, nb = self.rows_b.ptrs(k)
        if self.seed is None:
            if noise is not None or index is not None:
                raise ValueError("noise / index belong to the seeded form; without a seed the noises are read from hist_eps")
            check(lib.natinf_step_f32prod(ptr(z), ptr(cond), ptr(uncond), float(cfg), se, st, ptr(self.hist_x0),
                                          ptr(self.hist_eps), ptr(z_next), ic, vc, nc, self.rows_c.rows[k].diag,
                                          ib, vb, nb, k, self.c1[k], self.c2[k], self.E, stream_ptr()), "natinf_step_f32prod")
            return z_next
        if noise is None:
            raise ValueError("seeded form: step needs the initial noise (noise=); there is no hist_eps slab to read it from")
        if noise.dtype != torch.float32 or noise.numel() != self.E or not noise.is_contiguous() or noise.device != z.device:
            raise ValueError("noise must be a contiguous fp32 tensor of n_elem elements on the sampler's device")
        if se <= 0 or se % 4 or self.E % se or (self.epi is not None and se != self.epi):
            raise ValueError("sample_elems must be the per-image element count: a multiple of 4 dividing the element count"
                             + ("" if self.epi is None else f" (elems_per_image = {self.epi})"))
        index, first, stride = image_index_args(index, self.E // se, z.device)
        if inpaint and not guided:
            cfg, uncond_slot = self._launch_wide_guidance(self.E // se, float(cfg), uncond is not None)
            n_uncond = self.E // se if uncond is not None else 0
        if guided or inpaint:
            _check_guidance_tensors(cfg, uncond_slot, self.E // se, z.device)
            if n_uncond is None:
                n_uncond = 0 if uncond is None else uncond.numel() // st
            if inpaint:
                check(lib.natinf_step_f32prod_inpaint(ptr(z), ptr(cond), ptr(uncond), ptr(cfg), ptr(uncond_slot), int(n_uncond), se, st,
                                                      ptr(self.hist_x0), ptr(noise), ptr(z_next), ic, vc, nc, self.rows_c.rows[k].diag,
                                                      ib, vb, nb, k, self.c1[k], self.c2[k], self.seed, ptr(index), first, stride,
                                                      self.E, ptr(known), ptr(mask), ks, ms, ka, kstd, kcol, stream_ptr()),
                      "natinf_step_f32prod_inpaint")
                return z_next
            check(lib.natinf_step_f32prod_noise_guided(ptr(z), ptr(cond), ptr(uncond), ptr(cfg), ptr(uncond_slot), int(n_uncond), se, st,
                                                       ptr(self.hist_x0), ptr(noise), ptr(z_next), ic, vc, nc, self.rows_c.rows[k].diag,
                                                       ib, vb, nb, k, self.c1[k], self.c2[k], self.seed, ptr(index), first, stride,
                                                       self.E, stream_ptr()), "natinf_step_f32prod_noise_guided")
            return z_next
        check(lib.natinf_step_f32prod_noise(ptr(z), ptr(cond), ptr(uncond), float(cfg), se, st, ptr(self.hist_x0), ptr(noise),
                                            ptr(z_next), ic, vc, nc, self.rows_c.rows[k].diag, ib, vb, nb, k, self.c1[k],
                                            self.c2[k], self.seed, ptr(index), first, stride, self.E, stream_ptr()),
              "natinf_step_f32prod_noise")
        return z_next


class SD3NI:

    def __init__(self, weights: np.ndarray, sigmas: torch.Tensor, n_elem: int, device="cuda:0", cfg: float = 7.0,
                 dense: bool = False, euler: bool = False, elems_per_image: Optional[int] = None):
        _lib.require_gpu()
        if n_elem % 8:
            raise ValueError("element count must be a multiple of 8")
        self.E = int(n_elem)
        self.epi = None if elems_per_image is None else int(elems_per_image)
        _check_elems_per_image(self.epi, self.E, 8)
        self.device = torch.device(device)
        self.cfg = float(cfg)
        self.euler = bool(euler)
        sig = sigmas.detach().to("cpu", torch.float32)
        h = lambda t: float(t.to(torch.float16))
        if euler:
            n = sig.numel() - 1
            w32 = [-1 * (sig[i + 1] - sig[i]) for i in range(n)]
            W = np.zeros((n, n))
            tot = []
            for k in range(n):
                acc = 0
                for j in range(k + 1):
                    W[k, j] = h(w32[j])
                    acc = acc + w32[j]
                tot.append(float(acc))
            self.rows = SparseRows(W, lambda k: k + 1, torch.float32, self.device, dense=dense)
            self.totals = tot
        else:
            W = np.asarray(weights, np.float64)
            n = W.shape[0]
            self.rows = SparseRows(W, lambda k: k + 1, torch.float32, self.device, dense=dense)
            self.totals = [r.total for r in self.rows.rows]
        self.n_step = n
        self.sig = [h(sig[k]) for k in range(n + 1)]
        self.oms = [h(1 - sig[k]) for k in range(n + 1)]
        self.hist = torch.empty((n, self.E), dtype=torch.float16, device=self.device)
        self._x = [torch.empty(self.E, dtype=torch.float16, device=self.device) for _ in range(2)]
        self.mean = torch.empty(self.E, dtype=torch.float16, device=self.device)
        self._known_level = _level_memo(lambda renoise: sd_known_schedule(self.sig, self.oms, renoise))

    def _sample_elems(self, sample_elems: Optional[int]) -> int:
# ... 74 lines not shown
```

Before: 3546 images/s.

## Cache time-embedding rows per timestep and fuse stem im2col into conv GEMM

Adds a forward_t entry point taking a scalar timestep. The time-embedding dense output is computed once per distinct t and kept in an LRU slot cache with event synchronisation across streams, and later convs read one broadcast row (rowvec_ld=0). A new stem kernel builds the 3x3x3 patches straight into LDS and runs MFMA, which removes the separate im2col launch and its global buffer round trip. The sampler also stops allocating a labels tensor every step. The cache adds cross-stream event waits and carries results across calls, keyed on t and B.

```diff
diff --git a/include/natinf_ncsnpp.h b/include/natinf_ncsnpp.h
--- a/include/natinf_ncsnpp.h
+++ b/include/natinf_ncsnpp.h
@@ -31,6 +31,10 @@
 
 int natinf_ncsnpp_forward(natinf_ncsnpp_t h, const float* x, const float* labels, float* out, int B,
                           void* workspace, int64_t workspace_bytes, natinf_stream_t stream);
+
+int natinf_ncsnpp_forward_t(natinf_ncsnpp_t h, const float* x, float t, float* out, int B, void* workspace, int64_t workspace_bytes, natinf_stream_t stream);
+int natinf_set_temb_cache(int slots);
+int natinf_ncsnpp_temb_cache_stats(natinf_ncsnpp_t h, int64_t* hits, int64_t* misses);
 
 int natinf_ncsnpp_describe_gemms(natinf_ncsnpp_t h, int B, char* buf, int cap);
 
@@ -112,6 +116,9 @@
 int natinf_debug_head_conv(const void* x, int ld, int B, const float* scale, const float* shift, const void* w16, const float* bias, float* out, natinf_stream_t stream);
 int natinf_debug_time_embed(const float* labels, void* emb, int B, natinf_stream_t stream);
 int natinf_debug_stem_im2col(const float* x, void* A, int B, natinf_stream_t stream);
+int natinf_set_fuse_stem(int on);
+int natinf_debug_stem_conv(const float* x, const void* w_packed, const float* bias, void* out, float* gn_part, int B, natinf_stream_t stream);
+int natinf_debug_set_gemm_sample_rows(int log_rows);
 int natinf_debug_pack_conv(const float* src, void* dst, int N, int Cin, int taps, int dst_ld, int koff, int tap_stride_c, int chunked, float wmul, natinf_stream_t stream);
 int natinf_debug_pack_transpose(const float* src, void* dst, int K, int N, int dst_ld, natinf_stream_t stream);
 int natinf_debug_nhwc_to_nchw(const void* x, int ld, int C, int HW, int B, float* out, natinf_stream_t stream);
diff --git a/naturaldiffusion_amd/_lib.py b/naturaldiffusion_amd/_lib.py
--- a/naturaldiffusion_amd/_lib.py
+++ b/naturaldiffusion_amd/_lib.py
@@ -74,6 +74,9 @@
     "natinf_ncsnpp_load": (C.c_int, [_p, _p, _i64, _p, _i64, _p]),
     "natinf_ncsnpp_share": (C.c_int, [_p, _p]),
     "natinf_ncsnpp_forward": (C.c_int, [_p, _p, _p, _p, _i32, _p, _i64, _p]),
+    "natinf_ncsnpp_forward_t": (C.c_int, [_p, _p, _f32, _p, _i32, _p, _i64, _p]),
+    "natinf_set_temb_cache": (C.c_int, [_i32]),
+    "natinf_ncsnpp_temb_cache_stats": (C.c_int, [_p, C.POINTER(C.c_int64), C.POINTER(C.c_int64)]),
     "natinf_ncsnpp_debug_tap": (C.c_int, [_p, _i32, _p, _i64, _p]),
     "natinf_ncsnpp_describe_gemms": (C.c_int, [_p, _i32, C.c_char_p, _i32]),
     "natinf_debug_gemm": (C.c_int, [_i32, _i32, _i32, _i32, _i32, _i32, _i32, _i32, _p, _p, _p, _p, _p, _i32, _f32, _i32, _p]),
@@ -120,6 +123,9 @@
     "natinf_debug_head_conv": (C.c_int, [_p, _i32, _i32, _p, _p, _p, _p, _p, _p]),
     "natinf_debug_time_embed": (C.c_int, [_p, _p, _i32, _p]),
     "natinf_debug_stem_im2col": (C.c_int, [_p, _p, _i32, _p]),
+    "natinf_set_fuse_stem": (C.c_int, [_i32]),
+    "natinf_debug_stem_conv": (C.c_int, [_p, _p, _p, _p, _p, _i32, _p]),
+    "natinf_debug_set_gemm_sample_rows": (C.c_int, [_i32]),
     "natinf_debug_pack_conv": (C.c_int, [_p, _p, _i32, _i32, _i32, _i32, _i32, _i32, _i32, _f32, _p]),
     "natinf_debug_pack_transpose": (C.c_int, [_p, _p, _i32, _i32, _i32, _p]),
     "natinf_debug_nhwc_to_nchw": (C.c_int, [_p, _i32, _i32, _i32, _i32, _p, _p]),
diff --git a/naturaldiffusion_amd/csrc/engine_core.h b/naturaldiffusion_amd/csrc/engine_core.h
--- a/naturaldiffusion_amd/csrc/engine_core.h
+++ b/naturaldiffusion_amd/csrc/engine_core.h
@@ -31,6 +31,7 @@
     hipStream_t stream2 = nullptr; hipEvent_t* ev = nullptr;
     unsigned char* fin_done = nullptr;
     uint32_t* guard = nullptr;
+    const float* temb_row = nullptr;
     uint32_t* site(int i) const { return guard ? guard + 2 * i : nullptr; }
     bf16* act(const TRef& t) const { return reinterpret_cast<bf16*>(ws + t.off * B) + t.coff; }
     template <class T> T* at(int64_t off) const { return reinterpret_cast<T*>(ws + off * B); }
diff --git a/naturaldiffusion_amd/csrc/gemm_launch.h b/naturaldiffusion_amd/csrc/gemm_launch.h
--- a/naturaldiffusion_amd/csrc/gemm_launch.h
+++ b/naturaldiffusion_amd/csrc/gemm_launch.h
@@ -24,6 +24,7 @@
                     void launch_fp8(const void* gemm_args, int mxa, int w128, int raster, void* stream); void launch_splitk_reduce(const void* gemm_args, int slices, void* stream);
                     void launch_patch_embed(const float* z, const float* Wt, const float* bias, const float* pos, float* x, int C, int g, int D, int64_t rows, int x_f16, uint32_t* guard, void* stream); }
 namespace ncsn_upf { bool configure(); void launch(const void* gemm_args, int epi, void* stream); void fold(const float* w, void* dst_bf16, float* dst_f32, int N, int Cin, float wmul, void* stream); }
+namespace ncsn_stem { bool configure(); void launch(const void* gemm_args, const float* x, void* stream); }
 namespace ncsn_cg3 { bool configure(); int tile_rows(int shape); int tile_cols(int shape); void launch(const void* gemm_args, int shape, int epi, void* stream); }
 
 namespace {
@@ -162,7 +163,7 @@
     bool ok = hipFuncSetAttribute(reinterpret_cast<const void*>(&k_gemm_bf16), hipFuncAttributeMaxDynamicSharedMemorySize,
                                   GEMM_LDS_BYTES) == hipSuccess;
     ok = ok && set_lds<CfgR128x128>(&k_gemm_ring<2, 2, 4, 4, 4, 9>) && set_lds<W128Cfg>(&k_gemm_w128<9>) &&
-         configure_families(GemmFamilies{}) && configure_families(ConvGnShapes{}) && ncsn_upf::configure() && configure_families(Fp8Families{}) &&
+         configure_families(GemmFamilies{}) && configure_families(ConvGnShapes{}) && ncsn_upf::configure() && ncsn_stem::configure() && configure_families(Fp8Families{}) &&
          ncsn_cg3::configure() && ncsn_sg::configure() && ::configure_conv_ring() && configure_ncsnpp_kernels() && configure_dit_attention() && configure_flash_attention();
     if (!ok) (void)hipGetLastError();
     return ok;
diff --git a/naturaldiffusion_amd/csrc/ncsnpp.hip b/naturaldiffusion_amd/csrc/ncsnpp.hip
--- a/naturaldiffusion_amd/csrc/ncsnpp.hip
+++ b/naturaldiffusion_amd/csrc/ncsnpp.hip
@@ -45,6 +45,18 @@
 constexpr int UP_FOLD_DEFAULT = 1;
 int g_fuse_up_fold = UP_FOLD_DEFAULT;
 int g_fuse_up = 1;
+constexpr int TEMB_SLOTS_DEFAULT = 32;
+int g_temb_slots = TEMB_SLOTS_DEFAULT;
+
+struct TembCache {
+    struct Slot {
+        uint32_t key = 0; int B = 0; bool valid = false; uint64_t used = 0;
+        hipEvent_t filled = nullptr;
+        hipStream_t fill_stream = nullptr, use_stream = nullptr;
+    };
+    int slots = 0; float* buf = nullptr; std::vector<Slot> slot; uint64_t tick = 0; int64_t hits = 0, misses = 0;
+    void invalidate() { for (auto& s : slot) s.valid = false; }
+};
 
 }
 
@@ -60,6 +72,8 @@
     uint64_t plan_sig = 0;
     int last_B = 0; unsigned char* last_ws = nullptr;
     std::vector<unsigned char> fin_done;
+    int temb_ops = 0, dense_total = 0; int64_t dense_out = -1, tlab = -1;
+    TembCache tc;
 };
 
 namespace {
@@ -118,6 +132,21 @@
     hipLaunchKernelGGL(k_attn256<true>, dim3((unsigned)(2 * a.B)), dim3(256), A256_LDS_BYTES, s, (const bf16*)a.qk, 2 * C, C, (const bf16*)a.vT, a.out, a.o_ld,
                        1.0f / sqrtf((float)C), a.w3f, a.b3, a.x, a.x_ld, a.out_scale, a.gn_part, a.gn_quads);
     return 128;
+}
+
+int g_fuse_stem = 1;
+bool stem_conv_takes(const GemmArgs& g) {
+    return g_fuse_stem && g.gn_part && g.N == NF && g.M % 256 == 0 && choose_variant(g) == V_RING_256x128_W4 && effective_epi(V_RING_256x128_W4, g) == 2;
+}
+int launch_stem_conv(const GemmArgs& g, const float* x, hipStream_t s) {
+    const std::string row = gemm_row(g.M, g.N, 64, 0, 1, 1, "stem_conv", 2);
+    if (g_record) { *g_record += row + "\n"; return 256; }
+    GemmProf::Rec r;
+    const bool prof = g_gemm_prof.on && g_gemm_prof.begin(r, s);
+    if (prof) r.tag = row;
+    ncsn_stem::launch(&g, x, (void*)s);
+    if (prof) g_gemm_prof.end(r, s);
+    return 256;
 }
 
 struct Builder : PlanBuilder {
@@ -251,7 +280,7 @@
             if (fold_up) {
                 g.a0 = c.act(h); g.a0_ld = h.ld; g.a0_padded = 1; g.a0_C = cin; g.taps = 4; g.logW = logW - 1; g.logHW = logHW - 2;
                 g.M = c.B * (HWo / 4); g.N = 4 * cout; g.b = c.w<bf16>(w0); g.b_ld = 4 * cin; g.bias_n = c.w<float>(b0);
-                g.rowvec = c.at<float>(dout) + drow; g.rowvec_ld = dtotal; g.log_rows_per_sample = logHW - 2;
+                g.rowvec = (c.temb_row ? c.temb_row : c.at<float>(dout)) + drow; g.rowvec_ld = c.temb_row ? 0 : dtotal; g.log_rows_per_sample = logHW - 2;
                 g.c = c.act(t); g.c_ld = t.ld;
                 if (pt.valid) { g.gn_part = c.at<float>(pt.off); g.gn_quads = pt.quads; }
                 const int bm = launch_gemm(g, c.stream);
@@ -264,7 +293,7 @@
             g.M = c.B * HWo; g.N = cout; g.b = c.w<bf16>(w0); g.b_ld = K0a;
             if (w0f >= 0) g.b_frag = c.w<bf16>(w0f);
             g.bias_n = c.w<float>(b0);
-            g.rowvec = c.at<float>(dout) + drow; g.rowvec_ld = dtotal; g.log_rows_per_sample = logHW;
+            g.rowvec = (c.temb_row ? c.temb_row : c.at<float>(dout)) + drow; g.rowvec_ld = c.temb_row ? 0 : dtotal; g.log_rows_per_sample = logHW;
             if (skws >= 0) { g.splitk_ws = c.at<float>(skws); g.splitk_max = SK_MAX; }
             g.c = c.act(t); g.c_ld = t.ld;
             if (pt.valid) { g.gn_part = c.at<float>(pt.off); g.gn_quads = pt.quads; set_fin(g, pt, c); }
@@ -648,6 +677,7 @@
         dense_w = wres((int64_t)dense_total * TEMB * 2); dense_b = wres((int64_t)dense_total * 4);
         dense_out = arena.alloc((int64_t)dense_total * 4);
         const int64_t emb = arena.alloc(128 * 2), t1 = arena.alloc(TEMB * 2), t2 = arena.alloc(TEMB * 2);
+        E.dense_total = dense_total; E.dense_out = dense_out; E.tlab = arena.alloc(4);
 
         size_t mi = 0;
         {
@@ -677,6 +707,7 @@
                 g.c = c.at<float>(dout); g.c_ld = dtot; g.c_mode = OUT_F32;
                 launch_gemm(g, c.stream);
             });
+            E.temb_ops = (int)E.ops.size();
         }
         int si = 0;
         TRef cur = skip_slot(si++);
@@ -690,18 +721,22 @@
             const int64_t a0 = arena.alloc((int64_t)IMG * IMG * 64 * 2);
             const TRef dst = cur;
             const Part po = register_output(dst);
+            auto stem_gemm = [=](const Ctx& c) {
+                GemmArgs g = gemm_defaults();
+                g.a0 = c.at<bf16>(a0); g.a0_ld = 64; g.a0_C = 64; g.M = (int)((int64_t)c.B * IMG * IMG); g.N = NF;
+                g.b = c.w<bf16>(w); g.b_ld = 64; g.bias_n = c.w<float>(b);
+                g.c = c.act(dst); g.c_ld = dst.ld;
+                if (po.valid) { g.gn_part = c.at<float>(po.off); g.gn_quads = po.quads; }
+                return g;
+            };
             op(CLS_OTHER, [=](const Ctx& c) {
+                if (stem_conv_takes(stem_gemm(c))) return;
                 const int64_t rows = (int64_t)c.B * IMG * IMG;
                 hipLaunchKernelGGL(k_stem_im2col, dim3((unsigned)((rows * 8 + 255) / 256)), dim3(256), 0, c.stream, c.x, c.at<bf16>(a0), rows);
             });
             op(CLS_GEMM, [=](const Ctx& c) {
-                const int64_t rows = (int64_t)c.B * IMG * IMG;
-                GemmArgs g = gemm_defaults();
-                g.a0 = c.at<bf16>(a0); g.a0_ld = 64; g.a0_C = 64; g.M = (int)rows; g.N = NF;
-                g.b = c.w<bf16>(w); g.b_ld = 64; g.bias_n = c.w<float>(b);
-                g.c = c.act(dst); g.c_ld = dst.ld;
-                if (po.valid) { g.gn_part = c.at<float>(po.off); g.gn_quads = po.quads; }
-                const int bm = launch_gemm(g, c.stream);
+                const GemmArgs g = stem_gemm(c);
+                const int bm = stem_conv_takes(g) ? launch_stem_conv(g, c.x, c.stream) : launch_gemm(g, c.stream);
                 if (po.valid) c.part_bm[po.id] = bm;
             });
             arena.release(a0);
@@ -875,6 +910,7 @@
     natinf_ncsnpp* e = make_engine(flags);
     if (!e) return NATINF_ESTATE;
     e->plan_sig = plan_signature();
+    e->tc.slots = g_temb_slots;
     *out = e;
     return NATINF_OK;
 }
@@ -883,6 +919,8 @@
     if (!h) return NATINF_EINVAL;
     for (auto& r : h->recs) { (void)hipEventDestroy(r.a); (void)hipEventDestroy(r.b); }
     for (auto e : h->pool) (void)hipEventDestroy(e);
+    for (auto& sl : h->tc.slot) if (sl.filled) (void)hipEventDestroy(sl.filled);
+    if (h->tc.buf) (void)hipFree(h->tc.buf);
     delete h;
     return NATINF_OK;
 }
@@ -903,7 +941,9 @@
 
 int natinf_ncsnpp_load(natinf_ncsnpp_t h, const float* params_f32, int64_t n_params, void* packed, int64_t packed_bytes,
                        natinf_stream_t stream) {
-    return h ? h->load(params_f32, n_params, packed, packed_bytes, (hipStream_t)stream) : NATINF_EINVAL;
+    if (!h) return NATINF_EINVAL;
+    h->tc.invalidate();
+    return h->load(params_f32, n_params, packed, packed_bytes, (hipStream_t)stream);
 }
 
 int natinf_ncsnpp_share(natinf_ncsnpp_t h, natinf_ncsnpp_t loaded) {
@@ -913,25 +953,16 @@
         h->packs.size() != loaded->packs.size() || h->plan_sig != loaded->plan_sig)
         return NATINF_EINVAL;
     h->packed = loaded->packed;
+    h->tc.invalidate();
     return NATINF_OK;
 }
 
-int natinf_ncsnpp_forward(natinf_ncsnpp_t h, const float* x, const float* labels, float* out, int B, void* workspace,
-                          int64_t workspace_bytes, natinf_stream_t stream) {
-    if (!h || !x || !labels || !out || !workspace || B <= 0) return NATINF_EINVAL;
-    if (!h->packed) return NATINF_ESTATE;
-    if (workspace_bytes < h->ws_per_image * (int64_t)B || (int64_t)B * IMG * IMG >= (1LL << 31)) return NATINF_EINVAL;
-    if (!h->configured) {
-        if (!configure_gemm_kernels()) return NATINF_ENODEV;
-        h->configured = true;
-    }
-    Ctx c{B, reinterpret_cast<unsigned char*>(workspace), h->packed, (hipStream_t)stream, x, labels, out, h->part_bm.data()};
-    c.fin_done = h->fin_done.data();
+static int run_ops(natinf_ncsnpp_t h, const Ctx& c, size_t first) {
     g_launch_error = 0;
     if (!h->prof) {
-        for (const auto& f : h->ops) f(c);
+        for (size_t i = first; i < h->ops.size(); ++i) h->ops[i](c);
     } else {
-        for (size_t i = 0; i < h->ops.size(); ++i) {
+        for (size_t i = first; i < h->ops.size(); ++i) {
             natinf_ncsnpp::Rec r; r.cls = h->op_cls[i];
             for (hipEvent_t* e : {&r.a, &r.b}) {
                 if (!h->pool.empty()) { *e = h->pool.back(); h->pool.pop_back(); }
@@ -943,9 +974,83 @@
             h->recs.push_back(r);
         }
     }
-    h->last_B = B; h->last_ws = c.ws;
+    h->last_B = c.B; h->last_ws = c.ws;
     if (g_launch_error) { g_launch_error = 0; return NATINF_ESTATE; }
     return hipGetLastError() == hipSuccess ? NATINF_OK : NATINF_ELAUNCH;
+}
+
+int natinf_ncsnpp_forward(natinf_ncsnpp_t h, const float* x, const float* labels, float* out, int B, void* workspace,
+                          int64_t workspace_bytes, natinf_stream_t stream) {
+    if (!h || !x || !labels || !out || !workspace || B <= 0) return NATINF_EINVAL;
+    if (!h->packed) return NATINF_ESTATE;
+    if (workspace_bytes < h->ws_per_image * (int64_t)B || (int64_t)B * IMG * IMG >= (1LL << 31)) return NATINF_EINVAL;
+    if (!h->configured) {
+        if (!configure_gemm_kernels()) return NATINF_ENODEV;
+        h->configured = true;
+    }
+    Ctx c{B, reinterpret_cast<unsigned char*>(workspace), h->packed, (hipStream_t)stream, x, labels, out, h->part_bm.data()};
+    c.fin_done = h->fin_done.data();
+    return run_ops(h, c, 0);
+}
+
+int natinf_ncsnpp_forward_t(natinf_ncsnpp_t h, const float* x, float t, float* out, int B, void* workspace, int64_t workspace_bytes, natinf_stream_t stream) {
+    if (!h || !x || !out || !workspace || B <= 0) return NATINF_EINVAL;
+    if (!h->packed) return NATINF_ESTATE;
+    if (workspace_bytes < h->ws_per_image * (int64_t)B || (int64_t)B * IMG * IMG >= (1LL << 31)) return NATINF_EINVAL;
+    if (!h->configured) {
+        if (!configure_gemm_kernels()) return NATINF_ENODEV;
+        h->configured = true;
+    }
+    hipStream_t s = (hipStream_t)stream;
+    Ctx c{B, reinterpret_cast<unsigned char*>(workspace), h->packed, s, x, nullptr, out, h->part_bm.data()};
+    c.fin_done = h->fin_done.data();
+    TembCache& tc = h->tc;
+    const size_t row_bytes = (size_t)h->dense_total * 4;
+    if (tc.slots > 0 && !tc.buf) {
+        if (hipMalloc(reinterpret_cast<void**>(&tc.buf), (size_t)tc.slots * row_bytes) != hipSuccess) { (void)hipGetLastError(); tc.buf = nullptr; return NATINF_ENODEV; }
+        tc.slot.assign(tc.slots, TembCache::Slot());
+        for (auto& sl : tc.slot)
+            if (hipEventCreateWithFlags(&sl.filled, hipEventDisableTiming) != hipSuccess) { (void)hipGetLastError(); return NATINF_ENODEV; }
+    }
+    uint32_t key; memcpy(&key, &t, 4);
+    int hit = -1, victim = -1;
+    for (int i = 0; i < tc.slots; ++i) {
+        const TembCache::Slot& sl = tc.slot[i];
+        if (sl.valid && sl.key == key && sl.B == B) { hit = i; break; }
+        if (victim < 0 || (tc.slot[victim].valid && (!sl.valid || sl.used < tc.slot[victim].used))) victim = i;
+    }
+    if (hit >= 0) {
+        TembCache::Slot& sl = tc.slot[hit];
+        if (s != sl.fill_stream && hipStreamWaitEvent(s, sl.filled, 0) != hipSuccess) { (void)hipGetLastError(); return NATINF_ELAUNCH; }
+        sl.used = ++tc.tick; sl.use_stream = s; ++tc.hits;
+        c.temb_row = tc.buf + (size_t)hit * h->dense_total;
+        return run_ops(h, c, (size_t)h->temb_ops);
+    }
+    ++tc.misses;
+    float* lab = c.at<float>(h->tlab);
+    hipLaunchKernelGGL(k_fill_f32, dim3(grid1d(B, 256, 1 << 30)), dim3(256), 0, s, lab, t, (int64_t)B);
+    c.labels = lab;
+    const int rc = run_ops(h, c, 0);
+    if (rc != NATINF_OK || victim < 0) return rc;
+    TembCache::Slot& sl = tc.slot[victim];
+    if (sl.valid && sl.use_stream != s && hipDeviceSynchronize() != hipSuccess) { (void)hipGetLastError(); return NATINF_ELAUNCH; }
+    sl.valid = false;
+    if (hipMemcpyAsync(tc.buf + (size_t)victim * h->dense_total, c.at<float>(h->dense_out), row_bytes, hipMemcpyDeviceToDevice, s) != hipSuccess ||
+        hipEventRecord(sl.filled, s) != hipSuccess) { (void)hipGetLastError(); return NATINF_ELAUNCH; }
+    sl.key = key; sl.B = B; sl.valid = true; sl.used = ++tc.tick; sl.fill_stream = s; sl.use_stream = s;
+    return NATINF_OK;
+}
+
+int natinf_set_temb_cache(int slots) {
+    if (slots < 0 || slots > 4096) return NATINF_EINVAL;
+    g_temb_slots = slots;
+    return NATINF_OK;
+}
+
+int natinf_ncsnpp_temb_cache_stats(natinf_ncsnpp_t h, int64_t* hits, int64_t* misses) {
+    if (!h || !hits || !misses) return NATINF_EINVAL;
+    *hits = h->tc.hits; *misses = h->tc.misses;
+    return NATINF_OK;
 }
 
 int natinf_ncsnpp_describe_gemms(natinf_ncsnpp_t h, int B, char* buf, int cap) {
@@ -1000,12 +1105,21 @@
     return NATINF_OK;
 }
 
+int g_dbg_gemm_log_sample = 0;
+int natinf_debug_set_gemm_sample_rows(int log_rows) {
+    if (log_rows < 0 || log_rows > 24) return NATINF_EINVAL;
+    g_dbg_gemm_log_sample = log_rows;
+    return NATINF_OK;
+}
+
 int natinf_debug_gemm_fused(int variant, int M, int N, int K, const void* a, const void* b, const float* bias_n, const float* bias_m,
                             const float* rowvec, const float* gate, int log_rows_per_sample, const void* resid_bf16, const float* resid_f32,
                             float scale, int act, void* c, int c_f32, float* gn_part, int* bm_out, int fp32_slab, natinf_stream_t stream) {
     const int logW = g_dbg_conv_logW, c1 = g_dbg_conv_c1;
     const void* a1 = g_dbg_conv_a1;
     g_dbg_conv_logW = 0; g_dbg_conv_a1 = nullptr; g_dbg_conv_c1 = 0;
+    const int log_sample = g_dbg_gemm_log_sample;
+    g_dbg_gemm_log_sample = 0;
     if (variant < 0 || variant >= V_COUNT || !a || !b || !c || M <= 0 || N <= 0 || K <= 0 || c_f32 < 0 || c_f32 > 2) return NATINF_EINVAL;
     if (c_f32 == 2) {
         if (!logW || bias_m || rowvec || gate || resid_bf16 || resid_f32 || gn_part || act != ACT_NONE) return NATINF_EINVAL;
@@ -1018,7 +1132,7 @@
     if (logW) {
         g.taps = 9; g.a0_C = g.a0_ld = K / 9; g.logW = logW; g.logHW = 2 * logW; g.a0_padded = 1; g.b_ld = K + c1;
         if (a1) { g.a1 = (const bf16*)a1; g.a1_C = g.a1_ld = c1; }
-    }
+    } else if (log_sample) g.logHW = log_sample;
     g.bias_n = bias_n; g.bias_m = bias_m; g.rowvec = rowvec; g.rowvec_ld = N; g.gate = gate; g.gate_ld = N; g.log_rows_per_sample = log_rows_per_sample;
     g.resid = (const bf16*)resid_bf16; g.resid_ld = N; g.resid_f32 = resid_f32; g.resid_f32_ld = N;
     g.scale = scale; g.act = act; g.c = c; g.c_ld = N; g.c_mode = c_f32 == 2 ? OUT_F32_NCHW : (c_f32 ? OUT_F32 : OUT_BF16);
@@ -1323,6 +1437,19 @@
     return hipGetLastError() == hipSuccess ? NATINF_OK : NATINF_ELAUNCH;
 }
 
+int natinf_set_fuse_stem(int on) { g_fuse_stem = on != 0; return NATINF_OK; }
+
+int natinf_debug_stem_conv(const float* x, const void* w_packed, const float* bias, void* out, float* gn_part, int B, natinf_stream_t stream) {
+    if (!x || !w_packed || !out || !gn_part || B < 1 || B > (1 << 17) || dbg_misaligned(w_packed, 16) || dbg_misaligned(out, 16) || dbg_misaligned(gn_part, 8) ||
+        dbg_misaligned(bias, 16)) return NATINF_EINVAL;
+    if (!ncsn_stem::configure()) { (void)hipGetLastError(); return NATINF_ENODEV; }
+    GemmArgs g = gemm_defaults();
+    g.a0_ld = 64; g.a0_C = 64; g.M = B * 1024; g.N = NF; g.b = (const bf16*)w_packed; g.b_ld = 64; g.bias_n = bias;
+    g.c = out; g.c_ld = NF; g.gn_part = gn_part; g.gn_quads = NF / 4;
+    ncsn_stem::launch(&g, x, (void*)stream);
+    return hipGetLastError() == hipSuccess ? NATINF_OK : NATINF_ELAUNCH;
+}
+
 int natinf_debug_pack_conv(const float* src, void* dst, int N, int Cin, int taps, int dst_ld, int koff, int tap_stride_c, int chunked, float wmul, natinf_stream_t stream) {
     if (!src || !dst || N < 1 || Cin < 1 || taps < 1 || koff < 0 || (chunked != 0 && chunked != 1)) return NATINF_EINVAL;
     const int64_t n = (int64_t)N * Cin * taps;
diff --git a/naturaldiffusion_amd/csrc/stem_conv.h b/naturaldiffusion_amd/csrc/stem_conv.h
--- /dev/null
+++ b/naturaldiffusion_amd/csrc/stem_conv.h
@@ -0,0 +1,81 @@
+#pragma once
+#include "gemm_dma.h"
+
+namespace ncsn {
+
+using StemCfg = RingCfg<2, 2, 8, 4, 3>;
+
+__global__ __launch_bounds__(256, 2) void k_stem_conv(const GemmArgs g, const float* __restrict__ x)
+{
+    using Cfg = StemCfg;
+    constexpr int WN = 2, TM = 8, TN = 4, BM_ = Cfg::BM_, BN_ = Cfg::BN_, ROW = 32;
+    constexpr int A_TILE = BM_ * ROW * 2, B_TILE = BN_ * ROW * 2;
+    static_assert(BM_ == 256 && BN_ == 128 && 2 * (A_TILE + B_TILE) <= Cfg::LDS_BYTES, "one row per thread, both K-tiles resident");
+    extern __shared__ __attribute__((aligned(16))) unsigned char smem[];
+    lds_poison();
+    const int tid = threadIdx.x, lane = tid & 63;
+    const int wave = __builtin_amdgcn_readfirstlane(tid >> 6);
+    const int wm = wave / WN, wn = wave % WN;
+    const int m0 = blockIdx.x * BM_;
+    unsigned char* sA = smem;
+    unsigned char* sB = smem + 2 * A_TILE;
+
+    uint4 wv[4];
+#pragma unroll
+    for (int j = 0; j < 4; ++j) {
+        const int idx = tid + 256 * j, n = idx >> 3, ch = idx & 7;
+        wv[j] = gload_u4(g.b + (int64_t)n * g.b_ld + ch * 8);
+    }
+    const int m = m0 + tid;
+    const int b = m >> 10, p = m & 1023, yy = p >> 5, xx = p & 31;
+    const float* xb = x + (((int64_t)b * 3) << 10);
+    float v[27];
+#pragma unroll
+    for (int k = 0; k < 27; ++k) {
+        const int tap = k / 3, c = k - tap * 3, sy = yy + tap / 3 - 1, sx = xx + tap % 3 - 1;
+        v[k] = ((unsigned)sy < 32u && (unsigned)sx < 32u) ? xb[(c << 10) + sy * 32 + sx] : 0.f;
+    }
+    const int sw = (0x1320 >> (((tid >> 2) & 3) * 4)) & 3;
+#pragma unroll
+    for (int q = 0; q < 4; ++q) {
+        bf16x8 o;
+#pragma unroll
+        for (int e = 0; e < 8; ++e) o[e] = (bf16)(q * 8 + e < 27 ? v[q * 8 + e] : 0.f);
+        *reinterpret_cast<bf16x8*>(sA + tid * 64 + ((q ^ sw) << 4)) = o;
+        *reinterpret_cast<uint4*>(sA + A_TILE + tid * 64 + (q << 4)) = make_uint4(0u, 0u, 0u, 0u);
+    }
+#pragma unroll
+    for (int j = 0; j < 4; ++j) {
+        const int idx = tid + 256 * j, n = idx >> 3, ch = idx & 7, kt = ch >> 2, q = ch & 3;
+        const int swn = (0x1320 >> (((n >> 2) & 3) * 4)) & 3;
+        *reinterpret_cast<uint4*>(sB + kt * B_TILE + n * 64 + ((q ^ swn) << 4)) = wv[j];
+    }
+    __syncthreads();
+
+    f32x4 acc[TM][TN];
+#pragma unroll
+    for (int i = 0; i < TM; ++i)
+#pragma unroll
+        for (int j = 0; j < TN; ++j) acc[i][j] = f32x4{0.f, 0.f, 0.f, 0.f};
+    const int frow = lane & 15, fq = lane >> 4;
+    const int fko = (fq ^ ((0x1320 >> (((frow >> 2) & 3) * 4)) & 3)) << 3;
+#pragma unroll
+    for (int kt = 0; kt < 2; ++kt) {
+        const bf16* ta = reinterpret_cast<const bf16*>(sA + kt * A_TILE) + (wm * TM * 16 + frow) * ROW + fko;
+        const bf16* tb = reinterpret_cast<const bf16*>(sB + kt * B_TILE) + (wn * TN * 16 + frow) * ROW + fko;
+        bf16x8 fb[TN];
+#pragma unroll
+        for (int j = 0; j < TN; ++j) fb[j] = *reinterpret_cast<const bf16x8*>(tb + j * 16 * ROW);
+#pragma unroll
+        for (int i = 0; i < TM; ++i) {
+            const bf16x8 fa = *reinterpret_cast<const bf16x8*>(ta + i * 16 * ROW);
+#pragma unroll
+            for (int j = 0; j < TN; ++j)
+                acc[i][j] = __builtin_amdgcn_mfma_f32_16x16x32_bf16(fb[j], fa, acc[i][j], 0, 0, 0);
+        }
+    }
+    __syncthreads();
+    tile_epilogue<2, WN, TM, TN, typename Cfg::Epi, 2>(g, smem, acc, m0, 0, 0, tid, lane, wm, wn);
+}
+
+}
diff --git a/naturaldiffusion_amd/csrc/stem_conv.hip b/naturaldiffusion_amd/csrc/stem_conv.hip
--- /dev/null
+++ b/naturaldiffusion_amd/csrc/stem_conv.hip
@@ -0,0 +1,19 @@
+#include <hip/hip_runtime.h>
+#include <stdint.h>
+#include <string.h>
+
+namespace {
+#include "stem_conv.h"
+}
+using namespace ncsn;
+
+namespace ncsn_stem {
+__attribute__((visibility("hidden"))) bool configure() {
+    return hipFuncSetAttribute(reinterpret_cast<const void*>(&k_stem_conv), hipFuncAttributeMaxDynamicSharedMemorySize, StemCfg::LDS_BYTES) == hipSuccess;
+}
+__attribute__((visibility("hidden"))) void launch(const void* gemm_args, const float* x, void* stream) {
+    GemmArgs g;
+    memcpy(&g, gemm_args, sizeof(g));
+    hipLaunchKernelGGL(k_stem_conv, dim3((unsigned)(g.M / StemCfg::BM_)), dim3(StemCfg::THREADS), StemCfg::LDS_BYTES, reinterpret_cast<hipStream_t>(stream), g, x);
+}
+}
diff --git a/naturaldiffusion_amd/ncsnpp.py b/naturaldiffusion_amd/ncsnpp.py
--- a/naturaldiffusion_amd/ncsnpp.py
+++ b/naturaldiffusion_amd/ncsnpp.py
@@ -158,6 +158,24 @@
                                         stream_ptr()), "natinf_ncsnpp_forward")
         return out
 
+    def forward_uniform(self, x: torch.Tensor, t: float, out: torch.Tensor = None) -> torch.Tensor:
+        if x.dtype != torch.float32 or x.dim() != 4 or tuple(x.shape[1:]) != (3, 32, 32) or not x.is_cuda:
+            raise ValueError("x must be a CUDA fp32 tensor of shape [B,3,32,32]")
+        B = x.shape[0]
+        if B > self.max_batch:
+            raise ValueError(f"batch {B} exceeds max_batch {self.max_batch}")
+        x = x.contiguous()
+        if out is None:
+            out = torch.empty_like(x)
+        check(lib.natinf_ncsnpp_forward_t(self._h, ptr(x), float(t), ptr(out), B, ptr(self._ws), self._ws.numel(), stream_ptr()),
+              "natinf_ncsnpp_forward_t")
+        return out
+
+    def temb_cache_stats(self) -> Tuple[int, int]:
+        hits, misses = C.c_int64(), C.c_int64()
+        check(lib.natinf_ncsnpp_temb_cache_stats(self._h, C.byref(hits), C.byref(misses)), "natinf_ncsnpp_temb_cache_stats")
+        return hits.value, misses.value
+
     def profile(self, enable: bool) -> None:
         check(lib.natinf_ncsnpp_profile(self._h, 1 if enable else 0), "natinf_ncsnpp_profile")
 
diff --git a/naturaldiffusion_amd/sampler.py b/naturaldiffusion_amd/sampler.py
--- a/naturaldiffusion_amd/sampler.py
+++ b/naturaldiffusion_amd/sampler.py
@@ -540,8 +540,11 @@
         x = self.first_input(noise, **kw) if inpaint or gray_u is not None else noise
         xs = [x.view(shape)]
         for k in range(self.n_step):
-            labels = torch.full((B,), self.labels[k], dtype=torch.float32, device=self.device)
-            out = model_fn(x.view(shape), labels)
+            if hasattr(model_fn, "forward_uniform"):
+                out = model_fn.forward_uniform(x.view(shape), self.labels[k])
+            else:
+                labels = torch.full((B,), self.labels[k], dtype=torch.float32, device=self.device)
+                out = model_fn(x.view(shape), labels)
             x = self.step(k, x.reshape(-1), out.contiguous().reshape(-1), noise.reshape(-1), **kw)
             if return_all:
                 x = x.clone()
```

New measurement: 3571 images/s (median of 6 runs). Within noise of the previous version (+0.7%).
